# yangao07/LAMSA

Measured on AMD Instinct MI355X. Metric: aligned Gbase/s, 10 kbp ONT-error reads (12%: sub/ins/del 4% each), -T ont2d vs GRCh37-sized stand-in; inputs resident in HBM when the timed region starts (upload excluded: see pcie_inclusive_*), higher is better.
Workload: dtype int32

## Files before the change

### lamsa_amd/csrc/hp_align.h

```cpp
#pragma once
#include "hp_out.h"
#include "hp_sort.h"

namespace hp {

HP_FN void regs_push(ReadCtx &r, Regs &G, int cap, const Rec &rec)
{
    if (G.n >= cap) { r.cx.status |= ST_OVERFLOW; return; }
    const cig_t *c = rec.cig.c; const int n = rec.cig.n, k = G.n;
    const int reflen = cig_reflen(c, n);
    G.rb[k].chr = G.re[k].chr = rec.chr; G.rb[k].is_rev = G.re[k].is_rev = 1 - rec.nstrand;
    if (rec.nstrand == 1) {
        G.beg[k] = (c[0] & 0xf) == C_S ? (c[0] >> 4) + 1 : 1;
        G.end[k] = (c[n - 1] & 0xf) == C_S ? r.L - (c[n - 1] >> 4) : r.L;
        G.rb[k].pos = rec.offset; G.re[k].pos = rec.offset + reflen - 1;
    } else {
        G.beg[k] = (c[n - 1] & 0xf) == C_S ? (c[n - 1] >> 4) + 1 : 1;
        G.end[k] = (c[0] & 0xf) == C_S ? r.L - (c[0] >> 4) : r.L;
        G.re[k].pos = rec.offset; G.rb[k].pos = rec.offset + reflen - 1;
    }
    ++G.n;
}

HP_NOINL void regs_remain(ReadCtx &r, Regs &G, int min_thd, int max_thd)
{
    const lamsa_hp_para *P = r.cx.P;
    G.m = 0;
    if (G.n == 0) {
        if (min_thd < r.L && r.L <= max_thd) { G.r_beg[0] = 1; G.r_end[0] = r.L; G.r_bs[0] = G.r_bn[0] = G.r_es[0] = G.r_en[0] = 0; G.m = 1; }
        return;
    }
    for (int i = 1; i < G.n; ++i) {
        const int b = G.beg[i], e = G.end[i]; const RegB rb = G.rb[i], re = G.re[i];
        int k = i - 1;
        while (k >= 0 && G.beg[k] > b) { G.beg[k + 1] = G.beg[k]; G.end[k + 1] = G.end[k]; G.rb[k + 1] = G.rb[k]; G.re[k + 1] = G.re[k]; --k; }
        G.beg[k + 1] = b; G.end[k + 1] = e; G.rb[k + 1] = rb; G.re[k + 1] = re;
    }
    int gs = 0, g_beg = G.beg[0], g_end = G.end[0];
    int prev_gs = -1, prev_ge = -1, prev_end = 0, first = 1;
    for (int i = 1; i <= G.n; ++i) {
        if (i < G.n && G.beg[i] - g_end - 1 < P->bwt_seed_len) { if (G.end[i] > g_end) g_end = G.end[i]; continue; }
        if (first) {
            if (g_beg > min_thd && g_beg - 1 <= max_thd) { const int m = G.m++; G.r_beg[m] = 1; G.r_end[m] = g_beg - 1; G.r_bs[m] = 0; G.r_bn[m] = 0; G.r_es[m] = gs; G.r_en[m] = i - gs; }
            first = 0;
        } else if (g_beg - prev_end > min_thd && g_beg - 1 - prev_end <= max_thd) {
            const int m = G.m++; G.r_beg[m] = prev_end + 1; G.r_end[m] = g_beg - 1; G.r_bs[m] = prev_gs; G.r_bn[m] = prev_ge - prev_gs; G.r_es[m] = gs; G.r_en[m] = i - gs;
        }
        prev_gs = gs; prev_ge = i; prev_end = g_end;
        if (i < G.n) { gs = i; g_beg = G.beg[i]; g_end = G.end[i]; }
    }
    if (r.L - prev_end > min_thd && r.L - prev_end <= max_thd) {
        HP_STAT(10);
        const int m = G.m++; G.r_beg[m] = prev_end + 1; G.r_end[m] = r.L; G.r_bs[m] = prev_gs; G.r_bn[m] = prev_ge - prev_gs; G.r_es[m] = 0; G.r_en[m] = 0;
    }
}

HP_NOINL void fill_round(ReadCtx &r, const FLines &F, OutBuf &o, Regs *G, int reg_cap, int scale, int tags)
{
    Ctx &cx = r.cx;
    const size_t mark = arena_mark(cx.tmp);
    const LineBufs b = line_bufs(cx, r.L, scale, tags);
    LineRes *la = b.la;
    if (!la) { arena_release(cx.tmp, mark); return; }
    for (int j = 0; j < F.n; ++j) {
        if (!fill_line(r, F, j, *la, b.cur_buf, b.cur_cap, b.rec_buf, b.rec_cap)) break;
        out_line(cx, o, *la);
        if (G && la->tol_score >= 0) for (int k = 0; k <= la->cur_res_n; ++k) regs_push(r, *G, reg_cap, la->rec[k]);
    }
    arena_release(cx.tmp, mark);
}

HP_INL void read_bind(ReadCtx &r, const lamsa_hp_para &P, const RefView &ref, const BatchIn &in, int rd, char *slab, size_t slab_bytes, HP_L int32_t *lds, long long *prof, int lds_words = HP_BOTH_LDS_WORDS)
{
    r.cx.P = &P; r.cx.status = 0; r.cx.n_cells = 0; r.cx.lds_epoch = 0; r.cx.prof_dp = nullptr; r.n_pairs = 0; r.cx.lds = lds; r.cx.lds_words = lds_words; r.cx.prof = prof ? prof + (size_t)rd * 64 : nullptr;
    arena_init(r.cx.tmp, slab, slab_bytes);
    r.ref = ref;
    r.L = (int)(in.read_off[rd + 1] - in.read_off[rd]);
    r.read = in.read_seq + in.read_off[rd];
    r.seed_all = in.seed_all[rd]; r.last_len = in.last_len[rd];
    const int64_t s0 = in.seed_off[rd];
    r.seed_out = (int)(in.seed_off[rd + 1] - s0);
    r.seed_id = in.seed_id + s0; r.hit_off = in.hit_off + s0;
    r.hb = r.hit_off[0];
    r.H = (int)(r.hit_off[r.seed_out] - r.hb);
    r.h_pos = in.h_pos + r.hb; r.h_chr = in.h_chr + r.hb; r.h_cig_off = in.h_cig_off + r.hb; r.h_nm = in.h_nm + r.hb;
    r.h_len_dif = in.h_len_dif + r.hb; r.h_strand = in.h_strand + r.hb; r.h_cig_n = in.h_cig_n + r.hb; r.cig = in.cig;
    r.flip = false; r.cur_read = r.read; r.rc_ready = false; r.rc_read = nullptr; r.t_bases = 0; r.cs_words = 0;
    r.prof = r.cx.prof; r.leaf_bits = nullptr; r.leaf_on = false; r.nodes_ready = false;
}

HP_FN void nodes_fill(ReadCtx &r)
{
    const HP_G int64_t *g_hoff = (const HP_G int64_t *)r.hit_off;
    const HP_G int32_t *g_sid = (const HP_G int32_t *)r.seed_id;
    const HP_G int16_t *g_hnm = (const HP_G int16_t *)r.h_nm;
    const int64_t hb = r.hb;
    const int H = r.H, S = r.seed_out;
    const lamsa_hp_para *P = r.cx.P;
    HP_L int32_t *lo_ = r.cx.lds;
    const bool in_lds = S + 1 <= r.cx.lds_words;
    int min_num = 0;
    if (in_lds) wv::sync();
    for (int s0 = 0; s0 <= S; s0 += 64) {
        wv::Lane<int> few;
        WAVE_FOR(l) {
            const int s = s0 + l;
            int f = 0;
            if (s <= S) { const int o = (int)(g_hoff[s] - hb); if (in_lds) lo_[s] = o; if (s < S) f = (int)(g_hoff[s + 1] - hb) - o <= P->first_loci_thd; }
            few[l] = f;
        }
        min_num += __builtin_popcountll(wv::ballot(few));
    }
    wv::sync();
    const bool all_min = min_num == 0 || min_num * 3 < S;
    HP_G int32_t *g_from = (HP_G int32_t *)r.n_from, *g_in_de = (HP_G int32_t *)r.n_in_de, *g_son_n = (HP_G int32_t *)r.n_son_n, *g_first = (HP_G int32_t *)r.n_first,
                 *g_last = (HP_G int32_t *)r.n_last, *g_ms = (HP_G int32_t *)r.n_max_score, *g_mn = (HP_G int32_t *)r.n_max_NM, *g_mx = (HP_G int32_t *)r.n_max_node,
                 *g_nn = (HP_G int32_t *)r.n_node_n, *g_seed = (HP_G int32_t *)r.n_seed;
    HP_G NodeS *gd = (HP_G NodeS *)r.nd;
    for (int k0 = 0; k0 < H; k0 += 64) {
        WAVE_FOR(l) {
            const int k = k0 + l;
            if (k < H) {
                int lo = 0, hi = S;
                while (hi - lo > 1) { const int mid = (lo + hi) >> 1; if ((in_lds ? lo_[mid] : (int)(g_hoff[mid] - hb)) <= k) lo = mid; else hi = mid; }
                const int s = lo, b = in_lds ? lo_[s] : (int)(g_hoff[s] - hb), e = in_lds ? lo_[s + 1] : (int)(g_hoff[s + 1] - hb);
                const int nm = g_hnm[k];
                g_seed[k] = s;
                const int64_t pos = r.h_pos[k];
                const int w4 = ((int)g_sid[s] & 0xffff) | (((int)r.h_strand[k] & 0xff) << 16) | (((int)r.h_len_dif[k] & 0xff) << 24);
                const int flag = (all_min || e - b <= P->first_loci_thd) ? MIN_FLAG : MULTI_FLAG;
                hp_store16(gd + k, (int)(pos & 0xffffffffll), (int)(pos >> 32), r.h_chr[k], (s << 14) | (k - b));
                hp_store16((HP_G char *)(gd + k) + 16, w4, (flag & 0xff) | (F_INIT << 8) | (F_MATCH << 16), 1, nm);
                g_from[k] = -1; g_nn[k] = 1; g_in_de[k] = 0; g_son_n[k] = 0; g_first[k] = -1; g_last[k] = -1; g_ms[k] = 1; g_mn[k] = nm; g_mx[k] = k;
            }
        }
    }
    r.nodes_ready = true;
    wv::sync();
}

HP_INL void aux_bind(ReadCtx &r, int32_t *nm)
{
    const int c = r.H + 1;
    r.n_from = nm; r.n_in_de = nm + c; r.n_son_n = nm + 2 * c; r.n_first = nm + 3 * c;
    r.n_last = nm + 4 * c; r.n_next = nm + 5 * c; r.n_max_score = nm + 6 * c; r.n_max_NM = nm + 7 * c; r.n_max_node = nm + 8 * c;
    r.n_node_n = nm + 9 * c;
}

#ifdef HP_PROF
#define HP_STAMP(k) do { const long long now_ = wv::clock(); if (a.prof) a.prof[(size_t)rd * 64 + (k)] += now_ - t_last_; t_last_ = now_; } while (0)
#else
#define HP_STAMP(k) do { } while (0)
#endif

HP_NOINL void align_read(const AlignArgs &a, int rd, int wave_slot, HP_L int32_t *lds)
{
#ifdef HP_PROF
    long long t_last_ = wv::clock();
#endif
    ReadCtx r;
    read_bind(r, a.P, a.ref, a.in, rd, a.slab + (size_t)wave_slot * a.slab_per_wave, a.slab_per_wave, lds, a.prof);
    Ctx &cx = r.cx;
    const bool skip = a.in.read_skip && a.in.read_skip[rd];
    if (skip) { cx.status |= ST_UNSUPPORTED; r.H = 0; r.seed_out = 0; }
    const int H = r.H;
    const int tags = fill_tags(a.in.tags);
    const int out_cap = (int)read_out_cap(r.L, a.scale, tags);
    OutBuf o; o.n = 0; o.cap = out_cap;
    o.w = (int32_t *)arena_alloc(cx, sizeof(int32_t) * (size_t)out_cap);
    r.rc_read = (uint8_t *)arena_alloc(cx, (size_t)r.L + 16);
    int32_t *nm = (int32_t *)arena_alloc(cx, sizeof(int32_t) * 11 * (size_t)(H + 1));
    int32_t *sidx = (int32_t *)arena_alloc(cx, sizeof(int32_t) * 2 * (size_t)(H + 1));
    r.nd = (NodeS *)arena_alloc(cx, sizeof(NodeS) * (size_t)(H + 1));
    const int reg_cap = 256 * a.scale;
    Regs G; G.n = 0; G.m = 0;
    G.beg = (int32_t *)arena_alloc(cx, sizeof(int32_t) * 2 * (size_t)reg_cap); G.end = G.beg + reg_cap;
    G.rb = (RegB *)arena_alloc(cx, sizeof(RegB) * 2 * (size_t)reg_cap); G.re = G.rb + reg_cap;
    G.r_beg = (int32_t *)arena_alloc(cx, sizeof(int32_t) * 6 * (size_t)(reg_cap + 2));
    G.r_end = G.r_beg + (reg_cap + 2); G.r_bs = G.r_end + (reg_cap + 2); G.r_bn = G.r_bs + (reg_cap + 2); G.r_es = G.r_bn + (reg_cap + 2); G.r_en = G.r_es + (reg_cap + 2);
    int n0_pos = 1, n1_pos = 2;
    const size_t sort_mark = arena_mark(cx.tmp);
    uint64_t *sort_work = (uint64_t *)arena_alloc(cx, sizeof(uint64_t) * (size_t)(H + 1));
    if (!skip && o.w && r.rc_read && nm && sidx && sort_work && r.nd && G.beg && G.rb && G.r_beg) {
        const int c = H + 1;
        { HP_T0(t_sort_);
        sort_read_hits(r.h_pos, r.h_chr, r.h_strand, H, sidx, sidx + c, sort_work, (HP_L uint64_t *)lds, HP_BOTH_LDS_WORDS / 2, a.sort_pb, a.sort_cb);
        HP_TADD(cx, 46, t_sort_); }
        arena_release(cx.tmp, sort_mark);
        r.srt = sidx; r.rnk = sidx + c;
        aux_bind(r, nm); r.n_seed = nm + 10 * c;
        nodes_fill(r);
        out_put(cx, o, 0); out_put(cx, o, 0); out_put(cx, o, 0);
        HP_STAMP(0);
        {
            const size_t mark = arena_mark(cx.tmp);
            FLines F;
            const bool ok1 = chain_first(r, F);
            HP_STAMP(1);
            if (ok1 && F.n > 0) { o.w[n0_pos] = F.n; fill_round(r, F, o, &G, reg_cap, a.scale, tags); }
            HP_STAMP(2);
            arena_release(cx.tmp, mark);
        }
        if (!(cx.status & ST_DEAD)) {
            const size_t mark = arena_mark(cx.tmp);
            regs_remain(r, G, a.P.seed_len, r.L);
            FLines F;
            const bool ok2 = chain_remain(r, G, F);
            HP_STAMP(3);
            if (ok2 && F.n > 0) { o.w[n1_pos] = F.n; fill_round(r, F, o, nullptr, 0, a.scale, tags); }
            HP_STAMP(4);
            arena_release(cx.tmp, mark);
        }
    }
    const int st = cx.status;
    int n_words = (st & ST_DEAD) || !o.w ? 3 : o.n;
    unsigned long long off = 0;
    if (wv::leader()) off = atomicAdd(a.out.cursor, (unsigned long long)n_words);
    off = (unsigned long long)wv::uni64((long long)off);
    if ((int64_t)(off + (unsigned long long)n_words) <= a.out.stream_cap) {
        int32_t *dst = a.out.stream + off;
        if (n_words == 3 && (!o.w || (st & ST_DEAD))) { dst[0] = st; dst[1] = 0; dst[2] = 0; }
        else {
            o.w[0] = st;
            wv::sync();
            out_copy((HP_G int32_t *)dst, (const HP_G int32_t *)o.w, n_words);
        }
        a.out.read_out_off[rd] = (int64_t)off; a.out.read_out_len[rd] = n_words;
    } else { a.out.read_out_off[rd] = -1; a.out.read_out_len[rd] = 0; }
    a.out.read_status[rd] = st;
    HP_STAMP(5);
    if (a.out.read_tbases) a.out.read_tbases[rd] = (int32_t)(r.t_bases > 0x7fffffffLL ? 0x7fffffffLL : r.t_bases);
    if (a.out.read_work) {
        a.out.read_work[4 * rd] = (int32_t)(cx.n_cells > 0x7fffffffLL ? 0x7fffffffLL : cx.n_cells);
        a.out.read_work[4 * rd + 1] = (int32_t)(r.n_pairs > 0x7fffffffLL ? 0x7fffffffLL : r.n_pairs);
        a.out.read_work[4 * rd + 2] = (int32_t)(r.cs_words > 0x7fffffffLL ? 0x7fffffffLL : r.cs_words);
        a.out.read_work[4 * rd + 3] = 0;
    }
}

}
```

### lamsa_amd/csrc/hp_align_api.hip

```cpp
#include <hip/hip_runtime.h>
#include <algorithm>
#include <atomic>
#include <map>
#include <mutex>
#include <stdlib.h>
#include <string.h>
#include <time.h>
#include "hp_phase.h"
#include "hp_handle.h"
#include "hp_hostprep.h"

using namespace hp;

#ifndef HP_WAVES_PER_SIMD
#define HP_WAVES_PER_SIMD 4
#endif
__global__ __launch_bounds__(64, HP_WAVES_PER_SIMD) void k_align_batch(AlignArgs a)
{
    __shared__ int32_t lds[HP_BOTH_LDS_WORDS];
    const int slot = blockIdx.x;
    for (;;) {
        int u = 0;
        if (wv::leader()) u = atomicAdd(a.counter, 1);
        u = wv::uni(u);
        if (u >= a.n_units) break;
        align_read(a, a.order ? a.order[u] : u, slot, (HP_L int32_t *)lds);
    }
}

#ifndef HP_CHAIN_WAVES_PER_SIMD
#define HP_CHAIN_WAVES_PER_SIMD 4
#endif
#ifndef HP_FILL_WAVES_PER_SIMD
#define HP_FILL_WAVES_PER_SIMD 7
#endif
template <int WORDS, int WPS>
__global__ __launch_bounds__(64, WPS) void k_chain1(const PhaseArgs *ap)
{
    const PhaseArgs &a = *ap;
    constexpr bool ctx_lds = ph_ctx_in_lds(WORDS, WPS);
    __shared__ alignas(16) int32_t lds[WORDS + (ctx_lds ? PH_CTX_BYTES / 4 : 0)];
    ReadCtx &r = *(ctx_lds ? (ReadCtx *)(lds + WORDS) : (ReadCtx *)(a.slab + (size_t)blockIdx.x * a.slab_per_wave));
    for (;;) {
        int u = 0;
        if (wv::leader()) u = atomicAdd(&a.ctl->q_head[0], 1);
        u = wv::uni(u);
        if (u >= a.n_reads) break;
        phase_chain1(a, a.order ? a.order[u] : u, blockIdx.x, (HP_L int32_t *)lds, WORDS, r);
    }
    drain_stamp(a, 0);
}
template <int WORDS, int WPS>
__global__ __launch_bounds__(64, WPS) void k_chain2(const PhaseArgs *ap)
{
    const PhaseArgs &a = *ap;
    constexpr bool ctx_lds = ph_ctx_in_lds(WORDS, WPS);
    __shared__ alignas(16) int32_t lds[WORDS + (ctx_lds ? PH_CTX_BYTES / 4 : 0)];
    ReadCtx &r = *(ctx_lds ? (ReadCtx *)(lds + WORDS) : (ReadCtx *)(a.slab + (size_t)blockIdx.x * a.slab_per_wave));
    for (;;) {
        int u = 0;
        if (wv::leader()) u = atomicAdd(&a.ctl->q_head[2], 1);
        u = wv::uni(u);
        if (u >= a.n_reads) break;
        phase_chain2(a, a.order ? a.order[u] : u, blockIdx.x, (HP_L int32_t *)lds, WORDS, r);
    }
    drain_stamp(a, 2);
}
typedef void (*ChainKernel)(const PhaseArgs *);
struct ChainShape { ChainKernel k1, k2; int lds_words, waves_per_simd; };
static const ChainShape g_chain_shapes[3] = {
    {k_chain1<HP_CHAIN_LDS_WORDS, HP_CHAIN_WAVES_PER_SIMD>, k_chain2<HP_CHAIN_LDS_WORDS, HP_CHAIN_WAVES_PER_SIMD>, HP_CHAIN_LDS_WORDS, HP_CHAIN_WAVES_PER_SIMD},
    {k_chain1<3392, 3>, k_chain2<3392, 3>, 3392, 3},
    {k_chain1<5120, 2>, k_chain2<5120, 2>, 5120, 2},
};
__global__ __launch_bounds__(64, HP_FILL_WAVES_PER_SIMD) void k_fill(const PhaseArgs *ap, int round)
{
    const PhaseArgs &a = *ap;
    __shared__ alignas(16) int32_t lds[HP_LDS_WORDS + PH_CTX_BYTES / 4];
    ReadCtx &r = *(ReadCtx *)(lds + HP_LDS_WORDS);
    int n = 0;
    for (int b = 0; b < PH_NBUCKET; ++b) n += a.ctl->bucket_n[round][b];
    n = wv::uni(n);
    for (;;) {
        int g = 0;
        if (wv::leader()) g = atomicAdd(&a.ctl->q_head[1 + 2 * round], 1);
        g = wv::uni(g);
        if (g >= n) break;
        int b = 0;
        while (b < PH_NBUCKET - 1 && g >= a.ctl->bucket_n[round][b]) { g -= a.ctl->bucket_n[round][b]; ++b; }
        const int u = wv::uni(a.bucket_q[((size_t)round * PH_NBUCKET + b) * a.unit_cap + g]);
        phase_fill(a, round, u, blockIdx.x, (HP_L int32_t *)lds, r);
    }
    drain_stamp(a, 1 + 2 * round);
}
#ifndef HP_FILLDP_WAVES_PER_SIMD
#define HP_FILLDP_WAVES_PER_SIMD 2
#endif
#ifndef HP_LIST_WAVES_PER_SIMD
#define HP_LIST_WAVES_PER_SIMD 4
#endif
__global__ __launch_bounds__(64, HP_LIST_WAVES_PER_SIMD) void k_filllist(const PhaseArgs *ap, int round)
{
    const PhaseArgs &a = *ap;
    __shared__ alignas(16) int32_t lds[PH_CTX_BYTES / 4];
    ReadCtx &r = *(ReadCtx *)lds;
    int n = 0;
    for (int b = 0; b < PH_NBUCKET; ++b) n += a.ctl->bucket_n[round][b];
    n = wv::uni(n);
    for (;;) {
        int g = 0;
        if (wv::leader()) g = atomicAdd(&a.ctl->q_head[5], 1);
        g = wv::uni(g);
        if (g >= n) break;
        int b = 0;
        while (b < PH_NBUCKET - 1 && g >= a.ctl->bucket_n[round][b]) { g -= a.ctl->bucket_n[round][b]; ++b; }
        const int u = wv::uni(a.bucket_q[((size_t)round * PH_NBUCKET + b) * a.unit_cap + g]);
        phase_filllist(a, round, u, blockIdx.x, (HP_L int32_t *)lds, r);
    }
}
__global__ __launch_bounds__(64, 2) void k_filldp_small(const PhaseArgs *ap, int round)
{
    __shared__ int32_t lds[HP_LJ_LDS_WORDS(HP_LJ_QSMALL)];
    const PhaseArgs &a = *ap;
    int n = 0;
    for (int b = 0; b < LJ_NBUCKET; ++b) n += (lj_queue_n(a, round, b) + 63) >> 6;
    n = wv::uni(n);
    for (;;) {
        int g = 0;
        if (wv::leader()) g = atomicAdd(&a.ctl->q_head[6], 1);
        g = wv::uni(g);
        if (g >= n) break;
        int b = 0;
        for (; b < LJ_NBUCKET - 1; ++b) { const int gb = (lj_queue_n(a, round, b) + 63) >> 6; if (g < gb) break; g -= gb; }
        phase_filldp(a, round, b, g * 64, blockIdx.x, (HP_L int32_t *)lds, HP_LJ_QSMALL);
    }
}
__global__ __launch_bounds__(64, HP_WJ_WAVES_PER_SIMD) void k_filldp_wave(const PhaseArgs *ap, int round)
{
    __shared__ int32_t lds[HP_WJ_LDS_WORDS];
    const PhaseArgs &a = *ap;
    int n = 0, n_big = 0;
    for (int b = 0; b < WJ_NBUCKET; ++b) { const int k = wj_queue_n(a, round, b); if (b < WJ_NBIG) n_big += k; else n += k; }
    n = wv::uni(n); n_big = wv::uni(n_big);
    bool own_big = (int)blockIdx.x < a.n_wjb;
    for (;;) {
        int g = 0;
        const bool big = own_big;
        if (wv::leader()) g = atomicAdd(&a.ctl->q_head[big ? 8 : 7], 1);
        g = wv::uni(g);
        if (g >= (big ? n_big : n)) { if (!big) break; own_big = false; continue; }
        phase_wavejob(a, round, g, big, blockIdx.x, (HP_L int32_t *)lds);
    }
}
__global__ __launch_bounds__(64) void k_publish(const PhaseArgs *ap)
{
    const PhaseArgs &a = *ap;
    if (blockIdx.x == 0) publish_diag(a);
    for (;;) {
        int u = 0;
        if (wv::leader()) u = atomicAdd(&a.ctl->q_head[4], 1);
        u = wv::uni(u);
        if (u >= a.n_reads) break;
        phase_publish(a, u);
    }
}

__global__ void k_cig8_expand(const uint8_t *src, int32_t *dst, int64_t n)
{
    for (int64_t i = (int64_t)blockIdx.x * blockDim.x + threadIdx.x; i < n; i += (int64_t)gridDim.x * blockDim.x) { const int b = src[i]; dst[i] = ((b & 63) << 4) | (b >> 6); }
}
__global__ void k_off_widen(const int32_t *src, int64_t *dst, int64_t n)
{
    for (int64_t i = (int64_t)blockIdx.x * blockDim.x + threadIdx.x; i < n; i += (int64_t)gridDim.x * blockDim.x) dst[i] = src[i];
}
#define HP_SCAN_BLOCK 4096
__global__ __launch_bounds__(256) void k_scan_sums(const uint8_t *src, int64_t n, int64_t *sums)
{
    __shared__ int part[256];
    const int64_t b0 = (int64_t)blockIdx.x * HP_SCAN_BLOCK;
    int s = 0;
    for (int i = threadIdx.x; i < HP_SCAN_BLOCK; i += 256) { const int64_t k = b0 + i; s += k < n ? src[k] : 0; }
    part[threadIdx.x] = s;
    __syncthreads();
    for (int st = 128; st > 0; st >>= 1) { if ((int)threadIdx.x < st) part[threadIdx.x] += part[threadIdx.x + st]; __syncthreads(); }
    if (threadIdx.x == 0) sums[blockIdx.x] = part[0];
}
__global__ __launch_bounds__(256) void k_scan_bases(int64_t *sums, int64_t nb)
{
    __shared__ long long tot[256];
    const int64_t per = (nb + 255) / 256, a = (int64_t)threadIdx.x * per, b = a + per < nb ? a + per : nb;
    long long s = 0;
    for (int64_t i = a; i < b; ++i) s += sums[i];
    tot[threadIdx.x] = s;
    __syncthreads();
    if (threadIdx.x == 0) { long long run = 0; for (int t = 0; t < 256; ++t) { const long long v = tot[t]; tot[t] = run; run += v; } }
    __syncthreads();
    long long run = tot[threadIdx.x];
    for (int64_t i = a; i < b; ++i) { const long long v = sums[i]; sums[i] = run; run += v; }
}
__global__ __launch_bounds__(256) void k_scan_apply(const uint8_t *src, int64_t n, const int64_t *bases, int64_t *dst)
{
    __shared__ int part[256];
    const int64_t b0 = (int64_t)blockIdx.x * HP_SCAN_BLOCK + (int64_t)threadIdx.x * 16;
    int v[16], s = 0;
#pragma unroll
    for (int i = 0; i < 16; ++i) { const int64_t k = b0 + i; v[i] = k < n ? src[k] : 0; s += v[i]; }
    part[threadIdx.x] = s;
    __syncthreads();
    if (threadIdx.x == 0) { int run = 0; for (int t = 0; t < 256; ++t) { const int x = part[t]; part[t] = run; run += x; } }
    __syncthreads();
    long long run = bases[blockIdx.x] + part[threadIdx.x];
#pragma unroll
    for (int i = 0; i < 16; ++i) { const int64_t k = b0 + i; if (k < n) dst[k] = run; run += v[i]; }
}

static double now_s() { timespec t; clock_gettime(CLOCK_MONOTONIC, &t); return t.tv_sec + 1e-9 * t.tv_nsec; }
static const bool g_trace = getenv("LAMSA_HP_TRACE") != nullptr;
static const bool g_noshare = getenv("LAMSA_HP_FULL_GRIDS") != nullptr;
static const bool g_nowave = getenv("LAMSA_HP_NO_WAVE_JOBS") != nullptr;
static const bool g_nolane = getenv("LAMSA_HP_NO_LANE_DP") != nullptr;
static const bool g_mono = getenv("LAMSA_HP_ONE_KERNEL") != nullptr;

struct HostBuf {
    void *p = nullptr, *dev = nullptr; size_t cap = 0;
    int ensure(size_t bytes) {
        if (bytes <= cap) return 0;
        if (p) hipHostFree(p);
        p = dev = nullptr; cap = 0;
        size_t want = bytes + bytes / 4 + 256;
        if (hipHostMalloc(&p, want, hipHostMallocMapped) != hipSuccess) { p = nullptr; return -1; }
        if (hipHostGetDevicePointer(&dev, p, 0) != hipSuccess) { hipHostFree(p); p = nullptr; return -1; }
        cap = want;
        return 0;
    }
    void release() { if (p) hipHostFree(p); p = dev = nullptr; cap = 0; }
};

struct OutDev {
    DevBuf buf; HostBuf host; int64_t stream_cap = 0; int n_cap = 0;
    static size_t hdr(int n) { return al256(8 * (size_t)n) + 3 * al256(4 * (size_t)n) + 256 + al256(16 * (size_t)n); }
    int ensure(int n, int64_t cap) { stream_cap = cap; n_cap = n; return buf.ensure(4 * (size_t)cap + 256) || host.ensure(hdr(n) + 256); }
    int64_t *off() const { return (int64_t *)host.dev; }
    int32_t *len(int n) const { return (int32_t *)((char *)host.dev + al256(8 * (size_t)n)); }
    int32_t *st(int n) const { return (int32_t *)((char *)host.dev + al256(8 * (size_t)n) + al256(4 * (size_t)n)); }
    int32_t *tb(int n) const { return (int32_t *)((char *)host.dev + al256(8 * (size_t)n) + 2 * al256(4 * (size_t)n)); }
    unsigned long long *diag(int n) const { return (unsigned long long *)((char *)host.dev + al256(8 * (size_t)n) + 3 * al256(4 * (size_t)n)); }
    const unsigned long long *h_diag(int n) const { return (const unsigned long long *)((const char *)host.p + al256(8 * (size_t)n) + 3 * al256(4 * (size_t)n)); }
    int32_t *work(int n) const { return (int32_t *)((char *)host.dev + al256(8 * (size_t)n) + 3 * al256(4 * (size_t)n) + 256); }
    const int32_t *h_work(int n) const { return (const int32_t *)((const char *)host.p + al256(8 * (size_t)n) + 3 * al256(4 * (size_t)n) + 256); }
    const int64_t *h_off() const { return (const int64_t *)host.p; }
    const int32_t *h_len(int n) const { return (const int32_t *)((const char *)host.p + al256(8 * (size_t)n)); }
    const int32_t *h_st(int n) const { return (const int32_t *)((const char *)host.p + al256(8 * (size_t)n) + al256(4 * (size_t)n)); }
    const int32_t *h_tb(int n) const { return (const int32_t *)((const char *)host.p + al256(8 * (size_t)n) + 2 * al256(4 * (size_t)n)); }
    int32_t *stream(int) const { return (int32_t *)buf.p; }
    void release() { buf.release(); host.release(); }
};

struct Slot {
    DevBuf bin, misc, slab, pers, prof; OutDev out1;
    HostBuf args_host;
    hipEvent_t ep[7] = {nullptr, nullptr, nullptr, nullptr, nullptr, nullptr, nullptr};
    hipStream_t cs = nullptr;
    bool valid = false;
    bool phased = false;
    int32_t n_reads = 0; int64_t n_bases = 0, n_cig = 0, n_hits = 0;
    BatchIn in; const int32_t *d_order = nullptr;
    std::vector<int32_t> order, h_len, h_H; std::vector<uint8_t> h_skip;
    int32_t max_L = 0, max_H = 0;
    int32_t sort_pb = 40, sort_cb = 24;
    hipEvent_t e0 = nullptr, e1 = nullptr;
};

struct AlignState {
    Slot slot[2];
    int fifo[2] = {0, 0}, n_fifo = 0;
    int res_fifo[2] = {0, 0}, n_res = 0;
    DevBuf retry_list;
    OutDev out2;
    HostBuf stream;
    std::vector<int32_t> r_len, r_st, r_tb, r_work; std::vector<int64_t> r_off;
};

static std::map<lamsa_hp_handle *, AlignState *> g_states;
static std::mutex g_states_lock;
static AlignState *state_of(lamsa_hp_handle *h)
{
    std::lock_guard<std::mutex> guard(g_states_lock);
    auto it = g_states.find(h);
    if (it != g_states.end()) return it->second;
    return g_states[h] = new AlignState();
}
extern "C" void lamsa_hp_release_state_(lamsa_hp_handle *h)
{
    AlignState *S = nullptr;
    {
        std::lock_guard<std::mutex> guard(g_states_lock);
        auto it = g_states.find(h);
        if (it == g_states.end()) return;
        S = it->second;
        g_states.erase(it);
    }
    if (h->stream) hipStreamSynchronize(h->stream);
    if (h->stream_b) hipStreamSynchronize(h->stream_b);
    for (Slot &T : S->slot) { T.bin.release(); T.misc.release(); T.slab.release(); T.pers.release(); T.prof.release(); T.args_host.release(); T.out1.release(); for (hipEvent_t e : {T.e0, T.e1, T.ep[0], T.ep[1], T.ep[2], T.ep[3], T.ep[4], T.ep[5], T.ep[6]}) if (e) hipEventDestroy(e); }
    S->retry_list.release(); S->out2.release(); S->stream.release();
    delete S;
}

static int grow(lamsa_hp_handle *h, DevBuf &b, size_t bytes)
{
    if (bytes <= b.cap) return 0;
    if (hipStreamSynchronize(h->stream) != hipSuccess || hipStreamSynchronize(h->stream_b) != hipSuccess) return -1;
    return b.ensure(bytes);
}


static int upload_into(lamsa_hp_handle *h, Slot *S, const lamsa_hp_batch *B)
{
    S->valid = false;
    const double t_0 = now_s();
    const int n = B->n_reads;
    const int64_t n_slots = n ? B->seed_off[n] : 0, n_hits = n_slots ? B->hit_off[n_slots] : 0, n_bases = n ? B->read_off[n] : 0;
    S->h_len.assign((size_t)n, 0); S->h_H.assign((size_t)n, 0); S->h_skip.assign((size_t)n + 1, 0); S->max_L = 0; S->max_H = 0;
    if (n && (B->seed_off[0] != 0 || B->read_off[0] != 0 || (n_slots && B->hit_off[0] != 0))) { h->err = "offsets must start at 0"; return LAMSA_HP_EINVAL; }
    const bool packed_off = B->h_cig_off == nullptr, cig_bytes = B->cig8 != nullptr;
    if (B->n_cig < 0 || (!packed_off && B->n_cig > 0x7fffffffll)) { h->err = "more than 2^31-1 seed CIGAR elements with 32-bit h_cig_off: pass h_cig_off = NULL (CIGARs back to back in hit order) or split the batch"; return LAMSA_HP_EINVAL; }
    if (!cig_bytes && !B->cig && B->n_cig > 0) { h->err = "neither cig nor cig8 given"; return LAMSA_HP_EINVAL; }
    {
        std::atomic<int> bad(0);
        const int64_t sl = h->para.seed_len, ss = h->para.seed_step > 0 ? h->para.seed_step : 1;
        std::atomic<long long> max_pos(0), sum_cig(0);
        hp_parallel_blocks(n, [&](int r0, int r1) {
            long long mp = 0, sc = 0;
            for (int r = r0; r < r1 && !bad.load(std::memory_order_relaxed); ++r) {
                const int64_t L = B->read_off[r + 1] - B->read_off[r], ns = B->seed_off[r + 1] - B->seed_off[r];
                if (L < 0 || L > (1 << 24) || ns < 0) { bad = 1; return; }
                if (ns > HP_MAX_SLOTS) S->h_skip[r] = 1;
                {
                    const int64_t sa = L < sl ? 0 : 1 + (L - sl) / ss;
                    if (B->seed_all[r] != sa || B->last_len[r] != L - sl - (sa - 1) * ss) { bad = 7; return; }
                    if (sa > 32767) S->h_skip[r] = 1;
                }
                int64_t H = 0;
                for (int64_t s = B->seed_off[r]; s < B->seed_off[r + 1]; ++s) {
                    const int64_t m = B->hit_off[s + 1] - B->hit_off[s];
                    if (m < 0 || (m > HP_MAX_HITS_PER_SEED && !S->h_skip[r])) { bad = 2; return; }
                    if (B->seed_id[s] < 1 || B->seed_id[s] > B->seed_all[r] || (s > B->seed_off[r] && B->seed_id[s] <= B->seed_id[s - 1])) { bad = 3; return; }
                    H += m;
                }
                if (H > (1 << 22) && !S->h_skip[r]) { bad = 4; return; }
                for (int64_t i = B->read_off[r]; i < B->read_off[r + 1]; ++i) if (B->read_seq[i] > 4) { bad = 5; return; }
                for (int64_t k = B->hit_off[B->seed_off[r]]; k < B->hit_off[B->seed_off[r + 1]]; ++k) {
                    mp = B->h_pos[k] > mp ? B->h_pos[k] : mp;
                    if (B->h_len_dif[k] < -127 || B->h_len_dif[k] > 127) S->h_skip[r] = 1;
                    if (B->h_chr[k] < 1 || B->h_chr[k] > h->n_seqs || (B->h_strand[k] != 1 && B->h_strand[k] != -1) || B->h_pos[k] < 0 || B->h_pos[k] >= (1ll << 40) ||
                        (!packed_off && (B->h_cig_off[k] < 0 || (int64_t)B->h_cig_off[k] + B->h_cig_n[k] > B->n_cig))) { bad = 6; return; }
                    sc += B->h_cig_n[k];
                }
                S->h_len[r] = (int32_t)L; S->h_H[r] = (int32_t)H;
            }
            long long seen = max_pos.load();
            while (mp > seen && !max_pos.compare_exchange_weak(seen, mp)) { }
            sum_cig += sc;
        });
        static const char *why[] = {"", "read longer than 2^24 bases", "too many hits in one seed", "seed ids must be ascending in [1, seed_all]",
                                    "too many hits in one read", "read base code > 4",
                                    "bad hit record (contig id, strand, position or seed CIGAR range)",
                                    "seed_all / last_len do not match the read length and the handle's seed length and step"};
        if (bad) { h->err = why[bad.load()]; return LAMSA_HP_EINVAL; }
        if (packed_off && sum_cig.load() != B->n_cig) { h->err = "h_cig_off is NULL but the h_cig_n do not add up to n_cig"; return LAMSA_HP_EINVAL; }
        for (int r = 0; r < n; ++r) { if (S->h_skip[r]) { S->h_len[r] = 0; S->h_H[r] = 0; } S->max_L = std::max(S->max_L, S->h_len[r]); S->max_H = std::max(S->max_H, S->h_H[r]); }
        auto bits = [](unsigned long long x) { int b = 0; while (x) { ++b; x >>= 1; } return b; };
        S->sort_pb = bits((unsigned long long)max_pos.load()); S->sort_cb = bits((unsigned long long)(2 * (long long)h->n_seqs + 1));
    }
    const double t_1 = now_s();
    S->order.resize((size_t)n);
    for (int r = 0; r < n; ++r) S->order[r] = r;
    {
        std::vector<double> cost((size_t)n);
        for (int r = 0; r < n; ++r) cost[r] = (double)S->h_H[r] * S->h_H[r] / 64.0 + (double)S->h_len[r] * (2.0 * h->para.band_w + 1) / 16.0;
        std::stable_sort(S->order.begin(), S->order.end(), [&](int x, int y) { return cost[x] > cost[y]; });
    }
    size_t off = 0;
    auto place = [&](size_t bytes) { size_t o = off; off = al256(off + bytes + 16); return o; };
    const size_t o_roff = place(8 * ((size_t)n + 1)), o_rseq = place((size_t)n_bases), o_sall = place(4 * (size_t)n), o_last = place(4 * (size_t)n),
                 o_soff = place(8 * ((size_t)n + 1)), o_sid = place(4 * (size_t)n_slots), o_hoff = place(8 * ((size_t)n_slots + 1)),
                 o_pos = place(8 * (size_t)n_hits), o_chr = place(4 * (size_t)n_hits), o_coff = place(8 * (size_t)n_hits), o_nm = place(2 * (size_t)n_hits),
                 o_ld = place(2 * (size_t)n_hits), o_st = place((size_t)n_hits), o_cn = place((size_t)n_hits), o_cig = place(4 * (size_t)B->n_cig), o_ord = place(4 * (size_t)n),
                 o_stage = place(packed_off ? 8 * ((size_t)n_hits / HP_SCAN_BLOCK + 2) : 4 * (size_t)n_hits), o_cig8 = place(cig_bytes ? (size_t)B->n_cig : 0), o_skip = place((size_t)n);
    const double t_3 = now_s();
    if (S->bin.ensure(off)) { h->err = "hipMalloc(batch)"; return LAMSA_HP_ENOMEM; }
    char *d = (char *)S->bin.p;
    hipStream_t s = h->copy_stream;
    static const int64_t zero64 = 0;
#define UP(o, src, bytes) do { if ((bytes) > 0) HIPCHK(h, hipMemcpyAsync(d + (o), (src), (bytes), hipMemcpyHostToDevice, s), LAMSA_HP_EKERNEL); } while (0)
    if (n) { UP(o_roff, B->read_off, 8 * ((size_t)n + 1)); UP(o_soff, B->seed_off, 8 * ((size_t)n + 1)); }
    else { UP(o_roff, &zero64, 8); UP(o_soff, &zero64, 8); }
    UP(o_rseq, B->read_seq, (size_t)n_bases); UP(o_sall, B->seed_all, 4 * (size_t)n); UP(o_last, B->last_len, 4 * (size_t)n);
    UP(o_sid, B->seed_id, 4 * (size_t)n_slots);
    if (n_slots) UP(o_hoff, B->hit_off, 8 * ((size_t)n_slots + 1)); else UP(o_hoff, &zero64, 8);
    UP(o_pos, B->h_pos, 8 * (size_t)n_hits); UP(o_chr, B->h_chr, 4 * (size_t)n_hits);
    if (!packed_off) UP(o_stage, B->h_cig_off, 4 * (size_t)n_hits);
    UP(o_nm, B->h_nm, 2 * (size_t)n_hits); UP(o_ld, B->h_len_dif, 2 * (size_t)n_hits); UP(o_st, B->h_strand, (size_t)n_hits); UP(o_cn, B->h_cig_n, (size_t)n_hits);
    if (cig_bytes) UP(o_cig8, B->cig8, (size_t)B->n_cig); else UP(o_cig, B->cig, 4 * (size_t)B->n_cig);
    UP(o_ord, S->order.data(), 4 * (size_t)n); UP(o_skip, S->h_skip.data(), (size_t)n);
#undef UP
    if (cig_bytes && B->n_cig > 0) hipLaunchKernelGGL(k_cig8_expand, dim3(2048), dim3(256), 0, s, (const uint8_t *)(d + o_cig8), (int32_t *)(d + o_cig), (int64_t)B->n_cig);
    if (n_hits > 0) {
        if (!packed_off) hipLaunchKernelGGL(k_off_widen, dim3(2048), dim3(256), 0, s, (const int32_t *)(d + o_stage), (int64_t *)(d + o_coff), (int64_t)n_hits);
        else {
            const int64_t nb = (n_hits + HP_SCAN_BLOCK - 1) / HP_SCAN_BLOCK;
            hipLaunchKernelGGL(k_scan_sums, dim3((unsigned)nb), dim3(256), 0, s, (const uint8_t *)(d + o_cn), (int64_t)n_hits, (int64_t *)(d + o_stage));
            hipLaunchKernelGGL(k_scan_bases, dim3(1), dim3(256), 0, s, (int64_t *)(d + o_stage), nb);
            hipLaunchKernelGGL(k_scan_apply, dim3((unsigned)nb), dim3(256), 0, s, (const uint8_t *)(d + o_cn), (int64_t)n_hits, (const int64_t *)(d + o_stage), (int64_t *)(d + o_coff));
        }
    }
    HIPCHK(h, hipGetLastError(), LAMSA_HP_EKERNEL);
    HIPCHK(h, hipStreamSynchronize(s), LAMSA_HP_EKERNEL);
    if (g_trace) fprintf(stderr, "[lamsa_hp] upload: validate %.1f ms, order %.1f ms, copy %.1f ms (%.2f GB on the device)\n", 1e3 * (t_1 - t_0), 1e3 * (t_3 - t_1), 1e3 * (now_s() - t_3), off / 1e9);
    BatchIn &in = S->in;
    in.n_reads = n; in.read_skip = (const uint8_t *)(d + o_skip); in.read_off = (const int64_t *)(d + o_roff); in.read_seq = (const uint8_t *)(d + o_rseq);
    in.seed_all = (const int32_t *)(d + o_sall); in.last_len = (const int32_t *)(d + o_last); in.seed_off = (const int64_t *)(d + o_soff);
    in.seed_id = (const int32_t *)(d + o_sid); in.hit_off = (const int64_t *)(d + o_hoff); in.h_pos = (const int64_t *)(d + o_pos);
    in.h_chr = (const int32_t *)(d + o_chr); in.h_cig_off = (const int64_t *)(d + o_coff); in.h_nm = (const int16_t *)(d + o_nm);
    in.h_len_dif = (const int16_t *)(d + o_ld); in.h_strand = (const int8_t *)(d + o_st); in.h_cig_n = (const uint8_t *)(d + o_cn);
    in.cig = (const int32_t *)(d + o_cig);
    S->d_order = (const int32_t *)(d + o_ord);
    S->n_reads = n; S->n_bases = n_bases; S->n_cig = B->n_cig; S->n_hits = n_hits;
    S->valid = true;
    return LAMSA_HP_OK;
}

static int cap_waves(int n_waves, size_t slab_per_wave, int n_cu)
{
    static const size_t budget = []() { size_t f = 0, t = 0; if (hipMemGetInfo(&f, &t) != hipSuccess || t == 0) { t = (size_t)288 << 30; f = t; } return std::min(t / 4, f / 3); }();
    if (slab_per_wave * (size_t)n_waves <= budget) return n_waves;
    size_t fit = budget / (slab_per_wave ? slab_per_wave : 1);
    if (n_cu > 0 && fit >= (size_t)n_cu) fit -= fit % (size_t)n_cu;
    return fit < 1 ? 1 : (int)fit;
}

#ifdef HP_PROF
static void prof_report(Slot &T, const long long *d_prof, int n)
{
    if (!d_prof) return;
    {
        std::vector<long long> pr((size_t)n * 64);
        hipMemcpy(pr.data(), d_prof, sizeof(long long) * pr.size(), hipMemcpyDeviceToHost);
        if (const char *dump = getenv("LAMSA_HP_PROF_DUMP")) {
            if (FILE *fp = fopen(dump, "wb")) {
                for (int r = 0; r < n; ++r) { long long hl[2] = {T.h_H[r], T.h_len[r]}; fwrite(hl, 8, 2, fp); fwrite(&pr[(size_t)r * 64], 8, 64, fp); }
                fclose(fp);
            }
        }
        std::vector<int> idx((size_t)n); for (int i = 0; i < n; ++i) idx[i] = i;
        auto tot = [&](int r) { long long t = 0; for (int k = 0; k < 6; ++k) t += pr[(size_t)r * 64 + k]; return t; };
        std::sort(idx.begin(), idx.end(), [&](int x, int y) { return tot(x) > tot(y); });
        long long sum[64] = {0}; for (int r = 0; r < n; ++r) for (int k = 0; k < 64; ++k) sum[k] += pr[(size_t)r * 64 + k];
        fprintf(stderr, "[HP_PROF] cycles: setup chain1 fill1 chain2 fill2 publish | in chain1: init+minext mainscan track pop-loop bound+flines | o_l H\n");
        fprintf(stderr, "[HP_PROF] SUM  "); for (int k = 0; k < 11; ++k) fprintf(stderr, " %lld", sum[k] / 1000000); fprintf(stderr, " (Mcycles) targets %lld trips %lld init_Mcyc %lld\n", sum[11], sum[12], sum[13] / 1000000);
#ifdef HP_PROF_TRACK
        fprintf(stderr, "[HP_PROF] branch tracking (-DHP_PROF_TRACK: the line_build stamps below are off): marking pass, image build and write-back %lld Mcyc; %lld seeds visited; %lld tracks, %lld Mcyc in them, %lld steps up; "
                        "%lld arrivals at a node with several sons, %lld Mcyc in cut_branch\n", sum[16] / 1000000, sum[19], sum[18], sum[17] / 1000000, sum[20], sum[21], sum[22] / 1000000);
#endif
#ifdef HP_PROF_EDGE
        fprintf(stderr, "[HP_PROF] main pass (-DHP_PROF_EDGE: the line_build stamps below are off), Mcyc: dp_cluster_lds load+pack %lld, MIN extension %lld, target loop %lld, write-back %lld; cluster_lane %lld; build_sons %lld\n",
                sum[16] / 1000000, sum[17] / 1000000, sum[18] / 1000000, sum[19] / 1000000, sum[20] / 1000000, sum[21] / 1000000);
#else
        fprintf(stderr, "[HP_PROF] line_build: %lld lines (%lld without a gap), %lld anchors, %lld gaps | Mcyc: anchor walk %lld, gap list %lld, gaps in lanes %lld, gaps one by one %lld, assembly %lld\n",
                sum[21], sum[22], sum[12], sum[23], sum[16] / 1000000, sum[17] / 1000000, sum[18] / 1000000, sum[19] / 1000000, sum[20] / 1000000);
#endif
        fprintf(stderr, "[HP_PROF] gaps: %lld in lines with fewer than HP_GAP_MIN gaps (%lld lines with gaps); lane gaps: %lld hits scanned, %lld refused (range too long or too many active hits)\n", sum[54], sum[55], sum[11], sum[13]);
        { const char *nm[] = {"ksw_global", "ksw_extend", "backtrack", "ref_fetch", "head_fix", "frag_extend", "split_mapping", "tail_fix", "res_split", "res_aux", "mini_line_regs", "sort index"};
          for (int k = 0; k < 12; ++k) fprintf(stderr, "[HP_PROF] %-16s %8lld Mcyc %10lld calls\n", nm[k], sum[24 + 2 * k] / 1000000, sum[25 + 2 * k]);
#ifdef HP_PROF_FILL
          fprintf(stderr, "[HP_PROF] in frags_merge: boundary repair (merge_cigar_full) %lld Mcyc %lld calls; junctions through split_mapping %lld Mcyc %lld calls; fragments of several seeds %lld Mcyc %lld calls; 64-step gathers %lld Mcyc %lld\n", sum[16] / 1000000, sum[17], sum[18] / 1000000, sum[19], sum[20] / 1000000, sum[21], sum[22] / 1000000, sum[23]);
#endif
          fprintf(stderr, "[HP_PROF] direction-matrix bytes in HBM %lld (%lld jobs); hits passed through nodes_per_init %lld (%lld calls)\n", sum[52], sum[53], sum[54], sum[55]);
          fprintf(stderr, "[HP_PROF] chain_first start: seed loop %lld, node_set loop %lld, min_extend %lld Mcyc (%lld reads with a MIN pass)\n", sum[56] / 1000000, sum[57] / 1000000, sum[58] / 1000000, sum[59]);
          fprintf(stderr, "[HP_PROF] query <= 62: ksw_extend %lld Mcyc %lld calls, ksw_global %lld Mcyc %lld calls\n", sum[60] / 1000000, sum[61], sum[62] / 1000000, sum[63]);
          const char *bn[] = {"[bi_extend total]", "[bi_extend after left ext]", "17-32", "33-64", "65-128", "129-256", "257-512", ">512"};
          for (int k = 0; k < 2; ++k) fprintf(stderr, "[HP_PROF] ksw_extend qlen %-8s %8lld Mcyc %10lld calls\n", bn[k], sum[48 + 2 * k] / 1000000, sum[49 + 2 * k]); }
        {
            std::vector<long long> pd((size_t)n * 64);
            hipMemcpy(pd.data(), d_prof + ((size_t)n + 1) * 64, sizeof(long long) * pd.size(), hipMemcpyDeviceToHost);
            long long sd[64] = {0}; for (int r = 0; r < n; ++r) for (int k = 0; k < 64; ++k) sd[k] += pd[(size_t)r * 64 + k];
            const char *cn[] = {"one set, q <= 62", "packed, one set", "packed, two sets", "band 1 set slides", "band 2 sets slides", "band 4 sets slides", "int32 sets", "LDS / HBM rows",
                                "band 1 set fixed", "band 2 sets fixed", "band 4 sets fixed"};
            for (int c = 0; c < 11; ++c) fprintf(stderr, "[HP_PROF] wave jobs, ksw_extend %-18s %8lld Mcyc %10lld Mcells %9lld calls %10lld rows\n", cn[c], sd[4 * c] / 1000000, sd[4 * c + 1] / 1000000, sd[4 * c + 2], sd[4 * c + 3]);
            fprintf(stderr, "[HP_PROF] wave jobs, junctions of the class 'band 2 sets fixed': %lld jobs, wj_run %lld Mcyc of which staging %lld; ksw_bi_extend %lld Mcyc of which after the left extension %lld; "
                            "in ksw_extend_band<2>: setup and first fill %lld, rows %lld, backtrack %lld Mcyc\n",
                    sd[51], sd[50] / 1000000, sd[49] / 1000000, sd[47] / 1000000, sd[48] / 1000000, sd[44] / 1000000, sd[45] / 1000000, sd[46] / 1000000);
        }
        for (int q = 0; q < 8 && q < n; ++q) { int r = idx[q]; fprintf(stderr, "[HP_PROF] read %d L=%d:", r, T.h_len[r]); for (int k = 0; k < 11; ++k) fprintf(stderr, " %lld", pr[(size_t)r * 64 + k] / 1000000); fprintf(stderr, " | o_l %lld H %lld | targets %lld trips %lld init_Mcyc %lld\n", pr[(size_t)r * 64 + 14], pr[(size_t)r * 64 + 15], pr[(size_t)r * 64 + 11], pr[(size_t)r * 64 + 12], pr[(size_t)r * 64 + 13] / 1000000); }
    }
}
#endif

struct PhasedLayout { size_t bytes, o[15]; int unit_cap, lj_cap, wj_cap; int64_t fl_cap, line_cap, job_cap; };
static PhasedLayout phased_layout(int n, int64_t n_hits, int64_t n_bases, int64_t stream_cap)
{
    PhasedLayout Y;
    const size_t n_ent = (size_t)n_hits + (size_t)n + 1;
    Y.unit_cap = 8 * n + 1024;
    Y.fl_cap = 4 * n_hits + 2304 * (int64_t)n + 4096; Y.line_cap = stream_cap + 64 * (int64_t)Y.unit_cap;
    Y.job_cap = std::min<int64_t>(0x7fffff00ll, 4096 + 256 * (int64_t)n + 2 * n_bases);
    Y.lj_cap = (int)std::min<int64_t>(0x3fffffffll, 1024 + 16 * (int64_t)n + n_bases / 100);
    Y.wj_cap = (int)std::min<int64_t>(0x3fffffffll, 1024 + 32 * (int64_t)n + n_bases / 200);
    size_t off = 0;
    auto place = [&](size_t bytes) { size_t o = off; off = al256(off + bytes + 16); return o; };
    const size_t sz[15] = {sizeof(PhaseArgs), sizeof(PhaseCtl), sizeof(RdMeta) * ((size_t)n + 1), sizeof(NodeS) * n_ent, 4 * n_ent, 8 * n_ent, sizeof(UnitRec) * 2 * (size_t)Y.unit_cap,
                           4 * 2 * (size_t)PH_NBUCKET * Y.unit_cap, 4 * (size_t)Y.fl_cap, 4 * (size_t)Y.line_cap, 4 * (size_t)Y.job_cap, sizeof(LjRec) * (size_t)Y.lj_cap, 4 * (size_t)LJ_NBUCKET * Y.lj_cap,
                           sizeof(WjRec) * (size_t)Y.wj_cap, 4 * (size_t)WJ_NBUCKET * Y.wj_cap};
    for (int k = 0; k < 15; ++k) Y.o[k] = place(sz[k]);
    Y.bytes = off;
    return Y;
}

struct SlabPlan { size_t chain, fill, wj, wjb, wjb_off; int w_chain, w_fill, w_dp, w_wj, n_wjb, shape; size_t bytes; };
static int chain_shape(const lamsa_hp_para &P, int64_t n_reads, int64_t n_bases)
{
    static const int force = getenv("LAMSA_HP_CHAIN_SHAPE") ? atoi(getenv("LAMSA_HP_CHAIN_SHAPE")) : -1;
    if (force >= 0 && force < 3) return force;
    const int64_t mean_L = n_reads > 0 ? n_bases / n_reads : 0, ss = P.seed_step > 0 ? P.seed_step : 1;
    const int64_t est = mean_L / ss * 2 / 3;
    for (int k = 0; k < 2; ++k) if (est <= g_chain_shapes[k].lds_words / 5) return k;
    return 2;
}
static SlabPlan slab_plan(lamsa_hp_handle *h, int max_L, int max_H, bool shared = false, int shape = 0)
{
    SlabPlan Q;
    Q.shape = shape;
    const lamsa_hp_para &P = h->para;
    Q.chain = al256(((size_t)256 << 10) + 128 * (size_t)max_L + 424 * (size_t)max_H);
    Q.fill = al256(fill_slab_bytes(max_L, h->result_tags, sizeof(cig_t) * 3 * HP_LJ_CIG * 64 + (size_t)HP_LJ_QSMALL * HP_LJ_TSMALL * 64 + 64));
    { static const int kb = getenv("LAMSA_HP_WJ_SLAB_KB") ? atoi(getenv("LAMSA_HP_WJ_SLAB_KB")) : 0;
      Q.wj = ((size_t)(kb > 0 ? kb : 1024) << 10) + 33 * 256; }
    Q.wjb = al256((size_t)wj_need(&P, WJ_HEAD, max_L, max_L + 2 * P.hash_step + 64) + ((size_t)64 << 10)) + 33 * 256;
    if (Q.wjb < Q.wj) Q.wjb = Q.wj;
    if (g_nowave) Q.fill = std::max(Q.fill, al256(read_slab_bytes(P.band_w, max_L, max_H, 1, h->result_tags)));
    if (h->scratch_limit) { const size_t lim = al256(h->scratch_limit); Q.chain = std::min(Q.chain, lim); Q.fill = std::min(Q.fill, lim); Q.wj = std::min(Q.wj, lim); Q.wjb = std::min(Q.wjb, lim); }
    int pc = 0, pf = 0, pd = 0, pw = 0;
    if (hipOccupancyMaxActiveBlocksPerMultiprocessor(&pc, g_chain_shapes[shape].k1, 64, 0) != hipSuccess || pc < 1) pc = 4 * g_chain_shapes[shape].waves_per_simd;
    if (hipOccupancyMaxActiveBlocksPerMultiprocessor(&pf, k_fill, 64, 0) != hipSuccess || pf < 1) pf = 4;
    if (hipOccupancyMaxActiveBlocksPerMultiprocessor(&pd, k_filldp_small, 64, 0) != hipSuccess || pd < 1) pd = 4;
    if (hipOccupancyMaxActiveBlocksPerMultiprocessor(&pw, k_filldp_wave, 64, 0) != hipSuccess || pw < 1) pw = 4;
    if (shared && !g_noshare) { pc = std::min(pc, 8); pf = std::min(pf, 16); pw = std::min(pw, 16); }
    { static const int cf = getenv("LAMSA_HP_FILL_PER_CU") ? atoi(getenv("LAMSA_HP_FILL_PER_CU")) : 0, cc = getenv("LAMSA_HP_CHAIN_PER_CU") ? atoi(getenv("LAMSA_HP_CHAIN_PER_CU")) : 0,
                       cw = getenv("LAMSA_HP_WJ_PER_CU") ? atoi(getenv("LAMSA_HP_WJ_PER_CU")) : 0;
      if (cf > 0 && cf < pf) pf = cf;
      if (cc > 0 && cc < pc) pc = cc;
      if (cw > 0 && cw < pw) pw = cw; }
    Q.w_chain = cap_waves(h->n_cu * pc, Q.chain, h->n_cu); Q.w_fill = cap_waves(h->n_cu * pf, Q.fill, h->n_cu);
    Q.w_dp = std::min(h->n_cu * pd, Q.w_fill); Q.w_wj = cap_waves(h->n_cu * pw, Q.wj, h->n_cu);
    { const size_t budget_big = (size_t)12 << 30; size_t nb = budget_big / Q.wjb; if (nb < 1) nb = 1; Q.n_wjb = (int)std::min<size_t>(nb, (size_t)Q.w_wj); }
    Q.wjb_off = al256(Q.wj * (size_t)Q.w_wj);
    const size_t wj_bytes = Q.wjb_off + Q.wjb * (size_t)Q.n_wjb;
    Q.bytes = std::max(std::max(Q.chain * (size_t)Q.w_chain, Q.fill * (size_t)Q.w_fill), wj_bytes);
    return Q;
}

static int launch_phased(lamsa_hp_handle *h, AlignState *S, Slot &T, Slot &Ln, OutDev &O, hipEvent_t e0, hipEvent_t e1)
{
    const int n = T.n_reads;
    const int64_t n_hits = T.n_hits;
    const SlabPlan Q = slab_plan(h, T.max_L, T.max_H, S->n_fifo + S->n_res > 0, chain_shape(h->para, T.n_reads, T.n_bases));
    const int w_chain = Q.w_chain, w_fill = Q.w_fill, w_dp = Q.w_dp, w_wj = Q.w_wj;
    const PhasedLayout Y = phased_layout(n, n_hits, T.n_bases, O.stream_cap);
    const int unit_cap = Y.unit_cap, lj_cap = Y.lj_cap; const int64_t fl_cap = Y.fl_cap, line_cap = Y.line_cap, job_cap = Y.job_cap;
    const size_t off = Y.bytes, o_args = Y.o[0], o_ctl = Y.o[1], o_meta = Y.o[2], o_nd = Y.o[3], o_ns = Y.o[4], o_sx = Y.o[5], o_un = Y.o[6], o_bq = Y.o[7], o_fl = Y.o[8], o_ln = Y.o[9],
                 o_jb = Y.o[10], o_lj = Y.o[11], o_lq = Y.o[12], o_wj = Y.o[13], o_wq = Y.o[14];
    if (grow(h, Ln.slab, Q.bytes) || grow(h, Ln.pers, off) || Ln.misc.ensure(256)) { h->err = "hipMalloc(slab)"; return LAMSA_HP_ENOMEM; }
    char *d = (char *)Ln.pers.p;
    PhaseArgs a;
    a.P = h->para;
    a.ref.pac = h->d_pac; a.ref.l_pac = h->l_pac; a.ref.n_seqs = h->n_seqs; a.ref.seq_off = h->d_seq_off; a.ref.seq_len = h->d_seq_len;
    a.in = T.in; a.in.tags = h->result_tags;
    a.out.read_out_off = O.off(); a.out.read_out_len = O.len(n); a.out.read_status = O.st(n); a.out.read_tbases = O.tb(n); a.out.read_work = O.work(n); a.out.stream = O.stream(n);
    a.out.stream_cap = O.stream_cap; a.out.cursor = (unsigned long long *)((char *)Ln.misc.p + 64); a.out.diag = O.diag(n);
    a.slab = (char *)Ln.slab.p; a.slab_per_wave = Q.chain; a.slab_fill = Q.fill; a.slab_wj = Q.wj; a.slab_wjb = Q.wjb; a.wjb_off = Q.wjb_off; a.n_wjb = Q.n_wjb; a.sort_pb = T.sort_pb; a.sort_cb = T.sort_cb;
    a.order = T.d_order; a.n_reads = n; a.prof = nullptr;
#ifdef HP_PROF
    if (Ln.prof.ensure(sizeof(long long) * 64 * 2 * ((size_t)n + 1))) { h->err = "hipMalloc(prof)"; return LAMSA_HP_ENOMEM; }
    a.prof = (long long *)Ln.prof.p;
    HIPCHK(h, hipMemsetAsync(Ln.prof.p, 0, sizeof(long long) * 64 * 2 * ((size_t)n + 1), Ln.cs), LAMSA_HP_EKERNEL);
#endif
    a.g_nd = (NodeS *)(d + o_nd); a.g_nseed = (int32_t *)(d + o_ns); a.g_sidx = (int32_t *)(d + o_sx); a.meta = (RdMeta *)(d + o_meta);
    a.units = (UnitRec *)(d + o_un); a.unit_cap = unit_cap; a.bucket_q = (int32_t *)(d + o_bq);
    a.fl_base = (int32_t *)(d + o_fl); a.fl_cap = fl_cap; a.line_base = (int32_t *)(d + o_ln); a.line_cap = line_cap; a.ctl = (PhaseCtl *)(d + o_ctl);
    a.job_base = (int32_t *)(d + o_jb); a.job_cap = job_cap;
    a.ljobs = (LjRec *)(d + o_lj); a.lj_bucket = (int32_t *)(d + o_lq); a.lj_cap = g_nolane ? 0 : lj_cap;
    a.wjobs = (WjRec *)(d + o_wj); a.wj_bucket = (int32_t *)(d + o_wq); a.wj_cap = g_nowave ? 0 : Y.wj_cap;
    const bool list = !g_nolane || !g_nowave;
    hipStream_t s = Ln.cs;
    HIPCHK(h, hipMemsetAsync(Ln.misc.p, 0, 128, s), LAMSA_HP_EKERNEL);
    HIPCHK(h, hipMemsetAsync(d + o_ctl, 0, (o_meta - o_ctl) + sizeof(RdMeta) * ((size_t)n + 1), s), LAMSA_HP_EKERNEL);
    if (Ln.args_host.ensure(sizeof a)) { h->err = "hipHostMalloc(args)"; return LAMSA_HP_ENOMEM; }
    memcpy(Ln.args_host.p, &a, sizeof a);
    HIPCHK(h, hipMemcpyAsync(d + o_args, Ln.args_host.p, sizeof a, hipMemcpyHostToDevice, s), LAMSA_HP_EKERNEL);
    const PhaseArgs *da = (const PhaseArgs *)(d + o_args);
    HIPCHK(h, hipEventRecord(e0, s), LAMSA_HP_EKERNEL);
    hipLaunchKernelGGL(g_chain_shapes[Q.shape].k1, dim3(std::min(w_chain, n)), dim3(64), 0, s, da);
    HIPCHK(h, hipEventRecord(Ln.ep[0], s), LAMSA_HP_EKERNEL);
    if (list) {
        hipLaunchKernelGGL(k_filllist, dim3(w_fill), dim3(64), 0, s, da, 0);
        HIPCHK(h, hipEventRecord(Ln.ep[5], s), LAMSA_HP_EKERNEL);
        if (!g_nowave) hipLaunchKernelGGL(k_filldp_wave, dim3(w_wj), dim3(64), 0, s, da, 0);
        HIPCHK(h, hipEventRecord(Ln.ep[6], s), LAMSA_HP_EKERNEL);
        if (!g_nolane) hipLaunchKernelGGL(k_filldp_small, dim3(w_dp), dim3(64), 0, s, da, 0);
    } else { HIPCHK(h, hipEventRecord(Ln.ep[5], s), LAMSA_HP_EKERNEL); HIPCHK(h, hipEventRecord(Ln.ep[6], s), LAMSA_HP_EKERNEL); }
    HIPCHK(h, hipEventRecord(Ln.ep[4], s), LAMSA_HP_EKERNEL);
    hipLaunchKernelGGL(k_fill, dim3(w_fill), dim3(64), 0, s, da, 0);
    HIPCHK(h, hipEventRecord(Ln.ep[1], s), LAMSA_HP_EKERNEL);
    hipLaunchKernelGGL(g_chain_shapes[Q.shape].k2, dim3(std::min(w_chain, n)), dim3(64), 0, s, da);
    HIPCHK(h, hipEventRecord(Ln.ep[2], s), LAMSA_HP_EKERNEL);
    if (list) {
        HIPCHK(h, hipMemsetAsync(&((PhaseCtl *)(d + o_ctl))->q_head[5], 0, 16, s), LAMSA_HP_EKERNEL);
        hipLaunchKernelGGL(k_filllist, dim3(w_fill), dim3(64), 0, s, da, 1);
        if (!g_nowave) hipLaunchKernelGGL(k_filldp_wave, dim3(w_wj), dim3(64), 0, s, da, 1);
        if (!g_nolane) hipLaunchKernelGGL(k_filldp_small, dim3(w_dp), dim3(64), 0, s, da, 1);
    }
    hipLaunchKernelGGL(k_fill, dim3(w_fill), dim3(64), 0, s, da, 1);
    HIPCHK(h, hipEventRecord(Ln.ep[3], s), LAMSA_HP_EKERNEL);
    hipLaunchKernelGGL(k_publish, dim3(std::min(h->n_cu * 8, n)), dim3(64), 0, s, da);
    HIPCHK(h, hipGetLastError(), LAMSA_HP_EKERNEL);
    HIPCHK(h, hipEventRecord(e1, s), LAMSA_HP_EKERNEL);
    Ln.phased = true;
    return LAMSA_HP_OK;
}

static int launch_align(lamsa_hp_handle *h, AlignState *S, Slot &T, Slot &Ln, OutDev &O, const int32_t *d_order, int n_units, int scale, int max_L, int max_H,
                        hipEvent_t e0, hipEvent_t e1, bool wait)
{
    size_t slab_per_wave = al256(read_slab_bytes(h->para.band_w, max_L, max_H, scale, h->result_tags));
    if (scale == 1 && h->scratch_limit && slab_per_wave > h->scratch_limit) slab_per_wave = al256(h->scratch_limit);
    int per_cu = 0;
    if (hipOccupancyMaxActiveBlocksPerMultiprocessor(&per_cu, k_align_batch, 64, 0) != hipSuccess || per_cu < 1) per_cu = 4;
    int n_waves = h->n_cu * per_cu;
    if (n_waves > n_units) n_waves = n_units;
    n_waves = cap_waves(n_waves, slab_per_wave, h->n_cu);
    if (grow(h, Ln.slab, slab_per_wave * (size_t)n_waves) || Ln.misc.ensure(256)) { h->err = "hipMalloc(slab)"; return LAMSA_HP_ENOMEM; }
    const int n = T.n_reads;
    AlignArgs a;
    a.P = h->para;
    a.ref.pac = h->d_pac; a.ref.l_pac = h->l_pac; a.ref.n_seqs = h->n_seqs; a.ref.seq_off = h->d_seq_off; a.ref.seq_len = h->d_seq_len;
    a.in = T.in; a.in.tags = h->result_tags;
    a.out.read_out_off = O.off(); a.out.read_out_len = O.len(n); a.out.read_status = O.st(n); a.out.read_tbases = O.tb(n); a.out.read_work = O.work(n); a.out.stream = O.stream(n);
    a.out.stream_cap = O.stream_cap; a.out.cursor = (unsigned long long *)((char *)Ln.misc.p + 64); a.out.diag = nullptr;
    a.slab = (char *)Ln.slab.p; a.slab_per_wave = slab_per_wave; a.counter = (int32_t *)Ln.misc.p;
    a.order = d_order; a.n_units = n_units; a.scale = scale; a.prof = nullptr; a.sort_pb = T.sort_pb; a.sort_cb = T.sort_cb;
    hipStream_t s = Ln.cs;
    HIPCHK(h, hipMemsetAsync(Ln.misc.p, 0, 128, s), LAMSA_HP_EKERNEL);
    HIPCHK(h, hipEventRecord(e0, s), LAMSA_HP_EKERNEL);
    hipLaunchKernelGGL(k_align_batch, dim3(n_waves), dim3(64), 0, s, a);
    HIPCHK(h, hipGetLastError(), LAMSA_HP_EKERNEL);
    HIPCHK(h, hipEventRecord(e1, s), LAMSA_HP_EKERNEL);
    if (wait) HIPCHK(h, hipStreamSynchronize(s), LAMSA_HP_EKERNEL);
#ifdef HP_PROF
    prof_report(T, a.prof, n);
#endif
    return LAMSA_HP_OK;
}

static int slot_events(lamsa_hp_handle *h, Slot &Ln)
{
    Ln.cs = &Ln == &state_of(h)->slot[1] ? h->stream_b : h->stream;
    if (!Ln.e0) HIPCHK(h, hipEventCreate(&Ln.e0), LAMSA_HP_EKERNEL);
    if (!Ln.e1) HIPCHK(h, hipEventCreate(&Ln.e1), LAMSA_HP_EKERNEL);
    for (hipEvent_t &e : Ln.ep) if (!e) HIPCHK(h, hipEventCreate(&e), LAMSA_HP_EKERNEL);
    return LAMSA_HP_OK;
}

static int start_main(lamsa_hp_handle *h, AlignState *S, Slot &T, Slot &Ln)
{
    int rc = slot_events(h, Ln);
    if (rc) return rc;
    const int n = T.n_reads;
    if (n == 0) return LAMSA_HP_OK;
    if (Ln.out1.ensure(n, batch_out_cap(n, T.n_bases, h->result_tags))) { h->err = "hipMalloc(out)"; return LAMSA_HP_ENOMEM; }
    Ln.phased = false;
    if (!g_mono) return launch_phased(h, S, T, Ln, Ln.out1, Ln.e0, Ln.e1);
    return launch_align(h, S, T, Ln, Ln.out1, T.d_order, n, 1, T.max_L, T.max_H, Ln.e0, Ln.e1, false);
}

#define DL(dst, src, bytes) HIPCHK(h, hipMemcpyAsync((dst), (src), (bytes), hipMemcpyDeviceToHost, h->copy_stream), LAMSA_HP_EKERNEL)
#define DLSYNC() HIPCHK(h, hipStreamSynchronize(h->copy_stream), LAMSA_HP_EKERNEL)

static int finish_main(lamsa_hp_handle *h, AlignState *S, Slot &T, Slot &Ln, lamsa_hp_result *R)
{
    const int n = T.n_reads;
    for (float &v : h->kernel_ms) v = 0;
    S->r_st.assign((size_t)n + 1, 0); S->r_off.assign((size_t)n + 1, 0); S->r_len.assign((size_t)n + 1, 0); S->r_tb.assign((size_t)n + 1, 0); S->r_work.assign(4 * (size_t)n + 4, 0);
    if (S->stream.ensure(64)) { h->err = "hipHostMalloc(results)"; return LAMSA_HP_ENOMEM; }
    if (n == 0) {
        if (R) { R->stream = (const int32_t *)S->stream.p; R->stream_words = 0; R->read_off = S->r_off.data(); R->read_len = S->r_len.data(); R->read_status = S->r_st.data(); R->read_tbases = S->r_tb.data(); R->read_work = S->r_work.data(); }
        return LAMSA_HP_OK;
    }
    const double t_0 = now_s();
    HIPCHK(h, hipEventSynchronize(Ln.e1), LAMSA_HP_EKERNEL);
    const double t_1 = now_s();
    hipEventElapsedTime(&h->kernel_ms[0], Ln.e0, Ln.e1);
    if (Ln.phased) {
        hipEvent_t ev[6] = {Ln.e0, Ln.ep[0], Ln.ep[1], Ln.ep[2], Ln.ep[3], Ln.e1};
        for (int k = 0; k < 5; ++k) hipEventElapsedTime(&h->kernel_ms[2 + k], ev[k], ev[k + 1]);
        const unsigned long long *dg = Ln.out1.h_diag(n);
        for (int k = 0; k < 4; ++k) h->kernel_ms[7 + k] = dg[2 * k + 1] >= dg[2 * k] && dg[2 * k + 1] ? (float)((double)(dg[2 * k + 1] - dg[2 * k]) * 1e-5) : 0.f;
        h->kernel_ms[11] = (float)dg[8]; h->kernel_ms[12] = (float)dg[9];
        hipEventElapsedTime(&h->kernel_ms[13], Ln.ep[0], Ln.ep[4]);
        hipEventElapsedTime(&h->kernel_ms[14], Ln.ep[0], Ln.ep[5]);
        hipEventElapsedTime(&h->kernel_ms[15], Ln.ep[5], Ln.ep[6]);
        h->kernel_ms[16] = (float)dg[12]; h->kernel_ms[17] = (float)((double)dg[13] * 1e-6); h->kernel_ms[18] = (float)dg[14]; h->kernel_ms[19] = (float)((double)dg[15] * 4e-6); h->kernel_ms[20] = (float)((double)dg[16] * 1e-6);
#ifdef HP_PROF
        prof_report(T, (const long long *)Ln.prof.p, n);
#endif
    }
    memcpy(S->r_off.data(), Ln.out1.h_off(), 8 * (size_t)n); memcpy(S->r_len.data(), Ln.out1.h_len(n), 4 * (size_t)n);
    memcpy(S->r_st.data(), Ln.out1.h_st(n), 4 * (size_t)n); memcpy(S->r_tb.data(), Ln.out1.h_tb(n), 4 * (size_t)n); memcpy(S->r_work.data(), Ln.out1.h_work(n), 16 * (size_t)n);
    unsigned long long used1 = 0;
    for (int r = 0; r < n; ++r) if (S->r_off[r] >= 0 && (unsigned long long)(S->r_off[r] + S->r_len[r]) > used1) used1 = (unsigned long long)(S->r_off[r] + S->r_len[r]);
    if ((int64_t)used1 > Ln.out1.stream_cap) used1 = (unsigned long long)Ln.out1.stream_cap;
    std::vector<int32_t> again;
    for (int r = 0; r < n; ++r) if ((S->r_st[r] & LAMSA_HP_ST_OVERFLOW) || S->r_off[r] < 0) again.push_back(r);
#ifdef HP_CHAIN_STOP
    again.clear();
#endif
    unsigned long long used2 = 0;
    if (!again.empty()) {
        int mL = 0, mH = 0; int64_t cap2 = 1024;
        for (int r : again) { mL = std::max(mL, T.h_len[r]); mH = std::max(mH, T.h_H[r]); cap2 += read_out_cap(T.h_len[r], 8, h->result_tags); }
        if (grow(h, S->out2.buf, 4 * (size_t)cap2 + 256) || S->out2.host.ensure(OutDev::hdr(n) + 256) || grow(h, S->retry_list, 4 * again.size())) { h->err = "hipMalloc(retry)"; return LAMSA_HP_ENOMEM; }
        S->out2.stream_cap = cap2;
        HIPCHK(h, hipMemcpyAsync(S->retry_list.p, again.data(), 4 * again.size(), hipMemcpyHostToDevice, Ln.cs), LAMSA_HP_EKERNEL);
        int rc = launch_align(h, S, T, Ln, S->out2, (const int32_t *)S->retry_list.p, (int)again.size(), 8, mL, mH, h->ev0, h->ev1, true);
        if (rc) return rc;
        hipEventElapsedTime(&h->kernel_ms[1], h->ev0, h->ev1);
        const int64_t *off2 = S->out2.h_off(); const int32_t *len2 = S->out2.h_len(n), *st2 = S->out2.h_st(n), *tb2 = S->out2.h_tb(n), *wk2 = S->out2.h_work(n);
        for (int r : again) if (off2[r] >= 0 && (unsigned long long)(off2[r] + len2[r]) > used2) used2 = (unsigned long long)(off2[r] + len2[r]);
        if ((int64_t)used2 > cap2) used2 = (unsigned long long)cap2;
        for (int r : again) { S->r_st[r] = st2[r]; S->r_len[r] = len2[r]; S->r_tb[r] = tb2[r]; for (int q = 0; q < 4; ++q) S->r_work[4 * r + q] = wk2[4 * r + q]; S->r_off[r] = off2[r] < 0 ? -1 : (int64_t)used1 + off2[r]; }
    }
    for (int r = 0; r < n; ++r) if (S->r_off[r] < 0) { S->r_off[r] = 0; S->r_len[r] = 0; S->r_st[r] |= LAMSA_HP_ST_OVERFLOW; }
    if (!R) return LAMSA_HP_OK;
    if (S->stream.ensure(4 * (size_t)(used1 + used2) + 64)) { h->err = "hipHostMalloc(results)"; return LAMSA_HP_ENOMEM; }
    int32_t *hs = (int32_t *)S->stream.p;
    if (used1) DL(hs, Ln.out1.stream(n), 4 * (size_t)used1);
    if (used2) DL(hs + used1, S->out2.stream(n), 4 * (size_t)used2);
    DLSYNC();
    if (g_trace) fprintf(stderr, "[lamsa_hp] collect: waited %.1f ms for the kernel (%.1f ms), results %.1f ms (%.2f GB)\n", 1e3 * (t_1 - t_0), h->kernel_ms[0], 1e3 * (now_s() - t_1), 4e-9 * (double)(used1 + used2));
    R->stream = hs; R->stream_words = (int64_t)(used1 + used2); R->read_off = S->r_off.data(); R->read_len = S->r_len.data(); R->read_status = S->r_st.data(); R->read_tbases = S->r_tb.data(); R->read_work = S->r_work.data();
    return LAMSA_HP_OK;
}
#undef DL
#undef DLSYNC

static int check_batch_args(lamsa_hp_handle *h, const lamsa_hp_batch *B)
{
    if (!h || !B || B->n_reads < 0) return LAMSA_HP_EINVAL;
    if (!h->d_pac) { h->err = "handle was created without a reference"; return LAMSA_HP_EINVAL; }
    HIPCHK(h, hipSetDevice(h->device), LAMSA_HP_ENODEV);
    return LAMSA_HP_OK;
}

extern "C" int lamsa_hp_upload_batch(lamsa_hp_handle *h, const lamsa_hp_batch *B)
{
    int rc = check_batch_args(h, B);
    if (rc) return rc;
    AlignState *S = state_of(h);
    if (S->n_fifo || S->n_res) { h->err = "batches are in flight: collect them first"; return LAMSA_HP_EINVAL; }
    return upload_into(h, &S->slot[0], B);
}

extern "C" int lamsa_hp_run_uploaded(lamsa_hp_handle *h, lamsa_hp_result *R)
{
    if (!h) return LAMSA_HP_EINVAL;
    AlignState *S = state_of(h);
    if (S->n_fifo) { h->err = "submitted batches are in flight: collect them first"; return LAMSA_HP_EINVAL; }
    if (!S->slot[0].valid) { h->err = "no batch uploaded"; return LAMSA_HP_EINVAL; }
    HIPCHK(h, hipSetDevice(h->device), LAMSA_HP_ENODEV);
    if (S->n_res) { h->err = "runs of the resident batch are in flight: finish them first"; return LAMSA_HP_EINVAL; }
    int rc = start_main(h, S, S->slot[0], S->slot[0]);
    if (rc) return rc;
    return finish_main(h, S, S->slot[0], S->slot[0], R);
}

extern "C" int lamsa_hp_start_uploaded(lamsa_hp_handle *h)
{
    if (!h) return LAMSA_HP_EINVAL;
    AlignState *S = state_of(h);
    if (S->n_fifo) { h->err = "submitted batches are in flight: collect them first"; return LAMSA_HP_EINVAL; }
    if (!S->slot[0].valid) { h->err = "no batch uploaded"; return LAMSA_HP_EINVAL; }
    if (S->n_res >= 2) { h->err = "two runs are already in flight: finish one first"; return LAMSA_HP_EINVAL; }
    HIPCHK(h, hipSetDevice(h->device), LAMSA_HP_ENODEV);
    const int k = S->n_res == 1 ? 1 - S->res_fifo[0] : 0;
    S->slot[1].valid = false;
    const int rc = start_main(h, S, S->slot[0], S->slot[k]);
    if (rc) return rc;
    S->res_fifo[S->n_res++] = k;
    return LAMSA_HP_OK;
}

extern "C" int lamsa_hp_finish_uploaded(lamsa_hp_handle *h, lamsa_hp_result *R)
{
    if (!h) return LAMSA_HP_EINVAL;
    AlignState *S = state_of(h);
    if (S->n_res == 0) { h->err = "no run in flight"; return LAMSA_HP_EINVAL; }
    HIPCHK(h, hipSetDevice(h->device), LAMSA_HP_ENODEV);
    const int k = S->res_fifo[0];
    S->res_fifo[0] = S->res_fifo[1]; --S->n_res;
    return finish_main(h, S, S->slot[0], S->slot[k], R);
}

extern "C" int lamsa_hp_align_batch(lamsa_hp_handle *h, const lamsa_hp_batch *B, lamsa_hp_result *R)
{
    int rc = lamsa_hp_upload_batch(h, B);
    if (rc) return rc;
    return lamsa_hp_run_uploaded(h, R);
}

extern "C" int lamsa_hp_submit_batch(lamsa_hp_handle *h, const lamsa_hp_batch *B)
{
    int rc = check_batch_args(h, B);
    if (rc) return rc;
    AlignState *S = state_of(h);
    if (S->n_res) { h->err = "runs of the resident batch are in flight: finish them first"; return LAMSA_HP_EINVAL; }
    if (S->n_fifo >= 2) { h->err = "two batches are already in flight: collect one first"; return LAMSA_HP_EINVAL; }
    const int k = S->n_fifo == 1 ? 1 - S->fifo[0] : 0;
    rc = upload_into(h, &S->slot[k], B);
    if (rc) return rc;
    const double t_s = now_s();
    rc = start_main(h, S, S->slot[k], S->slot[k]);
    if (g_trace) fprintf(stderr, "[lamsa_hp] submit: launch queued in %.1f ms (scratch and output buffers are allocated on first use)\n", 1e3 * (now_s() - t_s));
    if (rc) { S->slot[k].valid = false; return rc; }
    S->fifo[S->n_fifo++] = k;
    return LAMSA_HP_OK;
}

extern "C" int lamsa_hp_collect_batch(lamsa_hp_handle *h, lamsa_hp_result *R)
{
    if (!h) return LAMSA_HP_EINVAL;
    AlignState *S = state_of(h);
    if (S->n_fifo == 0) { h->err = "no batch in flight"; return LAMSA_HP_EINVAL; }
    HIPCHK(h, hipSetDevice(h->device), LAMSA_HP_ENODEV);
    const int k = S->fifo[0];
    S->fifo[0] = S->fifo[1]; --S->n_fifo;
    const int rc = finish_main(h, S, S->slot[k], S->slot[k], R);
    S->slot[k].valid = false;
    return rc;
}

extern "C" void *lamsa_hp_host_alloc(size_t bytes)
{
    void *p = nullptr;
    if (hipHostMalloc(&p, bytes ? bytes : 1, hipHostMallocDefault) != hipSuccess) return nullptr;
    return p;
}
extern "C" void lamsa_hp_host_free(void *p) { if (p) hipHostFree(p); }

extern "C" int lamsa_hp_reserve(lamsa_hp_handle *h, int32_t n_reads, int64_t n_bases, int64_t n_hits, int64_t n_cig, int32_t max_read_len, int32_t max_hits_per_read)
{
    if (!h || n_reads < 0 || n_bases < 0 || n_hits < 0 || n_cig < 0) return LAMSA_HP_EINVAL;
    HIPCHK(h, hipSetDevice(h->device), LAMSA_HP_ENODEV);
    AlignState *S = state_of(h);
    if (S->n_fifo || S->n_res) { h->err = "batches are in flight"; return LAMSA_HP_EINVAL; }
    const SlabPlan Q = slab_plan(h, max_read_len, max_hits_per_read, false, chain_shape(h->para, n_reads, n_bases));
    const int64_t cap = batch_out_cap(n_reads, n_bases, h->result_tags);
    const PhasedLayout Y = phased_layout(n_reads, n_hits, n_bases, cap);
    const size_t in_bytes = (size_t)n_bases + 16 * (size_t)n_reads * 4 + 32 * ((size_t)n_hits + n_reads) + 8 * (size_t)n_hits + 5 * (size_t)n_cig + 64 * 256 + 4096;
    for (Slot &T : S->slot) {
        int rc = slot_events(h, T);
        if (rc) return rc;
        if (T.slab.ensure(Q.bytes) || T.pers.ensure(Y.bytes) || T.misc.ensure(256) || T.bin.ensure(in_bytes) || T.out1.ensure(n_reads, cap)) {
            for (Slot &U : S->slot) { U.slab.release(); U.pers.release(); U.bin.release(); U.out1.release(); }
            h->err = "hipMalloc(reserve)"; return LAMSA_HP_ENOMEM;
        }
    }
    return LAMSA_HP_OK;
}

extern "C" int lamsa_hp_set_scratch_limit(lamsa_hp_handle *h, size_t bytes)
{
    if (!h || (bytes && bytes < ((size_t)64 << 10))) return LAMSA_HP_EINVAL;
    h->scratch_limit = bytes;
    return LAMSA_HP_OK;
}

extern "C" int lamsa_hp_set_result_tags(lamsa_hp_handle *h, int flags)
{
    if (!h) return LAMSA_HP_EINVAL;
    if (!result_tags_valid(flags)) { h->err = "result tags: an unknown item, or LAMSA_HP_TAG_SUMMARY (no CIGAR is shipped) with an item that lists or splits"; return LAMSA_HP_EINVAL; }
    AlignState *S = state_of(h);
    if (S->n_fifo || S->n_res) { h->err = "batches are in flight: collect them first"; return LAMSA_HP_EINVAL; }
    h->result_tags = flags;
    return LAMSA_HP_OK;
}
```

### lamsa_amd/csrc/hp_core.h

```cpp
#pragma once
#include <hp/wave.h>
#include "../../include/lamsa_hp.h"

namespace hp {

typedef int32_t cig_t;
enum { C_M = 0, C_I = 1, C_D = 2, C_N = 3, C_S = 4, C_H = 5, C_EQ = 7, C_X = 8 };
enum { ST_OVERFLOW = LAMSA_HP_ST_OVERFLOW, ST_REFEXIT = LAMSA_HP_ST_REFEXIT, ST_UNSUPPORTED = LAMSA_HP_ST_UNSUPPORTED,
       ST_DEAD = ST_OVERFLOW | ST_REFEXIT | ST_UNSUPPORTED };

#define HP_NEG_INF (-0x40000000)

struct Arena {
    char *base; size_t cap, top;
};
HP_INL void arena_init(Arena &a, void *base, size_t cap) { a.base = (char *)base; a.cap = cap; a.top = 0; }
HP_INL size_t arena_mark(const Arena &a) { return a.top; }
HP_INL void arena_release(Arena &a, size_t m) { a.top = m; }

#ifndef HP_LDS_CELLS
#define HP_LDS_CELLS 512
#endif
#ifndef HP_LDS_Z_BYTES
#define HP_LDS_Z_BYTES 512
#endif
#define HP_LDS_WORDS (2 * HP_LDS_CELLS + HP_LDS_CELLS / 4 + HP_LDS_Z_BYTES / 4)
#ifndef HP_CHAIN_LDS_WORDS
#define HP_CHAIN_LDS_WORDS 2432
#endif
#define HP_BOTH_LDS_WORDS (HP_CHAIN_LDS_WORDS > HP_LDS_WORDS ? HP_CHAIN_LDS_WORDS : HP_LDS_WORDS)
#define HP_LANE_STRIP_WORDS HP_CHAIN_LDS_WORDS

struct Ctx {
    const lamsa_hp_para *P;
    HP_L int32_t *lds;
    int lds_words;
    Arena tmp;
    int status;
    long long n_cells;
    long long *prof;
    long long *prof_dp = nullptr;
    int lds_epoch;
};
#if defined(HP_PROF_EDGE) && (defined(HP_PROF_TRACK) || defined(HP_PROF_FILL))
#error "-DHP_PROF_EDGE, -DHP_PROF_TRACK and -DHP_PROF_FILL all use prof slots 16 .. 23: one of them per build"
#endif
#ifdef HP_PROF_FILL
#define HP_PROF_CHAIN_ON 0
#define HP_TADD_FILL(cx, slot, v) HP_TADD(cx, slot, v)
#else
#define HP_PROF_CHAIN_ON 1
#define HP_TADD_FILL(cx, slot, v) do { } while (0)
#endif
#ifdef HP_PROF
#define HP_T0(v) const long long v = wv::clock()
#define HP_TADD(cx, slot, v) do { if ((cx).prof) { (cx).prof[slot] += wv::clock() - (v); (cx).prof[(slot) + 1] += 1; } } while (0)
#else
#define HP_T0(v) do { } while (0)
#define HP_TADD(cx, slot, v) do { } while (0)
#endif

#ifndef HP_DPLOG
#define HP_DPLOG(kind, qlen, tlen, w, cells) do { } while (0)
#endif
#ifndef HP_STAT
#define HP_STAT(i) do { } while (0)
#endif
#ifndef HP_STAT_ADD
#define HP_STAT_ADD(i, n) ((void)0)
#endif
#ifndef HP_STAT_MAX
#define HP_STAT_MAX(i, v) ((void)0)
#endif
#ifdef HP_STAT_SLOTS
static_assert(HP_STAT_SLOTS >= 97, "the array of the path counters ends before the last slot the device sources use");
#define HP_STATX_ADD(i, n) HP_STAT_ADD(i, n)
#define HP_STATX_MAX(i, v) HP_STAT_MAX(i, v)
#else
#define HP_STATX_ADD(i, n) ((void)0)
#define HP_STATX_MAX(i, v) ((void)0)
#endif

HP_INL void *arena_alloc(Ctx &cx, size_t bytes) {
    size_t b = (bytes + 15) & ~(size_t)15;
    if (cx.tmp.top + b > cx.tmp.cap) { cx.status |= ST_OVERFLOW; return nullptr; }
    void *p = cx.tmp.base + cx.tmp.top;
    cx.tmp.top += b;
    return p;
}

struct CigV { cig_t *c; int n, cap; };
HP_INL void cig_bind(CigV &v, cig_t *mem, int cap) { v.c = mem; v.n = 0; v.cap = mem ? cap : 0; }
HP_INL bool cig_alloc(Ctx &cx, CigV &v, int cap) {
    cig_t *m = (cig_t *)arena_alloc(cx, (size_t)cap * sizeof(cig_t));
    cig_bind(v, m, cap);
    return m != nullptr;
}
HP_INL void cig_raw_push(Ctx &cx, CigV &v, cig_t w) {
    if (v.n >= v.cap) { cx.status |= ST_OVERFLOW; return; }
    v.c[v.n++] = w;
}
HP_INL void cig_push0(Ctx &cx, CigV &v, cig_t w) {
    if (v.n > 0 && (v.c[v.n - 1] & 0xf) == (w & 0xf)) { v.c[v.n - 1] += (w >> 4) << 4; return; }
    cig_raw_push(cx, v, w);
}
HP_INL void cig_push1(Ctx &cx, CigV &v, cig_t w) { if ((w >> 4) == 0) return; cig_push0(cx, v, w); }
HP_FN void cig_pushv(Ctx &cx, CigV &v, const cig_t *c, int n) {
    if (n == 0) return;
    const HP_G cig_t *src = (const HP_G cig_t *)c;
    HP_G cig_t *dst = (HP_G cig_t *)v.c;
    const int vn = v.n;
    int j = 0;
    if (vn > 0) {
        const cig_t last = dst[vn - 1], c0 = src[0];
        if ((last & 0xf) == (c0 & 0xf)) { dst[vn - 1] = last + ((c0 >> 4) << 4); j = 1; }
        else if (((last & 0xf) == C_I && (c0 & 0xf) == C_S) || ((last & 0xf) == C_S && (c0 & 0xf) == C_I)) {
            dst[vn - 1] = (((last >> 4) + (c0 >> 4)) << 4) | C_S; j = 1;
        }
    }
    const int m = n - j;
    if (vn + m > v.cap) { cx.status |= ST_OVERFLOW; return; }
    for (int b0 = 0; b0 < m; b0 += 64) { WAVE_FOR(l) { const int i = b0 + l; if (i < m) dst[vn + i] = src[j + i]; } }
    v.n = vn + m;
    wv::sync();
}
HP_FN void cig_pushw(Ctx &cx, CigV &v, cig_t w) {
    if (v.n > 0) {
        const cig_t last = v.c[v.n - 1];
        if ((last & 0xf) == (w & 0xf)) { v.c[v.n - 1] = last + ((w >> 4) << 4); return; }
        if (((last & 0xf) == C_I && (w & 0xf) == C_S) || ((last & 0xf) == C_S && (w & 0xf) == C_I)) { v.c[v.n - 1] = (((last >> 4) + (w >> 4)) << 4) | C_S; return; }
    }
    if (v.n + 1 > v.cap) { cx.status |= ST_OVERFLOW; return; }
    v.c[v.n++] = w;
}
HP_FN void cig_invert(cig_t *c, int n) {
    HP_G cig_t *g = (HP_G cig_t *)c;
    for (int b0 = 0; b0 < n / 2; b0 += 64) {
        WAVE_FOR(l) { const int a = b0 + l; if (a < n / 2) { const cig_t x = g[a], y = g[n - 1 - a]; g[a] = y; g[n - 1 - a] = x; } }
    }
    wv::sync();
}
HP_FN int cig_readlen(const cig_t *c, int n) {
    const HP_G cig_t *g = (const HP_G cig_t *)c;
    int tot = 0;
    for (int b0 = 0; b0 < n; b0 += 64) {
        wv::Lane<int> x;
        WAVE_FOR(l) { const int i = b0 + l; int v = 0; if (i < n) { const cig_t w = g[i]; const int op = w & 0xf; if (op == C_M || op == C_I || op == C_S) v = w >> 4; } x[l] = v; }
        tot += wv::reduce_sum(x);
    }
    return tot;
}
HP_FN int cig_reflen(const cig_t *c, int n) {
    const HP_G cig_t *g = (const HP_G cig_t *)c;
    int tot = 0;
    for (int b0 = 0; b0 < n; b0 += 64) {
        wv::Lane<int> x;
        WAVE_FOR(l) { const int i = b0 + l; int v = 0; if (i < n) { const cig_t w = g[i]; const int op = w & 0xf; if (op == C_M || op == C_D || op == C_H) v = w >> 4; } x[l] = v; }
        tot += wv::reduce_sum(x);
    }
    return tot;
}

struct Seq { const uint8_t *p; int stride; };
HP_INL int seq_at(const Seq &s, int i) { return s.p[(long)i * s.stride]; }
HP_INL Seq seq_fwd(const uint8_t *p) { Seq s; s.p = p; s.stride = 1; return s; }
HP_INL Seq seq_rev(const uint8_t *p, int len) { Seq s; s.p = p + (len > 0 ? len - 1 : 0); s.stride = -1; return s; }

HP_INL int sub_score(const lamsa_hp_para *P, int t, int q) { return (t > 3 || q > 3) ? -1 : (t == q ? P->match : -P->mis); }

HP_INL int iabs(int x) { return x < 0 ? -x : x; }
HP_INL int imin(int a, int b) { return a < b ? a : b; }
HP_INL int imax(int a, int b) { return a > b ? a : b; }

}
```

### lamsa_amd/csrc/hp_fill.h

```cpp
#pragma once
#include "hp_split.h"
#include "hp_lalign.h"

namespace hp {

#define HP_REC_MAX 64

struct Rec {
    int64_t offset, refend; int32_t chr, nstrand, readend, score, NM; CigV cig;
    int32_t *mm; int32_t n_mm;
    int32_t sum[8];
};
struct LineRes {
    int line_score, tol_score, tol_NM, cur_res_n;
    int32_t *ev; int ev_cap;
    int tags;
    Rec rec[HP_REC_MAX];
};


HP_INL bool contig_clip(const RefView &ref, int chr, int64_t start0, int32_t &len)
{
    const int32_t clen = ref.seq_len[chr - 1];
    if (start0 > clen || start0 < 0) return false;
// ... 247 lines not shown
#undef HP_MF_E2
        if (ok) {
            vn = n1;
            if (n1 > 0) c1c[n1 - 1] = e1;
            const int last = cig_pushv_known(cx, c1c, vn, c1cap, e1, bd.c, bd.n, bd_first);
            cig_pushv_known(cx, c1c, vn, c1cap, last, _c2 + ci, c2_n - ci, e2);
        }
        arena_release(cx.tmp, mark);
        if (!ok) return false;
    }
    c1.n = vn;
    *c1_refend = refend0 + c2_reflen;
    *c1_readend = readend0 + c2_readlen;
    HP_TADD_FILL(cx, 16, tmf_);
    return true;
}

HP_INL bool merge_cigar(ReadCtx &r, CigV &c1, int64_t *c1_refend, int *c1_readend, int chr,
                        const cig_t *_c2, int c2_n, int c2_reflen, int c2_readlen)
{
    if (c2_n == 0) return true;
    const int n1 = c1.n;
    if (n1 > 1) {
        const cig_t t = ((const HP_G cig_t *)c1.c)[n1 - 1], h = ((const HP_G cig_t *)_c2)[0];
        const int top = t & 0xf, hop = h & 0xf;
        if ((((top == C_I || top == C_D) && (t >> 4) <= 3) && hop != C_S && hop != C_H) ||
            (((hop == C_I || hop == C_D) && (h >> 4) <= 3) && top != C_S && top != C_H))
            return merge_cigar_full(r, c1, c1_refend, c1_readend, chr, _c2, c2_n, c2_reflen, c2_readlen);
    }
    cig_pushv(r.cx, c1, _c2, c2_n);
    *c1_refend += c2_reflen;
    *c1_readend += c2_readlen;
    return true;
}

#ifndef HP_FRAG_BLOCK_MIN
#define HP_FRAG_BLOCK_MIN 3
#endif
HP_INL int seed_at_after_block(const HP_G int32_t *g_seed, int i, int step, int nb) { return g_seed[i + step * (nb - 1)]; }

HP_INL bool frag_step(ReadCtx &r, const FLines &F, int frag, int i, int chr, CigV &fc, int64_t &ref_end, int &re, int &last)
{
    Ctx &cx = r.cx;
    const lamsa_hp_para *P = cx.P;
    const int s = F.fr_seed[F.fr_seed_off[frag] + i];
    GapGeo g;
    const bool inside = gap_geo(r, r.h_strand[last] == 1, last, s, g);
    const int32_t *gt = F.gt ? F.gt + GS_WORDS * (F.fr_seed_off[frag] + i) : nullptr;
    const size_t m2 = arena_mark(cx.tmp);
    const cig_t *gc; int gn; int32_t len2;
    if (gt && gt[GS_HAS] && F.jarena) { gc = F.jarena + gt[GS_OFF]; gn = gt[GS_N]; len2 = gt[GS_TLEN]; }
    else {
        if (!inside) { cx.status |= ST_REFEXIT; return false; }
        uint8_t *tb = nullptr;
        len2 = g.tlen;
        if (len2 > 0) {
            tb = (uint8_t *)arena_alloc(cx, (size_t)len2 + 16);
            if (!tb || !ref_fetch(r, g.chr, g.start0, &len2, tb)) return false;
        }
        const uint8_t *qp = r.cur_read + g.qoff;
        CigV c;
        if (!cig_alloc(cx, c, g.qlen + len2 + 8)) return false;
        ksw_global(cx, g.qlen, seq_fwd(qp), len2, seq_fwd(tb ? tb : qp), P->del_gapo, P->del_gape, P->ins_gapo, P->ins_gape, P->band_w, &c);
        gc = c.c; gn = c.n;
    }
    const bool ok = merge_cigar(r, fc, &ref_end, &re, chr, gc, gn, len2, g.qlen) &&
                    (r.cs_words += r.h_cig_n[s], merge_cigar(r, fc, &ref_end, &re, chr, r.cig + r.h_cig_off[s], r.h_cig_n[s], P->seed_len + r.h_len_dif[s], P->seed_len));
    last = s;
    arena_release(cx.tmp, m2);
    return ok;
}

HP_INL int frag_steps_block(ReadCtx &r, const FLines &F, int frag, int i, int step, int n_steps, CigV &fc, int64_t &ref_end, int &re, int &last, cig_t &top)
{
    Ctx &cx = r.cx;
    const lamsa_hp_para *P = cx.P;
    if (!F.gt || !F.jarena || fc.n < 1 || (top & 0xf) != C_M) return 0;
    const int fro = F.fr_seed_off[frag];
    const HP_G int32_t *g_seed = (const HP_G int32_t *)(F.fr_seed + fro);
    const HP_G int32_t *g_gt = (const HP_G int32_t *)(F.gt + GS_WORDS * (size_t)fro);
    const HP_G cig_t *g_ja = (const HP_G cig_t *)F.jarena, *g_cig = (const HP_G cig_t *)r.cig;
    const int nb = n_steps < 32 ? n_steps : 32, K = 2 * nb;
    const int seed_len = P->seed_len;
    const bool plus = r.h_strand[last] == 1;
    wv::Lane<int> n, wf, wl, rl, ql, cw; wv::Lane<long long> src;
    WAVE_FOR(l) {
        n[l] = 0; wf[l] = 0; wl[l] = 0; rl[l] = 0; ql[l] = 0; cw[l] = 0; src[l] = 0;
        if (l < K) {
            const int j = l >> 1, idx = i + step * j;
            const int s = g_seed[idx], prev = j == 0 ? last : g_seed[idx - step];
            if (!(l & 1)) {
                int g[GS_WORDS]; hp_load16(g_gt + GS_WORDS * (size_t)idx, g);
                if (g[GS_HAS]) {
                    GapGeo gg; gap_geo(r, plus, prev, s, gg);
                    n[l] = g[GS_N]; src[l] = (long long)(g_ja + g[GS_OFF]); rl[l] = g[GS_TLEN]; ql[l] = gg.qlen;
                } else n[l] = -1;
            } else {
                n[l] = r.h_cig_n[s]; src[l] = (long long)(g_cig + r.h_cig_off[s]); rl[l] = seed_len + r.h_len_dif[s]; ql[l] = seed_len; cw[l] = n[l];
            }
            if (n[l] > 0) { const HP_G cig_t *w = (const HP_G cig_t *)src[l]; wf[l] = w[0]; wl[l] = w[n[l] - 1]; }
        }
    }
    {
        wv::Lane<int> bad;
        WAVE_FOR(l) { bad[l] = l < K && (n[l] <= 0 || (wf[l] & 0xf) != C_M || (wl[l] & 0xf) != C_M); }
        if (wv::ballot(bad)) return 0;
    }
    wv::Lane<int> adv, S, big;
    WAVE_FOR(l) { adv[l] = l < K ? n[l] - 1 : 0; S[l] = l < K ? (wf[l] >> 4) : 0; big[l] = l < K && n[l] >= 2; }
    const int n_new = wv::reduce_sum(adv);
    if (fc.n + n_new > fc.cap) return 0;
    wv::Lane<int> base = adv;
    wv::scan_add_excl(base);
    { wv::Lane<int> h = S; wv::scan_add_excl(h); WAVE_FOR(l) { S[l] += h[l]; } }
    const unsigned long long mb = wv::ballot(big);
    wv::Lane<int> e_of;
    WAVE_FOR(l) { const unsigned long long above = l < 63 ? (mb >> (l + 1)) << (l + 1) : 0ull; e_of[l] = above ? __builtin_ctzll(above) : K - 1; }
    const wv::Lane<int> S_e = wv::gather(S, e_of);
    HP_G cig_t *out = (HP_G cig_t *)fc.c;
    const int B0 = fc.n - 1;
    const int e0 = mb ? __builtin_ctzll(mb) : K - 1;
    const cig_t top_new = top + (cig_t)(wv::bcast(S, e0) << 4);
    wv::Lane<int> adj;
    WAVE_FOR(l) {
        adj[l] = 0;
        if (l == 0) out[B0] = top_new;
        if (big[l]) {
            adj[l] = wl[l] + ((S_e[l] - S[l]) << 4);
            const HP_G cig_t *w = (const HP_G cig_t *)src[l];
            HP_G cig_t *o = out + B0 + base[l];
            for (int t = 1; t < n[l] - 1; ++t) o[t] = w[t];
            o[n[l] - 1] = adj[l];
        }
    }
    top = mb ? (cig_t)wv::bcast(adj, 63 - __builtin_clzll(mb)) : top_new;
    fc.n += n_new;
    ref_end += wv::reduce_sum(rl); re += wv::reduce_sum(ql); r.cs_words += wv::reduce_sum(cw);
    last = seed_at_after_block(g_seed, i, step, nb);
    wv::sync();
    return nb;
}

HP_NOINL bool frag_extend_multi(ReadCtx &r, const FLines &F, int frag, Rec &res)
{
    HP_STAT(27);
    Ctx &cx = r.cx;
    const lamsa_hp_para *P = cx.P;
    const int32_t *seed = F.fr_seed + F.fr_seed_off[frag];
    const int seed_n = F.fr_seed_off[frag + 1] - F.fr_seed_off[frag];
    const int strand = r.h_strand[seed[0]], chr = r.h_chr[seed[0]];
    const size_t mark = arena_mark(cx.tmp);
    CigV fc;
    int cap = 0;
    {   const HP_G int32_t *g_seed = (const HP_G int32_t *)seed;
        for (int b0 = 0; b0 < seed_n; b0 += 64) { wv::Lane<int> c; WAVE_FOR(l) { c[l] = b0 + l < seed_n ? (int)r.h_cig_n[g_seed[b0 + l]] : 0; } cap += wv::reduce_sum(c); }
        cap += seed_n * (2 * iabs(P->seed_step) + 64);
    }
    if (!cig_alloc(cx, fc, cap + 16)) return false;
    int i, rs, re, last;
    if (strand == 1) { i = seed_n - 1; last = seed[i]; rs = (sid(r, r.n_seed[last]) - 1) * P->seed_step + 1; }
    else { i = 0; last = seed[0]; rs = r.last_len + (sid(r, r.n_seed[last]) - 1) * P->seed_step + 1; }
    re = rs - 1 + P->seed_len;
    cig_pushv(cx, fc, r.cig + r.h_cig_off[last], r.h_cig_n[last]); r.cs_words += r.h_cig_n[last];
    const int64_t ref_start = r.h_pos[last];
    int64_t ref_end = r.h_pos[last] + P->seed_len - 1 + r.h_len_dif[last];
    const int step = strand == 1 ? -1 : 1;
    bool ok = true;
    i += step;
    while (i >= 0 && i < seed_n && ok) {
        const int left = step == 1 ? seed_n - i : i + 1;
        if (left >= HP_FRAG_BLOCK_MIN && fc.n > 0) {
            cig_t top = ((const HP_G cig_t *)fc.c)[fc.n - 1];
            const int took = frag_steps_block(r, F, frag, i, step, left, fc, ref_end, re, last, top);
            if (took) { HP_STAT(24); i += step * took; continue; }
        }
        const int one_by_one = left < 32 ? left : 32;
        HP_STAT(25);
        for (int t = 0; t < one_by_one && ok; ++t) { ok = frag_step(r, F, frag, i, chr, fc, ref_end, re, last); i += step; }
    }
    if (ok) ok = merge_cigar(r, res.cig, &res.refend, &res.readend, chr, fc.c, fc.n, (int)(ref_end - ref_start + 1), re - rs + 1);
    arena_release(cx.tmp, mark);
    return ok && !(cx.status & (ST_REFEXIT | ST_OVERFLOW));
}

HP_INL bool frag_extend(ReadCtx &r, const FLines &F, int frag, Rec &res)
{
    const int o0 = F.fr_seed_off[frag], o1 = F.fr_seed_off[frag + 1];
    if (o1 - o0 != 1) return frag_extend_multi(r, F, frag, res);
    const lamsa_hp_para *P = r.cx.P;
    const int s = F.fr_seed[o0];
    r.cs_words += r.h_cig_n[s];
    const bool ok = merge_cigar(r, res.cig, &res.refend, &res.readend, r.h_chr[s], r.cig + r.h_cig_off[s], r.h_cig_n[s],
                                P->seed_len + r.h_len_dif[s], P->seed_len);
    return ok && !(r.cx.status & (ST_REFEXIT | ST_OVERFLOW));
}

HP_NOINL bool split_sv(ReadCtx &r, const JGeo &g, Rec &res)
{
    HP_STAT(28);
    Ctx &cx = r.cx;
    const lamsa_hp_para *P = cx.P;
    const int hash_len = P->hash_len, s_qlen = g.s_qlen, dis = g.dis;
    const uint8_t *qp = r.cur_read + g.qoff;
    const int64_t at1_off = g.at1_off, at2_off = g.at2_off;
    const int at1_ld = g.at1_ld, at1_chr = g.at1_chr, at2_chr = g.at2_chr;
    const int gh0 = hash_len * P->match;
    const size_t mark = arena_mark(cx.tmp);
    int s_tlen = 0;
    int32_t tl;
    CigV sc;
    bool ok = true;
    if (dis > g.match_dis) {
        s_tlen = s_qlen + dis; tl = s_tlen;
        uint8_t *tb = (uint8_t *)arena_alloc(cx, (size_t)(s_tlen > 0 ? s_tlen : 0) + 16);
        ok = tb && cig_alloc(cx, sc, s_qlen + s_tlen + 64) && ref_fetch(r, at1_chr, at1_off + P->seed_len + at1_ld - 1, &tl, tb);
        if (ok) {
            s_tlen = tl;
            if (s_qlen < hash_len) { HP_STATX_ADD(64, 1); ksw_bi_extend(cx, s_qlen, seq_fwd(qp), s_tlen, seq_fwd(tb), gh0, gh0, sc); }
            else { HP_STATX_ADD(65, 1); split_indel_map(cx, sc, qp, s_qlen, tb, s_tlen, 0); }
        }
    } else {
        s_tlen = s_qlen + dis;
        if (s_tlen < 2 * P->hash_step) {
            int32_t _s_tlen = s_qlen + hash_len;
            int lqe, lte, rqe, rte;
            uint8_t *tb1 = (uint8_t *)arena_alloc(cx, (size_t)_s_tlen + 16), *tb2 = (uint8_t *)arena_alloc(cx, (size_t)_s_tlen + 16);
            CigV lc, rcg;
            ok = tb1 && tb2 && cig_alloc(cx, sc, 2 * (s_qlen + _s_tlen) + 64) && cig_alloc(cx, lc, s_qlen + _s_tlen + 8) && cig_alloc(cx, rcg, s_qlen + _s_tlen + 8);
            ok = ok && ref_fetch(r, at1_chr, at1_off + P->seed_len + at1_ld - 1, &_s_tlen, tb1);
            if (ok) {
                ksw_extend(cx, s_qlen, seq_fwd(qp), _s_tlen, seq_fwd(tb1), P->band_w, gh0, &lqe, &lte, &lc);
                ok = ref_fetch(r, at2_chr, at2_off - _s_tlen - 1, &_s_tlen, tb2);
            }
            if (ok) {
                HP_STATX_ADD(66, 1);
                const Seq rq = seq_rev(qp, s_qlen), rt = seq_rev(tb2, _s_tlen);
                ksw_extend(cx, s_qlen, rq, _s_tlen, rt, P->band_w, gh0, &rqe, &rte, &rcg);
                cig_invert(rcg.c, rcg.n);
                sw_mid_fix(cx, sc, lc.c, lc.n, rcg.c, rcg.n, s_qlen, rq, lqe, rqe, s_qlen + dis, rt, lte, rte);
            }
        } else {
            s_tlen += 2 * (hash_len - dis); tl = s_tlen;
            uint8_t *tb = (uint8_t *)arena_alloc(cx, (size_t)s_tlen + 16);
            ok = tb && cig_alloc(cx, sc, s_qlen + s_tlen + 64) && ref_fetch(r, at1_chr, at1_off + P->seed_len + at1_ld + dis - hash_len - 1, &tl, tb);
            if (ok) {
                s_tlen = tl;
                const int off_dis = (s_tlen != s_qlen - dis + 2 * hash_len) ? 0 : -dis;
                s_tlen = s_qlen + dis;
                if (s_tlen < hash_len) { HP_STATX_ADD(69, 1); ksw_bi_extend(cx, s_qlen, seq_fwd(qp), s_tlen, seq_fwd(tb + hash_len - dis), gh0, gh0, sc); }
                else { HP_STATX_ADD(off_dis ? 67 : 68, 1); split_indel_map(cx, sc, qp, s_qlen, tb + hash_len - dis, s_tlen, off_dis); }
            }
        }
    }
    if (ok) ok = merge_cigar(r, res.cig, &res.refend, &res.readend, at1_chr, sc.c, sc.n, s_tlen, s_qlen);
    arena_release(cx.tmp, mark);
    return ok && !(cx.status & (ST_REFEXIT | ST_OVERFLOW));
}

HP_NOINL bool split_mismatch(ReadCtx &r, const JGeo &g, const int32_t *jt, const int32_t *jarena, Rec &res)
{
    HP_STAT(29);
    Ctx &cx = r.cx;
    if (jt && jt[GS_HAS] && jarena) {
        return merge_cigar(r, res.cig, &res.refend, &res.readend, g.at1_chr, jarena + jt[GS_OFF], jt[GS_N], jt[GS_TLEN], g.s_qlen) && !(cx.status & (ST_REFEXIT | ST_OVERFLOW));
    }
    const size_t mark = arena_mark(cx.tmp);
    int32_t tl = g.tl;
    CigV sc;
    uint8_t *tb = (uint8_t *)arena_alloc(cx, (size_t)tl + 16);
    bool ok = tb && cig_alloc(cx, sc, g.s_qlen + tl + 64) && ref_fetch(r, g.at1_chr, g.start0, &tl, tb);
    if (ok) {
        ksw_bi_extend(cx, g.s_qlen, seq_fwd(r.cur_read + g.qoff), tl, seq_fwd(tb), 100, 100, sc);
        ok = merge_cigar(r, res.cig, &res.refend, &res.readend, g.at1_chr, sc.c, sc.n, tl, g.s_qlen);
    }
    arena_release(cx.tmp, mark);
    return ok && !(cx.status & (ST_REFEXIT | ST_OVERFLOW));
}

HP_INL bool split_mapping(ReadCtx &r, const FLines &F, int f1, int f2, Rec &res)
{
    Ctx &cx = r.cx;
    JGeo g; junction_geo(r, F, f1, f2, g);
    if (g.cls == JC_EXIT) { cx.status |= ST_REFEXIT; return false; }
    if (g.cls == JC_SV) return split_sv(r, g, res);
    if (g.cls == JC_MIS) return split_mismatch(r, g, F.jt ? F.jt + GS_WORDS * (f1 < f2 ? f1 : f2) : nullptr, F.jarena, res);
    if (g.tl <= 0) return !(cx.status & (ST_REFEXIT | ST_OVERFLOW));
    const size_t mark = arena_mark(cx.tmp);
    cig_t *w = (cig_t *)arena_alloc(cx, sizeof(cig_t));
    bool ok = w != nullptr;
    if (ok) {
        ((HP_G cig_t *)w)[0] = (g.tl << 4) | C_D;
        wv::sync();
        ok = merge_cigar(r, res.cig, &res.refend, &res.readend, g.at1_chr, w, 1, g.tl, 0);
    }
    arena_release(cx.tmp, mark);
    return ok && !(cx.status & (ST_REFEXIT | ST_OVERFLOW));
}


struct MergeSrc { const cig_t *p; int n, first, last, reflen, readlen; const HP_L int32_t *ls; bool staged; };
enum { FM_SW = 8, FM_JW = 10, FM_W = FM_SW + FM_JW };

struct MergeLoc { int n, readend; int64_t refend; };
HP_INL void mloc_out(const MergeLoc &m, Rec &res) { res.cig.n = m.n; res.refend = m.refend; res.readend = m.readend; }
HP_INL void mloc_in(MergeLoc &m, const Rec &res) { m.n = res.cig.n; m.refend = res.refend; m.readend = res.readend; }
HP_INL bool merge_fast_loc(ReadCtx &r, Rec &res, MergeLoc &m, int &tail, bool &ovf, int chr, const MergeSrc &S, HP_G cig_t *dst, int cap)
{
    if (S.n == 0) return true;
    Ctx &cx = r.cx;
    const int n1 = m.n;
    if (n1 > 1) {
        const int top = tail & 0xf, hop = S.first & 0xf;
        if ((((top == C_I || top == C_D) && (tail >> 4) <= 3) && hop != C_S && hop != C_H) ||
            (((hop == C_I || hop == C_D) && (S.first >> 4) <= 3) && top != C_S && top != C_H)) {
            mloc_out(m, res);
            wv::sync();
            bool ok;
            if (S.p) ok = merge_cigar_full(r, res.cig, &res.refend, &res.readend, chr, S.p, S.n, S.reflen, S.readlen);
            else {
                const size_t mark = arena_mark(cx.tmp);
                cig_t *w = (cig_t *)arena_alloc(cx, sizeof(cig_t));
                ok = w != nullptr;
                if (ok) { ((HP_G cig_t *)w)[0] = S.first; wv::sync(); ok = merge_cigar_full(r, res.cig, &res.refend, &res.readend, chr, w, 1, S.reflen, S.readlen); }
                arena_release(cx.tmp, mark);
            }
            wv::sync();
            mloc_in(m, res);
            tail = m.n > 0 ? (int)dst[m.n - 1] : 0;
            return ok && !(cx.status & (ST_REFEXIT | ST_OVERFLOW));
        }
    }
    int j = 0;
    if (n1 > 0) {
        if ((tail & 0xf) == (S.first & 0xf)) { tail = tail + ((S.first >> 4) << 4); dst[n1 - 1] = tail; j = 1; }
        else if (((tail & 0xf) == C_I && (S.first & 0xf) == C_S) || ((tail & 0xf) == C_S && (S.first & 0xf) == C_I)) { tail = (((tail >> 4) + (S.first >> 4)) << 4) | C_S; dst[n1 - 1] = tail; j = 1; }
    }
    const int mm = S.n - j;
    if (n1 + mm > cap) ovf = true;
    else if (mm > 0) {
        if (S.staged) { WAVE_FOR(l) { if (l < mm) dst[n1 + l] = S.ls[j + l]; } }
        else if (S.p) { const HP_G cig_t *src = (const HP_G cig_t *)S.p; for (int b0 = 0; b0 < mm; b0 += 64) { WAVE_FOR(l) { const int i = b0 + l; if (i < mm) dst[n1 + i] = src[j + i]; } } }
        else dst[n1] = S.first;
        m.n = n1 + mm; tail = S.last;
    }
    m.refend += S.reflen;
    m.readend += S.readlen;
    return !ovf;
}

HP_NOINL bool frags_merge(ReadCtx &r, const FLines &F, int f0, int nfr, int strand, Rec &res)
{
    Ctx &cx = r.cx;
    const lamsa_hp_para *P = cx.P;
    const size_t mark = arena_mark(cx.tmp);
    int32_t *pl = (int32_t *)arena_alloc(cx, sizeof(int32_t) * 16 * 64);
    if (!pl) return false;
    HP_G int32_t *g_pl = (HP_G int32_t *)pl;
    wv::sync();
    bool ok = true, ovf = false;
    long long cs_ = 0;
    MergeLoc ml; mloc_in(ml, res);
    HP_G cig_t *const res_c = (HP_G cig_t *)wv::uni64((long long)res.cig.c); const int res_cap = wv::uni(res.cig.cap);
    const cig_t *const seed_cigs = (const cig_t *)wv::uni64((long long)r.cig); const cig_t *const job_cigs = (const cig_t *)wv::uni64((long long)F.jarena);
    const int seed_len = wv::uni(P->seed_len);
    int tail = ml.n > 0 ? (int)res_c[ml.n - 1] : 0;
    HP_L int32_t *const stg = cx.lds;
    const bool stage = cx.lds_words >= 64 * FM_W;
    for (int t0 = 0; t0 < nfr && ok; t0 += 64) {
        HP_T0(tg64_);
        bool staged_ok = stage;
        const int epoch0 = cx.lds_epoch;
        wv::sync();
        WAVE_FOR(l) {
            const int t = t0 + l;
            int v[16];
            for (int k = 0; k < 16; ++k) v[k] = 0;
            if (t < nfr) {
                const int f = strand == 1 ? f0 + nfr - 1 - t : f0 + t;
                const int o0 = F.fr_seed_off[f], o1 = F.fr_seed_off[f + 1];
                v[0] = o1 - o0 == 1;
                if (v[0]) {
                    const int s = F.fr_seed[o0];
                    const int64_t co = r.h_cig_off[s]; const int cn = r.h_cig_n[s];
                    v[1] = (int)(co & 0xffffffffll); v[2] = (int)(co >> 32); v[3] = cn; v[6] = P->seed_len + r.h_len_dif[s]; v[7] = r.h_chr[s];
                    if (cn > 0) { v[4] = r.cig[co]; v[5] = r.cig[co + cn - 1]; }
                    if (stage && cn > 0 && cn <= FM_SW) {
                        int w[FM_SW];
#pragma unroll
                        for (int k = 0; k < FM_SW; ++k) w[k] = k < cn ? (int)r.cig[co + k] : 0;
#pragma unroll
                        for (int k = 0; k < FM_SW; ++k) stg[l * FM_W + k] = w[k];
                    }
                }
                if (t < nfr - 1) {
                    const int f2 = strand == 1 ? f - 1 : f + 1;
                    JGeo G; junction_geo(r, F, f, f2, G);
                    v[8] = 3; v[15] = G.at1_chr;
                    if (G.cls == JC_DEL) { v[8] = G.tl > 0 ? 1 : 0; v[10] = 1; v[11] = v[12] = (G.tl << 4) | C_D; v[13] = G.tl; v[14] = 0; }
                    else if (G.cls == JC_MIS) {
                        const int32_t *jt = F.jt ? F.jt + GS_WORDS * (f < f2 ? f : f2) : nullptr;
                        if (jt && jt[GS_HAS] && F.jarena) {
                            v[8] = 2; v[9] = jt[GS_OFF]; v[10] = jt[GS_N]; v[13] = jt[GS_TLEN]; v[14] = G.s_qlen;
                            if (jt[GS_N] > 0) { v[11] = F.jarena[jt[GS_OFF]]; v[12] = F.jarena[jt[GS_OFF] + jt[GS_N] - 1]; }
                            if (stage && jt[GS_N] > 0 && jt[GS_N] <= FM_JW) {
                                int w[FM_JW];
#pragma unroll
                                for (int k = 0; k < FM_JW; ++k) w[k] = k < jt[GS_N] ? (int)F.jarena[jt[GS_OFF] + k] : 0;
#pragma unroll
                                for (int k = 0; k < FM_JW; ++k) stg[l * FM_W + FM_SW + k] = w[k];
                            }
                        }
                    }
                }
            }
            for (int k = 0; k < 16; ++k) g_pl[k * 64 + l] = v[k];
        }
        wv::sync();
        wv::Lane<int> V[16];
        WAVE_FOR(l) { for (int k = 0; k < 16; ++k) V[k][l] = g_pl[k * 64 + l]; }
        const int cnt = nfr - t0 < 64 ? nfr - t0 : 64;
        HP_TADD_FILL(cx, 22, tg64_);
        for (int q = 0; q < cnt && ok; ++q) {
            const int t = t0 + q, f = strand == 1 ? f0 + nfr - 1 - t : f0 + t;
            if (wv::bcast(V[0], q)) {
#if defined(HP_PROF) && defined(HP_PROF_FILL)
                const long long tpa_ = wv::clock();
#endif
                MergeSrc S;
                S.p = seed_cigs + (((int64_t)wv::bcast(V[2], q) << 32) | (unsigned)wv::bcast(V[1], q)); S.n = wv::bcast(V[3], q); S.first = wv::bcast(V[4], q); S.last = wv::bcast(V[5], q);
                S.reflen = wv::bcast(V[6], q); S.readlen = seed_len;
                if (cx.lds_epoch != epoch0) staged_ok = false;
                S.ls = stg + q * FM_W; S.staged = staged_ok && S.n <= FM_SW;
                cs_ += S.n;
#if defined(HP_PROF) && defined(HP_PROF_FILL)
                const long long tpb_ = wv::clock();
#endif
                ok = merge_fast_loc(r, res, ml, tail, ovf, wv::bcast(V[7], q), S, res_c, res_cap);
#if defined(HP_PROF) && defined(HP_PROF_FILL)
                if (cx.prof) { cx.prof[13] += tpb_ - tpa_; cx.prof[11] += wv::clock() - tpb_; }
#endif
            } else {
                mloc_out(ml, res);
                wv::sync();
                HP_T0(tfm_);
                staged_ok = false;
                ok = frag_extend_multi(r, F, f, res);
                HP_TADD_FILL(cx, 20, tfm_);
                wv::sync();
                mloc_in(ml, res);
                tail = ml.n > 0 ? (int)res_c[ml.n - 1] : 0;
            }
            if (!ok || t == nfr - 1) continue;
            const int kind = wv::bcast(V[8], q);
            if (kind == 3) {
                mloc_out(ml, res);
                wv::sync();
                HP_T0(tsm_);
                staged_ok = false;
                ok = split_mapping(r, F, f, strand == 1 ? f - 1 : f + 1, res);
                HP_TADD_FILL(cx, 18, tsm_);
                wv::sync();
                mloc_in(ml, res);
                tail = ml.n > 0 ? (int)res_c[ml.n - 1] : 0;
            } else if (kind != 0) {
#if defined(HP_PROF) && defined(HP_PROF_FILL)
                const long long tpc_ = wv::clock();
#endif
                MergeSrc S;
                S.p = kind == 2 ? job_cigs + wv::bcast(V[9], q) : nullptr; S.n = wv::bcast(V[10], q); S.first = wv::bcast(V[11], q); S.last = wv::bcast(V[12], q);
                S.reflen = wv::bcast(V[13], q); S.readlen = wv::bcast(V[14], q);
                if (cx.lds_epoch != epoch0) staged_ok = false;
                S.ls = stg + q * FM_W + FM_SW; S.staged = staged_ok && kind == 2 && S.n <= FM_JW;
                ok = merge_fast_loc(r, res, ml, tail, ovf, wv::bcast(V[15], q), S, res_c, res_cap);
#if defined(HP_PROF) && defined(HP_PROF_FILL)
                if (cx.prof) cx.prof[12] += wv::clock() - tpc_;
#endif
            }
        }
    }
    mloc_out(ml, res);
    r.cs_words += cs_;
    if (ovf) cx.status |= ST_OVERFLOW;
    wv::sync();
    arena_release(cx.tmp, mark);
    return ok && !(cx.status & (ST_REFEXIT | ST_OVERFLOW));
}

HP_NOINL bool head_fix(ReadCtx &r, const FLines &F, int line, Rec &res)
{
    Ctx &cx = r.cx;
    const lamsa_hp_para *P = cx.P;
    EndGeo g;
    const int kind = end_geo(r, F, line, r.h_strand[F.fr_seed[F.fr_seed_off[F.frag_off[line]]]], true, g);
    if (kind == EG_EXIT) { cx.status |= ST_REFEXIT; return false; }
    res.offset = r.h_pos[g.s];
    if (kind == EG_NONE) { res.refend = res.offset - 1; res.cig.n = 0; return true; }
    {   const int32_t *ht = F.ht ? F.ht + ES_LINE * line : nullptr;
        if (ht && ht[ES_HAS] && F.jarena) {
            HP_STAT(20);
            res.offset -= ht[ES_REFLEN];
            res.refend = res.offset - 1;
            cig_pushv(cx, res.cig, F.jarena + ht[ES_OFF], ht[ES_N]);
            res.refend += ht[ES_REFLEN];
            res.readend += ht[ES_READLEN];
            return !(cx.status & (ST_REFEXIT | ST_OVERFLOW));
        }
    }
    const int read_len = g.read_len;
    int32_t ref_len = g.ref_len;
    const size_t mark = arena_mark(cx.tmp);
    uint8_t *tb = (uint8_t *)arena_alloc(cx, (size_t)(ref_len > 0 ? ref_len : 0) + 16);
    CigV c;
    bool ok = tb && cig_alloc(cx, c, read_len + ref_len + 16) && ref_fetch(r, g.chr, g.start0, &ref_len, tb);
    if (ok) {
        int qre, tre;
        const int rr = ksw_extend_r(cx, read_len, seq_fwd(r.cur_read + g.read_start), ref_len, seq_fwd(tb), P->band_w, P->seed_len * P->match, &qre, &tre, &c);
        if (rr != 0) cig_push1(cx, c, ((read_len - qre) << 4) | C_S);
        cig_invert(c.c, c.n);
        res.offset -= cig_reflen(c.c, c.n);
        res.refend = res.offset - 1;
        cig_pushv(cx, res.cig, c.c, c.n);
        res.refend += cig_reflen(c.c, c.n);
        res.readend += cig_readlen(c.c, c.n);
    }
    arena_release(cx.tmp, mark);
    return ok && !(cx.status & (ST_REFEXIT | ST_OVERFLOW));
}

HP_NOINL bool tail_fix(ReadCtx &r, const FLines &F, int line, Rec &res)
{
    Ctx &cx = r.cx;
    const lamsa_hp_para *P = cx.P;
    EndGeo g;
    const int kind = end_geo(r, F, line, r.h_strand[F.fr_seed[F.fr_seed_off[F.frag_off[line]]]], false, g);
    if (kind == EG_EXIT) { cx.status |= ST_REFEXIT; return false; }
    if (kind == EG_NONE) return true;
    {   const int32_t *ht = F.ht ? F.ht + ES_LINE * line + ES_WORDS : nullptr;
        if (ht && ht[ES_HAS] && F.jarena) {
            HP_STAT(21);
            return merge_cigar(r, res.cig, &res.refend, &res.readend, g.chr, F.jarena + ht[ES_OFF], ht[ES_N], ht[ES_REFLEN], ht[ES_READLEN]) && !(cx.status & (ST_REFEXIT | ST_OVERFLOW));
        }
    }
    const int read_len = g.read_len;
    int32_t ref_len = g.ref_len;
    const size_t mark = arena_mark(cx.tmp);
    uint8_t *tb = (uint8_t *)arena_alloc(cx, (size_t)ref_len + 16);
    CigV c;
    bool ok = tb && cig_alloc(cx, c, read_len + ref_len + 16) && ref_fetch(r, g.chr, g.start0, &ref_len, tb);
    if (ok) {
        int qle, tle;
        const int rr = ksw_extend_c(cx, read_len, seq_fwd(r.cur_read + g.read_start), ref_len, seq_fwd(tb), P->band_w, P->seed_len * P->match, &qle, &tle, &c);
        if (rr != 0) cig_push1(cx, c, ((read_len - qle) << 4) | C_S);
        ok = merge_cigar(r, res.cig, &res.refend, &res.readend, g.chr, c.c, c.n, cig_reflen(c.c, c.n), cig_readlen(c.c, c.n));
    }
    arena_release(cx.tmp, mark);
    return ok && !(cx.status & (ST_REFEXIT | ST_OVERFLOW));
}

HP_NOINL bool res_split(ReadCtx &r, LineRes &la, cig_t *buf, int buf_cap)
{
    Ctx &cx = r.cx;
    const lamsa_hp_para *P = cx.P;
    const int read_len = r.L, split_len = P->split_len;
    const int n = la.rec[0].cig.n;
    const HP_G cig_t *src = (const HP_G cig_t *)la.rec[0].cig.c;
    if (la.rec[0].cig.c == buf) { cx.status |= ST_REFEXIT; return false; }
    HP_G cig_t *oc = (HP_G cig_t *)buf;
    {
        bool plain = n <= buf_cap;
        for (int j0 = 0; j0 < n && plain; j0 += 64) {
            wv::Lane<int> bad;
            WAVE_FOR(l) {
                const int j = j0 + l;
                int b = 0;
                if (j < n) {
                    const int w = src[j], op = w & 0xf, len = w >> 4;
                    const int nxt = j + 1 < n ? (int)src[j + 1] : -1;
                    b = len == 0 || (op != C_M && op != C_I && op != C_D && op != C_S) || ((op == C_I || op == C_D) && len >= split_len) ||
                        (nxt >= 0 && (nxt & 0xf) == op) || (op == C_S && j > 0 && j < n - 1 && nxt >= 0 && (nxt & 0xf) == C_H);
                }
                bad[l] = b;
            }
            if (wv::ballot(bad) != 0) plain = false;
        }
        if (plain) {
            for (int j0 = 0; j0 < n; j0 += 64) { WAVE_FOR(l) { const int j = j0 + l; if (j < n) oc[j] = src[j]; } }
            cig_bind(la.rec[0].cig, buf, buf_cap); la.rec[0].cig.n = n;
            wv::sync();
            return !(cx.status & ST_OVERFLOW);
        }
    }
    int res_n = 0, used = 0;
    int wn = 0, pend = 0; bool have = false;
    int rd_tot = 0, ref_rec = 0;
#define HP_RS_PUSH(w_) do { const int v_ = (w_); if ((v_ >> 4) != 0) { \
        if (have && (pend & 0xf) == (v_ & 0xf)) pend += (v_ >> 4) << 4; \
        else { if (have) { if (used + wn < buf_cap) oc[used + wn++] = pend; else cx.status |= ST_OVERFLOW; } pend = v_; have = true; } } } while (0)
#define HP_RS_NEW_REC(extra_ref) do { \
        if (have) { if (used + wn < buf_cap) oc[used + wn++] = pend; else cx.status |= ST_OVERFLOW; have = false; } \
        cig_bind(la.rec[res_n].cig, buf + used, wn); la.rec[res_n].cig.n = wn; \
        used += wn; wn = 0; \
        if (res_n + 1 >= HP_REC_MAX) { cx.status |= ST_OVERFLOW; return false; } \
        ++res_n; ++la.cur_res_n; \
        la.rec[res_n].chr = la.rec[res_n - 1].chr; la.rec[res_n].nstrand = la.rec[res_n - 1].nstrand;         \
        la.rec[res_n].offset = la.rec[res_n - 1].offset + ref_rec + (extra_ref); ref_rec = 0; } while (0)
    bool skip = false;
    for (int j0 = 0; j0 < n; j0 += 64) {
        wv::Lane<int> W;
        WAVE_FOR(l) { const int j = j0 + l; W[l] = j < n ? src[j] : 0; }
        const int peek = j0 + 64 < n ? (int)src[j0 + 64] : 0;
        const int cnt = n - j0 < 64 ? n - j0 : 64;
        for (int jj = 0; jj < cnt; ++jj) {
            if (skip) { skip = false; continue; }
            const int j = j0 + jj;
            const int cw = wv::bcast(W, jj), nw = jj < 63 ? wv::bcast(W, jj + 1) : peek;
            const int op = cw & 0xf, len = cw >> 4;
            if (op == C_M) { HP_RS_PUSH(cw); rd_tot += len; if (len != 0) ref_rec += len; }
            else if (op == C_I && len >= split_len) {
                HP_RS_PUSH(((read_len - rd_tot) << 4) | C_S);
                HP_RS_NEW_REC(0);
                HP_RS_PUSH(((len + rd_tot) << 4) | C_S);
                rd_tot += len;
            } else if (op == C_D && len >= split_len) {
                HP_RS_PUSH(((read_len - rd_tot) << 4) | C_S);
                HP_RS_NEW_REC(len);
                HP_RS_PUSH((rd_tot << 4) | C_S);
            } else if (op == C_I) { HP_RS_PUSH(cw); rd_tot += len; }
            else if (op == C_D) { HP_RS_PUSH(cw); ref_rec += len; }
            else if (op == C_S) {
                if (j > 0 && j < n - 1 && (nw & 0xf) == C_H) {
                    const int Sn = len, Hn = nw >> 4;
                    HP_RS_PUSH(((read_len - rd_tot) << 4) | C_S);
                    HP_RS_NEW_REC(Hn);
                    HP_RS_PUSH(((rd_tot + Sn) << 4) | C_S);
                    rd_tot += Sn;
                    skip = true;
                } else { HP_RS_PUSH(cw); rd_tot += len; }
            } else if (op != C_H) { cx.status |= ST_REFEXIT; return false; }
        }
    }
    if (have) { if (used + wn < buf_cap) oc[used + wn++] = pend; else cx.status |= ST_OVERFLOW; }
    cig_bind(la.rec[res_n].cig, buf + used, buf_cap - used); la.rec[res_n].cig.n = wn;
#undef HP_RS_PUSH
#undef HP_RS_NEW_REC
    wv::sync();
    return !(cx.status & ST_OVERFLOW);
}

HP_NOINL bool res_aux(ReadCtx &r, LineRes &la)
{
    Ctx &cx = r.cx;
    const lamsa_hp_para *P = cx.P;
    HP_G int32_t *ev = (HP_G int32_t *)la.ev;
    int ev_n = 0;
    for (int m = 0; m <= la.cur_res_n; ++m) {
        Rec &rec = la.rec[m];
        const int ev0 = ev_n;
        const size_t mark = arena_mark(cx.tmp);
        int32_t ref_len = cig_reflen(rec.cig.c, rec.cig.n);
        uint8_t *ref = (uint8_t *)arena_alloc(cx, (size_t)(ref_len > 0 ? ref_len : 0) + 16);
        if (!ref || !ref_fetch(r, rec.chr, rec.offset - 1, &ref_len, ref)) { arena_release(cx.tmp, mark); return false; }
        if (la.tags & LAMSA_HP_TAG_LEFT_ALIGN) lalign_cigar(rec.cig.c, rec.cig.n, r.cur_read, r.L, ref, ref_len);
        int ref_i = 0, read_i = 0, n_mm = 0, n_m = 0, n_io = 0, n_ie = 0, n_do = 0, n_de = 0;
        bool bad = false;
        const HP_G cig_t *gc = (const HP_G cig_t *)rec.cig.c;
        const HP_G uint8_t *gread = (const HP_G uint8_t *)r.cur_read, *gref = (const HP_G uint8_t *)ref;
        const int cn = rec.cig.n;
        for (int c0 = 0; c0 < cn && !bad; c0 += 64) {
            wv::Lane<int> rinc, finc, opl, lenl, isbad;
            WAVE_FOR(l) {
                const int i = c0 + l;
                int op = -1, len = 0;
                if (i < cn) { const cig_t w = gc[i]; op = w & 0xf; len = w >> 4; }
                opl[l] = op; lenl[l] = len;
                rinc[l] = (op == C_M || op == C_I || op == C_S) ? len : 0;
                finc[l] = (op == C_M || op == C_D) ? len : 0;
                isbad[l] = i < cn && op != C_M && op != C_I && op != C_D && op != C_S;
            }
            const int r_tot = wv::reduce_sum(rinc), f_tot = wv::reduce_sum(finc);
            wv::Lane<int> rs = rinc, fs = finc;
            wv::scan_add_excl(rs); wv::scan_add_excl(fs);
            wv::Lane<int> mlen, mm, il, dl, io, dq;
            WAVE_FOR(l) {
                const int op = opl[l], len = lenl[l];
                int ml = 0;
                if (op == C_M) {
                    if (len < 0 || read_i + rs[l] + len > r.L || ref_i + fs[l] + len > ref_len) isbad[l] = 1;
                    else ml = len;
                }
                mlen[l] = ml; mm[l] = 0;
                il[l] = op == C_I ? len : 0; dl[l] = op == C_D ? len : 0; io[l] = op == C_I; dq[l] = op == C_D;
            }
            if (wv::ballot(isbad) != 0) { bad = true; break; }
            {
                wv::Lane<int> rend, delta, ism;
                WAVE_FOR(l) { rend[l] = rs[l] + rinc[l]; delta[l] = fs[l] - rs[l]; ism[l] = mlen[l] > 0; }
                enum { RA_U = 4 };
                for (int q0 = 0; q0 < r_tot; q0 += 64 * RA_U) {
                    wv::Lane<int> e[RA_U];
#pragma unroll
                    for (int u = 0; u < RA_U; ++u) { WAVE_FOR(l) { e[u][l] = 0; } }
#pragma unroll
                    for (int step = 32; step >= 1; step >>= 1) {
#pragma unroll
                        for (int u = 0; u < RA_U; ++u) {
                            wv::Lane<int> probe;
                            WAVE_FOR(l) { probe[l] = e[u][l] + step - 1; }
                            const wv::Lane<int> v = wv::gather(rend, probe);
                            WAVE_FOR(l) { if (v[l] <= q0 + 64 * u + l) e[u][l] += step; }
                        }
                    }
                    wv::Lane<int> a[RA_U], b[RA_U];
#pragma unroll
                    for (int u = 0; u < RA_U; ++u) {
                        const wv::Lane<int> dv = wv::gather(delta, e[u]), mv = wv::gather(ism, e[u]);
                        WAVE_FOR(l) { const int q = q0 + 64 * u + l; a[u][l] = 0; b[u][l] = 0; if (q < r_tot && mv[l]) { a[u][l] = gread[read_i + q]; b[u][l] = gref[ref_i + q + dv[l]] + 256; } }
                    }
#pragma unroll
                    for (int u = 0; u < RA_U; ++u) { WAVE_FOR(l) { mm[l] += b[u][l] != 0 && a[u][l] != b[u][l] - 256; } }
                    if (ev) {
#pragma unroll
                        for (int u = 0; u < RA_U; ++u) {
                            const wv::Lane<int> dv = wv::gather(delta, e[u]);
                            wv::Lane<int> f, slot;
                            WAVE_FOR(l) { f[l] = b[u][l] != 0 && a[u][l] != b[u][l] - 256; slot[l] = f[l]; }
                            const int cnt = __builtin_popcountll(wv::ballot(f));
                            if (cnt == 0) continue;
                            wv::scan_add_excl(slot);
                            WAVE_FOR(l) {
                                const int k = ev_n + slot[l];
                                if (f[l] && k < la.ev_cap) ev[k] = ((ref_i + q0 + 64 * u + l + dv[l]) << 2) | (b[u][l] - 256);
                            }
                            ev_n += cnt;
                        }
                    }
                }
            }
            const int mms = wv::reduce_sum(mm);
            n_mm += mms; n_m += wv::reduce_sum(mlen) - mms;
            n_ie += wv::reduce_sum(il); n_de += wv::reduce_sum(dl);
            n_io += __builtin_popcountll(wv::ballot(io)); n_do += __builtin_popcountll(wv::ballot(dq));
            read_i += r_tot; ref_i += f_tot;
        }
        arena_release(cx.tmp, mark);
        if (bad || read_i != r.L || ref_i != ref_len) { cx.status |= ST_REFEXIT; return false; }
        rec.NM = n_mm + n_ie + n_de;
        rec.score = n_m * P->match - n_mm * P->mis - n_io * P->ins_gapo - n_ie * P->ins_gape - n_do * P->del_gapo - n_de * P->del_gape;
        {
            const int w0 = cn > 0 ? (int)gc[0] : 0, w1 = cn > 0 ? (int)gc[cn - 1] : 0;
            const int s0 = (w0 & 0xf) == C_S ? w0 >> 4 : 0, s1 = (w1 & 0xf) == C_S ? w1 >> 4 : 0;
            rec.sum[0] = (rec.nstrand == 1 ? s0 : s1) + 1; rec.sum[1] = r.L - (rec.nstrand == 1 ? s1 : s0);
            rec.sum[2] = ref_len; rec.sum[3] = n_m + n_mm; rec.sum[4] = n_ie; rec.sum[5] = n_de; rec.sum[6] = n_io; rec.sum[7] = n_do;
        }
        if (ev) {
            if (ev_n > la.ev_cap) { cx.status |= ST_OVERFLOW; return false; }
            rec.mm = la.ev + ev0; rec.n_mm = ev_n - ev0;
        }
        if (rec.score < 0) {
            ev_n = ev0;
            for (int i = m + 1; i <= la.cur_res_n; ++i) la.rec[i - 1] = la.rec[i];
            --m; --la.cur_res_n;
        } else { la.tol_score += rec.score; la.tol_NM += rec.NM; }
    }
    if (ev) wv::sync();
    if (la.cur_res_n < 0) la.tol_score = -1;
    else la.tol_score -= la.cur_res_n * P->split_pen;
    return true;
}


#ifdef HP_PROF
#define HP_TIMED(slot, call) ([&]() { HP_T0(t_); const bool ok_ = (call); HP_TADD(r.cx, slot, t_); return ok_; }())
#else
#define HP_TIMED(slot, call) (call)
#endif
HP_NOINL bool fill_line(ReadCtx &r, const FLines &F, int line, LineRes &la, cig_t *cur_buf, int cur_cap, cig_t *rec_buf, int rec_cap)
{
    Ctx &cx = r.cx;
    const lamsa_hp_para *P = cx.P;
    const int f0 = F.frag_off[line], nfr = F.frag_off[line + 1] - f0;
    const int first_seed = F.fr_seed[F.fr_seed_off[f0]];
    const int strand = r.h_strand[first_seed];
    la.line_score = F.line_score[line]; la.cur_res_n = 0; la.tol_score = la.tol_NM = 0;
    Rec &r0 = la.rec[0];
    cig_bind(r0.cig, cur_buf, cur_cap);
// ... 25 lines not shown
```

### lamsa_amd/csrc/hp_phase.h

```cpp
#pragma once
#include "hp_align.h"
#include "hp_lanedp.h"
#include "hp_wavejob.h"

namespace hp {

struct RdMeta {
    int64_t fl_off[2];
    int32_t fl_n[2], fl_tot[2], fl_nfrag[2];
    int32_t unit_base[2];
    int32_t status;
    int32_t tbases;
    int32_t cells, pairs;
    int32_t cs_words, pad_;
};

struct UnitRec {
    int32_t read, line;
    int64_t out_off;
    int32_t out_len, n_reg;
    int32_t pad[2];
};

enum { PH_NBUCKET = 8 };

struct alignas(128) PhaseCtl {
    alignas(128) int32_t q_head[12];
    alignas(128) int32_t n_units[2];
    int32_t bucket_n[2][PH_NBUCKET];
    alignas(128) unsigned long long fl_cursor;
    alignas(128) unsigned long long line_cursor;
    alignas(128) unsigned long long job_cursor;
    alignas(128) int32_t lj_n[2]; int32_t lj_bucket_n[2][24];
    alignas(128) int32_t wj_n[2]; int32_t wj_bucket_n[2][WJ_NBUCKET];
    alignas(128) unsigned long long wj_bytes;
    alignas(128) unsigned long long wj_cells;
    alignas(128) unsigned long long t_first_inv[4], t_last[4];
};

struct LjRec;
struct PhaseArgs {
    lamsa_hp_para P;
    RefView ref;
    BatchIn in;
    BatchOut out;
    char *slab; size_t slab_per_wave;
    int32_t sort_pb, sort_cb;
    const int32_t *order;
    int32_t n_reads;
    long long *prof;
    NodeS *g_nd; int32_t *g_nseed; int32_t *g_sidx;
    RdMeta *meta;
    UnitRec *units; int32_t unit_cap;
    int32_t *bucket_q;
    int32_t *fl_base; int64_t fl_cap;
    int32_t *line_base; int64_t line_cap;
    int32_t *job_base; int64_t job_cap;
    struct LjRec *ljobs; int32_t *lj_bucket; int32_t lj_cap;
    WjRec *wjobs; int32_t *wj_bucket; int32_t wj_cap;
    size_t slab_fill, slab_wj;
    size_t slab_wjb, wjb_off; int32_t n_wjb;
    PhaseCtl *ctl;
};

HP_INL void drain_stamp(const PhaseArgs &a, int k)
{
    if (wv::leader()) { const unsigned long long now = wv::wall(); atomicMax(&a.ctl->t_first_inv[k], ~now); atomicMax(&a.ctl->t_last[k], now); }
}

HP_INL void meta_flag(const PhaseArgs &a, int rd, const ReadCtx &r)
{
    if (wv::leader()) {
        const long long tb = r.t_bases, nc = r.cx.n_cells, np = r.n_pairs, cw = r.cs_words;
        if (r.cx.status) atomicOr(&a.meta[rd].status, r.cx.status);
        if (tb > 0) atomicAdd(&a.meta[rd].tbases, (int)(tb > 0x3fffffffLL ? 0x3fffffffLL : tb));
        if (nc > 0) atomicAdd(&a.meta[rd].cells, (int)(nc > 0x3fffffffLL ? 0x3fffffffLL : nc));
        if (np > 0) atomicAdd(&a.meta[rd].pairs, (int)(np > 0x3fffffffLL ? 0x3fffffffLL : np));
        if (cw > 0) atomicAdd(&a.meta[rd].cs_words, (int)(cw > 0x3fffffffLL ? 0x3fffffffLL : cw));
    }
}

HP_FN void units_push(const PhaseArgs &a, ReadCtx &r, int rd, int round, const FLines &F, const FlStore &fs)
{
    RdMeta &M = a.meta[rd];
    int base = 0;
    if (wv::leader()) base = atomicAdd(&a.ctl->n_units[round], F.n);
    base = wv::uni(base);
    if (base + F.n > a.unit_cap) { r.cx.status |= ST_OVERFLOW; return; }
    M.fl_off[round] = fs.got_off; M.fl_n[round] = F.n; M.fl_tot[round] = fs.got_tot; M.fl_nfrag[round] = F.nfrag; M.unit_base[round] = base;
    const lamsa_hp_para *P = r.cx.P;
    const int tiles = (2 * P->band_w + 1 + 63) / 64;
    for (int j = 0; j < F.n; ++j) {
        const int f0 = F.frag_off[j], f1 = F.frag_off[j + 1];
        const int n_seed = F.fr_seed_off[f1] - F.fr_seed_off[f0];
        const int sa = r.seed_id[r.n_seed[F.fr_seed[F.fr_seed_off[f0]]]], sb = r.seed_id[r.n_seed[F.fr_seed[F.fr_seed_off[f1] - 1]]];
        const int s_lo = sa < sb ? sa : sb, s_hi = sa < sb ? sb : sa;
        long long ext = (long long)(s_lo - 1 + r.seed_all - s_hi) * P->seed_step;
        if (ext < 0) ext = 0;
        const long long cost = ext * tiles * 8 + (long long)n_seed * 64;
        int b = 0;
        for (long long c = cost >> 10; c > 0 && b < PH_NBUCKET - 1; c >>= 1) ++b;
        const int bucket = PH_NBUCKET - 1 - b;
        UnitRec &U = a.units[(size_t)round * a.unit_cap + base + j];
        U.read = rd; U.line = j; U.out_off = 0; U.out_len = 0; U.n_reg = 0;
        int at = 0;
        if (wv::leader()) at = atomicAdd(&a.ctl->bucket_n[round][bucket], 1);
        at = wv::uni(at);
        a.bucket_q[((size_t)round * PH_NBUCKET + bucket) * a.unit_cap + at] = base + j;
    }
}

HP_INL void pers_bind(ReadCtx &r, const PhaseArgs &a, int rd)
{
    const int64_t pb = r.hb + rd;
    r.nd = a.g_nd + pb; r.n_seed = a.g_nseed + pb;
    r.srt = a.g_sidx + 2 * pb; r.rnk = a.g_sidx + 2 * pb + (r.H + 1);
}

#ifdef HP_PROF
#define PH_T0() const long long ph_t0_ = wv::clock()
#define PH_TADD(k) do { if (r.prof) r.prof[k] += wv::clock() - ph_t0_; } while (0)
#define PH_TMID(k, v) do { if (r.prof) { const long long now_ = wv::clock(); r.prof[k] += now_ - v; v = now_; } } while (0)
#else
#define PH_T0() do { } while (0)
#define PH_TADD(k) do { } while (0)
#define PH_TMID(k, v) do { } while (0)
#endif

enum { PH_CTX_BYTES = 512 };
static_assert(sizeof(ReadCtx) <= PH_CTX_BYTES, "the read context must fit its per-wave block");
constexpr bool ph_ctx_in_lds(int words, int waves_per_simd)
{
    return 4 * waves_per_simd * (((size_t)words * 4 + PH_CTX_BYTES + 511) / 512 * 512) <= 160 * 1024;
}
static_assert(PH_CTX_BYTES % 512 == 0, "the LDS block of a wave is sized in units of 512 bytes");
static_assert(28 * (4 * HP_LDS_WORDS + PH_CTX_BYTES) <= 160 * 1024, "DP rows + read context of 7 waves per SIMD must fit the CU's LDS");
struct ChainOut { FLines F; FlStore fs; };

HP_NOINL void phase_chain1(const PhaseArgs &a, int rd, int wave_slot, HP_L int32_t *lds, int lds_words, ReadCtx &r)
{
#ifdef HP_PROF
    long long ph_t_ = wv::clock();
#endif
    if (a.in.read_skip && a.in.read_skip[rd]) { if (wv::leader()) atomicOr(&a.meta[rd].status, ST_UNSUPPORTED); return; }
    read_bind(r, a.P, a.ref, a.in, rd, a.slab + (size_t)wave_slot * a.slab_per_wave + PH_CTX_BYTES, a.slab_per_wave - PH_CTX_BYTES, lds, a.prof, lds_words);
    pers_bind(r, a, rd);
    Ctx &cx = r.cx;
    const int H = r.H, c = H + 1;
    ChainOut *co = (ChainOut *)arena_alloc(cx, sizeof(ChainOut));
    int32_t *nm = (int32_t *)arena_alloc(cx, sizeof(int32_t) * 10 * (size_t)c);
    const size_t sort_mark = arena_mark(cx.tmp);
    uint64_t *sort_work = (uint64_t *)arena_alloc(cx, sizeof(uint64_t) * (size_t)c);
    if (co && nm && sort_work) {
        int32_t *sidx = a.g_sidx + 2 * (r.hb + rd);
        { HP_T0(t_sort_);
        sort_read_hits(r.h_pos, r.h_chr, r.h_strand, H, sidx, sidx + c, sort_work, (HP_L uint64_t *)lds, lds_words / 2, a.sort_pb, a.sort_cb);
        HP_TADD(cx, 46, t_sort_); }
        arena_release(cx.tmp, sort_mark);
        aux_bind(r, nm);
        nodes_fill(r);
        PH_TMID(0, ph_t_);
        FLines &F = co->F;
        FlStore &fs = co->fs; fs.base = a.fl_base; fs.cap = a.fl_cap; fs.cursor = &a.ctl->fl_cursor; fs.got_off = 0; fs.got_tot = 0;
#if defined(HP_CHAIN_STOP) && HP_CHAIN_STOP == 0
        const bool ok1 = true; F.n = 0; F.nfrag = 0;
#else
        const bool ok1 = chain_first(r, F, &fs);
#endif
        PH_TMID(1, ph_t_);
        if (ok1 && F.n > 0) units_push(a, r, rd, 0, F, fs);
        else if (!ok1 && !(cx.status & (ST_REFEXIT | ST_OVERFLOW))) cx.status |= ST_OVERFLOW;
    }
    meta_flag(a, rd, r);
}

#ifdef HP_PH_CTX_SHARED
HP_INL ReadCtx &ph_frame_ctx()
{
    alignas(16) static thread_local unsigned char blk[PH_CTX_BYTES];
    static thread_local bool born = false;
    if (!born) { for (int i = 0; i < PH_CTX_BYTES; ++i) blk[i] = 0xa5; born = true; }
    return *reinterpret_cast<ReadCtx *>(blk);
}
#define PH_FRAME_CTX(r) ReadCtx &r = ph_frame_ctx()
#else
#define PH_FRAME_CTX(r) ReadCtx r##_frame_; ReadCtx &r = r##_frame_
#endif
HP_FN void phase_chain1(const PhaseArgs &a, int rd, int wave_slot, HP_L int32_t *lds, int lds_words = HP_CHAIN_LDS_WORDS)
{
    PH_FRAME_CTX(r);
    phase_chain1(a, rd, wave_slot, lds, lds_words, r);
}

struct FillLoc { FLines F; OutBuf o; Regs G; };

HP_NOINL void phase_fill(const PhaseArgs &a, int round, int u, int wave_slot, HP_L int32_t *lds, ReadCtx &r)
{
    UnitRec &U = a.units[(size_t)round * a.unit_cap + u];
    const int rd = U.read, line = U.line;
    RdMeta &M = a.meta[rd];
    if (*(volatile int32_t *)&M.status & ST_DEAD) return;
    PH_T0();
    read_bind(r, a.P, a.ref, a.in, rd, a.slab + (size_t)wave_slot * a.slab_fill, a.slab_fill, lds, a.prof, HP_LDS_WORDS);
    pers_bind(r, a, rd);
    Ctx &cx = r.cx;
    FillLoc *fl = (FillLoc *)arena_alloc(cx, sizeof(FillLoc));
    if (!fl) { meta_flag(a, rd, r); return; }
    FLines &F = fl->F;
    F.n = M.fl_n[round]; F.nfrag = M.fl_nfrag[round];
    flines_bind(F, a.fl_base + M.fl_off[round], F.n, M.fl_tot[round]);
    F.jarena = a.job_base;
    const int tags = fill_tags(a.in.tags);
    OutBuf &o = fl->o; o.n = 0; o.cap = line_out_cap(r.L, tags);
    o.w = (int32_t *)arena_alloc(cx, sizeof(int32_t) * (size_t)o.cap);
    r.rc_read = (uint8_t *)arena_alloc(cx, (size_t)r.L + 16);
    const LineBufs b = line_bufs(cx, r.L, 1, tags);
    LineRes *la = b.la;
    int n_reg = 0;
    if (o.w && r.rc_read && la) {
        const bool ok = fill_line(r, F, line, *la, b.cur_buf, b.cur_cap, b.rec_buf, b.rec_cap);
        if (!ok && !(cx.status & (ST_REFEXIT | ST_OVERFLOW))) cx.status |= ST_OVERFLOW;
        if (ok) {
            out_line(cx, o, *la);
            if (round == 0 && la->tol_score >= 0) {
                Regs &G = fl->G; G.n = 0; G.m = 0;
                const size_t mark = arena_mark(cx.tmp);
                G.beg = (int32_t *)arena_alloc(cx, sizeof(int32_t) * 2 * HP_REC_MAX); G.end = G.beg ? G.beg + HP_REC_MAX : nullptr;
                G.rb = (RegB *)arena_alloc(cx, sizeof(RegB) * 2 * HP_REC_MAX); G.re = G.rb ? G.rb + HP_REC_MAX : nullptr;
                if (G.beg && G.rb) {
                    for (int k = 0; k <= la->cur_res_n; ++k) regs_push(r, G, HP_REC_MAX, la->rec[k]);
                    for (int k = 0; k < G.n; ++k) out_reg(cx, o, G, k);
                    n_reg = G.n;
                }
                arena_release(cx.tmp, mark);
            }
        }
    }
    if (!(cx.status & (ST_REFEXIT | ST_OVERFLOW))) {
        unsigned long long off = 0;
        if (wv::leader()) off = atomicAdd(&a.ctl->line_cursor, (unsigned long long)o.n);
        off = (unsigned long long)wv::uni64((long long)off);
        if ((int64_t)(off + (unsigned long long)o.n) <= a.line_cap) {
            wv::sync();
            out_copy((HP_G int32_t *)(a.line_base + off), (const HP_G int32_t *)o.w, o.n);
            U.out_off = (int64_t)off; U.out_len = o.n; U.n_reg = n_reg;
        } else cx.status |= ST_OVERFLOW;
    }
    PH_TADD(round == 0 ? 2 : 4);
    meta_flag(a, rd, r);
}

HP_FN void phase_fill(const PhaseArgs &a, int round, int u, int wave_slot, HP_L int32_t *lds)
{
    PH_FRAME_CTX(r);
    phase_fill(a, round, u, wave_slot, lds, r);
}

struct LjRec { int64_t qaddr, tk, slot; int32_t rd; uint16_t tlen; uint8_t qlen; int8_t type_comp; };
enum { LJ_NCLS = HP_LJ_QSMALL / 16, LJ_NBUCKET = 2 * LJ_NCLS };
HP_INL int lj_bucket_of(int type, int qlen)
{
    const int cls = (qlen > 0 ? qlen - 1 : 0) >> 4;
    return (type == 1 ? 0 : LJ_NCLS) + (LJ_NCLS - 1 - cls);
}

HP_NOINL void phase_filllist(const PhaseArgs &a, int round, int u, int wave_slot, HP_L int32_t *lds, ReadCtx &r)
{
    UnitRec &U = a.units[(size_t)round * a.unit_cap + u];
    const int rd = U.read, line = U.line;
    RdMeta &M = a.meta[rd];
    if (*(volatile int32_t *)&M.status & ST_DEAD) return;
    read_bind(r, a.P, a.ref, a.in, rd, a.slab + (size_t)wave_slot * a.slab_fill, a.slab_fill, lds, a.prof, 0);
    pers_bind(r, a, rd);
    const lamsa_hp_para *P = r.cx.P;
    const bool lane_ok = lj_params_ok(P) && a.lj_cap > 0, wave_ok = a.wj_cap > 0;
    if (!lane_ok && !wave_ok) return;
    FLines F;
    F.n = M.fl_n[round]; F.nfrag = M.fl_nfrag[round];
    flines_bind(F, a.fl_base + M.fl_off[round], F.n, M.fl_tot[round]);
    const int f0 = F.frag_off[line], nfr = F.frag_off[line + 1] - f0;
    const int p0 = F.fr_seed_off[f0], np = F.fr_seed_off[f0 + nfr] - p0;
    const int strand = r.h_strand[F.fr_seed[p0]];
    const int n_junc = (nfr - 1) + np, n_cand = n_junc + 2;
    r.flip = strand != 1;
    const int64_t rbase = a.in.read_off[rd];
    long long tb = 0;
    int32_t *frag_of = (int32_t *)arena_alloc(r.cx, sizeof(int32_t) * (size_t)(np + 1));
    if (!frag_of) { r.flip = false; return; }
    {
        HP_G int32_t *g_fo = (HP_G int32_t *)frag_of;
        const HP_G int32_t *g_so = (const HP_G int32_t *)F.fr_seed_off;
        for (int b0 = 0; b0 < nfr; b0 += 64) { WAVE_FOR(l) { const int f = f0 + b0 + l; if (b0 + l < nfr) { for (int q = g_so[f]; q < g_so[f + 1]; ++q) g_fo[q - p0] = f; } } }
        wv::sync();
    }
    long long *cand = (long long *)arena_alloc(r.cx, sizeof(long long) * 4 * (size_t)(n_cand + 64));
    if (!cand) { r.flip = false; return; }
    int n_lb[LJ_NBUCKET], n_wb[WJ_NBUCKET];
#pragma unroll
    for (int b = 0; b < LJ_NBUCKET; ++b) n_lb[b] = 0;
#pragma unroll
    for (int b = 0; b < WJ_NBUCKET; ++b) n_wb[b] = 0;
    for (int c0 = 0; c0 < n_cand; c0 += 64) {
        wv::Lane<int> ty, qo, ql, tl, qrev; wv::Lane<long long> tk, sl;
        WAVE_FOR(l) {
            const int c = c0 + l;
            int type = 0, qoff = 0, qlen = 0, tlen = 0, rev = 0; long long k0 = 0, slot = 0;
            if (c < nfr - 1) {
                const int jf = f0 + c;
                JGeo G; junction_geo(r, F, strand == 1 ? jf + 1 : jf, strand == 1 ? jf : jf + 1, G);
                if (G.cls == JC_MIS) { type = 1; qoff = G.qoff; qlen = G.s_qlen; tlen = G.tl; slot = (F.jt + GS_WORDS * jf) - a.fl_base; k0 = r.ref.seq_off[G.at1_chr - 1] + G.start0; }
            } else if (c < n_junc) {
                const int p = p0 + (c - (nfr - 1));
                const int lo = ((const HP_G int32_t *)frag_of)[p - p0];
                const int fb = F.fr_seed_off[lo], seed_n = F.fr_seed_off[lo + 1] - fb;
                const int ip = p - fb + (strand == 1 ? 1 : -1);
                GapGeo G;
                if (seed_n > 1 && ip >= 0 && ip < seed_n && gap_geo(r, strand == 1, F.fr_seed[fb + ip], F.fr_seed[p], G)) {
                    type = 2; qoff = G.qoff; qlen = G.qlen; tlen = G.tlen; slot = (F.gt + GS_WORDS * p) - a.fl_base; k0 = r.ref.seq_off[G.chr - 1] + G.start0;
                }
            } else if (c < n_cand && wave_ok) {
                const bool head = c == n_junc;
                EndGeo G;
                if (end_geo(r, F, line, strand, head, G) == EG_JOB && G.read_len > 0 && G.ref_len > 0 && G.read_start >= 0 && G.read_start + G.read_len <= r.L) {
                    type = head ? 3 : 4; qlen = G.read_len; tlen = G.ref_len; slot = (F.ht + ES_LINE * line + (head ? 0 : ES_WORDS)) - a.fl_base;
                    qoff = head ? G.read_start + G.read_len - 1 : G.read_start; rev = head;
                    k0 = r.ref.seq_off[G.chr - 1] + G.start0 + (head ? G.ref_len - 1 : 0);
                }
            }
            const bool small = type != 0 && type <= 2 && qlen <= HP_LJ_QSMALL && tlen <= HP_LJ_TSMALL;
            if (type != 0 && !(small ? lane_ok : wave_ok)) type = 0;
            if (type != 0 && !small) type |= 16;
            ty[l] = type; qo[l] = qoff; ql[l] = qlen; tl[l] = tlen; sl[l] = slot; tk[l] = k0; qrev[l] = rev;
        }
        WAVE_FOR(l) {
            const int c = c0 + l;
            if (c < n_cand) { HP_G int32_t *cw = (HP_G int32_t *)cand + 8 * (size_t)c; cw[0] = ty[l]; cw[1] = qo[l]; cw[2] = ql[l]; cw[3] = tl[l] | (qrev[l] << 30); *(HP_G long long *)(cw + 4) = tk[l]; *(HP_G long long *)(cw + 6) = sl[l]; }
        }
#pragma unroll
        for (int b = 0; b < LJ_NBUCKET; ++b) { wv::Lane<int> inb; WAVE_FOR(l) inb[l] = ty[l] != 0 && !(ty[l] & 16) && lj_bucket_of(ty[l], ql[l]) == b; n_lb[b] += __builtin_popcountll(wv::ballot(inb)); }
        { wv::Lane<int> wb; WAVE_FOR(l) wb[l] = (ty[l] & 16) ? wj_bucket_of(P, ty[l] & 15, ql[l], tl[l], wj_need(P, ty[l] & 15, ql[l], tl[l]) > (long long)a.slab_wj) : -1;
#pragma unroll
          for (int b = 0; b < WJ_NBUCKET; ++b) { wv::Lane<int> inb; WAVE_FOR(l) inb[l] = wb[l] == b; n_wb[b] += __builtin_popcountll(wv::ballot(inb)); } }
    }
    int n_l = 0, n_w = 0;
#pragma unroll
    for (int b = 0; b < LJ_NBUCKET; ++b) n_l += n_lb[b];
#pragma unroll
    for (int b = 0; b < WJ_NBUCKET; ++b) n_w += n_wb[b];
    if (n_l + n_w > 0) {
        wv::Lane<int> got;
        WAVE_FOR(l) {
            int v = 0, add = 0; int32_t *ctr = nullptr;
#pragma unroll
            for (int b = 0; b < LJ_NBUCKET; ++b) if (l == b) { add = n_lb[b]; ctr = &a.ctl->lj_bucket_n[round][b]; }
#pragma unroll
            for (int b = 0; b < WJ_NBUCKET; ++b) if (l == LJ_NBUCKET + b) { add = n_wb[b]; ctr = &a.ctl->wj_bucket_n[round][b]; }
            if (l == LJ_NBUCKET + WJ_NBUCKET) { add = n_l; ctr = &a.ctl->lj_n[round]; }
            if (l == LJ_NBUCKET + WJ_NBUCKET + 1) { add = n_w; ctr = &a.ctl->wj_n[round]; }
            if (ctr && add > 0) v = atomicAdd(ctr, add);
            got[l] = v;
        }
        int base_l = wv::bcast(got, LJ_NBUCKET + WJ_NBUCKET), base_w = wv::bcast(got, LJ_NBUCKET + WJ_NBUCKET + 1);
        bool ok_l = n_l > 0 && base_l + n_l <= a.lj_cap, ok_w = n_w > 0 && base_w + n_w <= a.wj_cap;
        int pos_lb[LJ_NBUCKET], pos_wb[WJ_NBUCKET];
#pragma unroll
        for (int b = 0; b < LJ_NBUCKET; ++b) { pos_lb[b] = wv::bcast(got, b); if (n_lb[b] > 0 && pos_lb[b] + n_lb[b] > a.lj_cap) ok_l = false; }
#pragma unroll
        for (int b = 0; b < WJ_NBUCKET; ++b) { pos_wb[b] = wv::bcast(got, LJ_NBUCKET + b); if (n_wb[b] > 0 && pos_wb[b] + n_wb[b] > a.wj_cap) ok_w = false; }
#pragma unroll
        for (int b = 0; b < LJ_NBUCKET; ++b) if (!ok_l && n_lb[b] > 0) { for (int k0 = 0; k0 < n_lb[b]; k0 += 64) { WAVE_FOR(l) { const int k = pos_lb[b] + k0 + l; if (k0 + l < n_lb[b] && k < a.lj_cap) a.lj_bucket[(size_t)b * a.lj_cap + k] = -1; } } }
#pragma unroll
        for (int b = 0; b < WJ_NBUCKET; ++b) if (!ok_w && n_wb[b] > 0) { for (int k0 = 0; k0 < n_wb[b]; k0 += 64) { WAVE_FOR(l) { const int k = pos_wb[b] + k0 + l; if (k0 + l < n_wb[b] && k < a.wj_cap) a.wj_bucket[(size_t)b * a.wj_cap + k] = -1; } } }
        wv::sync();
        for (int c0 = 0; c0 < n_cand && (ok_l || ok_w); c0 += 64) {
            wv::Lane<int> ty, qo, ql, tl, qrev; wv::Lane<long long> tk, sl;
            WAVE_FOR(l) {
                const int c = c0 + l;
                ty[l] = 0; qo[l] = 0; ql[l] = 0; tl[l] = 0; qrev[l] = 0; tk[l] = 0; sl[l] = 0;
                if (c < n_cand) { const HP_G int32_t *cw = (const HP_G int32_t *)cand + 8 * (size_t)c; ty[l] = cw[0]; qo[l] = cw[1]; ql[l] = cw[2]; tl[l] = cw[3] & 0x3fffffff; qrev[l] = (cw[3] >> 30) & 1; tk[l] = *(const HP_G long long *)(cw + 4); sl[l] = *(const HP_G long long *)(cw + 6); }
            }
            wv::Lane<int> has, big, tbl;
            WAVE_FOR(l) { has[l] = ok_l && ty[l] != 0 && !(ty[l] & 16); big[l] = ok_w && (ty[l] & 16) != 0; tbl[l] = (has[l] || big[l]) ? tl[l] : 0; }
            const unsigned long long m = wv::ballot(has), mw = wv::ballot(big);
            if (m) {
                wv::Lane<int> at;
                WAVE_FOR(l) {
                    at[l] = base_l + __builtin_popcountll(m & ((1ull << l) - 1));
                    if (has[l]) {
                        LjRec &J = a.ljobs[at[l]];
                        J.qaddr = strand == 1 ? rbase + qo[l] : rbase + (r.L - 1 - qo[l]);
                        J.tk = tk[l]; J.slot = sl[l]; J.rd = rd; J.qlen = (uint8_t)ql[l]; J.tlen = (uint16_t)tl[l]; J.type_comp = (int8_t)(ty[l] | (strand == 1 ? 0 : 16));
                    }
                }
                base_l += __builtin_popcountll(m);
#pragma unroll
                for (int b = 0; b < LJ_NBUCKET; ++b) {
                    wv::Lane<int> inb;
                    WAVE_FOR(l) inb[l] = has[l] && lj_bucket_of(ty[l], ql[l]) == b;
                    const unsigned long long mb = wv::ballot(inb);
                    if (!mb) continue;
                    WAVE_FOR(l) { if (inb[l]) a.lj_bucket[(size_t)b * a.lj_cap + pos_lb[b] + __builtin_popcountll(mb & ((1ull << l) - 1))] = at[l]; }
                    pos_lb[b] += __builtin_popcountll(mb);
                }
            }
            if (mw) {
                wv::Lane<int> at, bk;
                WAVE_FOR(l) {
                    at[l] = base_w + __builtin_popcountll(mw & ((1ull << l) - 1)); bk[l] = -1;
                    if (big[l]) {
                        const int type = ty[l] & 15;
                        WjRec &J = a.wjobs[at[l]];
                        const int back = qrev[l] ? 1 : 0, comp = strand == 1 ? 0 : 1;
                        J.qaddr = strand == 1 ? rbase + qo[l] : rbase + (r.L - 1 - qo[l]);
                        J.tk = tk[l]; J.slot = sl[l]; J.rd = rd; J.qlen = ql[l]; J.tlen = tl[l];
                        J.type_comp = type | (comp << 4) | ((back ^ comp) << 5) | (back << 6);
                        bk[l] = wj_bucket_of(P, type, ql[l], tl[l], wj_need(P, type, ql[l], tl[l]) > (long long)a.slab_wj);
                    }
                }
                base_w += __builtin_popcountll(mw);
#pragma unroll
                for (int b = 0; b < WJ_NBUCKET; ++b) {
                    wv::Lane<int> inb;
                    WAVE_FOR(l) inb[l] = bk[l] == b;
                    const unsigned long long mb = wv::ballot(inb);
                    if (!mb) continue;
                    WAVE_FOR(l) { if (inb[l]) a.wj_bucket[(size_t)b * a.wj_cap + pos_wb[b] + __builtin_popcountll(mb & ((1ull << l) - 1))] = at[l]; }
                    pos_wb[b] += __builtin_popcountll(mb);
                }
            }
            tb += wv::reduce_sum(tbl);
        }
    }
    r.flip = false;
    r.t_bases = tb;
    meta_flag(a, rd, r);
}

HP_FN void phase_filllist(const PhaseArgs &a, int round, int u, int wave_slot, HP_L int32_t *lds)
{
    PH_FRAME_CTX(r);
    phase_filllist(a, round, u, wave_slot, lds, r);
}

HP_INL int lj_queue_n(const PhaseArgs &a, int round, int b) { const int n = a.ctl->lj_bucket_n[round][b]; return n < a.lj_cap ? n : a.lj_cap; }
HP_INL int wj_queue_n(const PhaseArgs &a, int round, int b) { const int n = a.ctl->wj_bucket_n[round][b]; return n < a.wj_cap ? n : a.wj_cap; }

HP_INL void phase_filldp(const PhaseArgs &a, int round, int bucket, int off, int wave_slot, HP_L int32_t *lds, int qcap)
{
    const lamsa_hp_para *P = &a.P;
    const int n_in = lj_queue_n(a, round, bucket);
    const int cnt = n_in - off < 64 ? n_in - off : 64;
    char *slab = a.slab + (size_t)wave_slot * a.slab_fill;
    cig_t *cbuf = (cig_t *)slab;
    uint8_t *zbuf = (uint8_t *)(slab + sizeof(cig_t) * 3 * HP_LJ_CIG * 64);
    if (sizeof(cig_t) * 3 * HP_LJ_CIG * 64 + (size_t)qcap * HP_LJ_TSMALL * 64 + 64 > a.slab_fill) return;
    const int32_t *bq = a.lj_bucket + (size_t)bucket * a.lj_cap + off;
    wv::Lane<int> nw, rdl, cel; wv::Lane<long long> slotl;
    wv::sync();
    WAVE_FOR(l) {
        nw[l] = 0; rdl[l] = -1; cel[l] = 0; slotl[l] = 0;
        if (l < cnt && bq[l] >= 0) {
            const LjRec R = a.ljobs[bq[l]];
            LaneJob J;
            const int comp = (R.type_comp >> 4) & 1, type = R.type_comp & 15;
            J.q = (const HP_G uint8_t *)(a.in.read_seq + R.qaddr); J.qs = comp ? -1 : 1; J.qcomp = comp; J.qlen = R.qlen; J.pac = (const HP_G uint8_t *)a.ref.pac; J.tk = R.tk; J.ts = 1; J.tlen = R.tlen;
            J.z = (HP_G uint8_t *)zbuf; J.zl = l; J.zs = qcap; J.cells = 0; J.row = lds + l; J.qrow = (HP_L uint8_t *)(lds + (qcap + 2) * 64) + l; J.rev = 0;
            lj_stage_query(J);
            LCig out, Lc, Rc;
            out.c = cbuf + (size_t)l * 3 * HP_LJ_CIG; out.n = 0; Lc.c = out.c + HP_LJ_CIG; Lc.n = 0; Rc.c = Lc.c + HP_LJ_CIG; Rc.n = 0;
            if (type == 1) lj_bi_extend(P, J, 100, 100, Lc, Rc, out);
            else lj_global(P, J, P->del_gapo, P->del_gape, P->ins_gapo, P->ins_gape, P->band_w, &out);
            nw[l] = out.n; rdl[l] = R.rd; cel[l] = (int)J.cells; slotl[l] = R.slot | ((long long)R.tlen << 48);
        }
    }
    wv::Lane<int> pre = nw;
    wv::scan_add_excl(pre);
    const int total = wv::reduce_sum(nw);
    unsigned long long base = 0;
    if (wv::leader()) base = atomicAdd(&a.ctl->job_cursor, (unsigned long long)total);
    base = (unsigned long long)wv::uni64((long long)base);
    if ((int64_t)(base + (unsigned long long)total) > a.job_cap) return;
    WAVE_FOR(l) {
        if (l < cnt && bq[l] >= 0) {
            const cig_t *src = cbuf + (size_t)l * 3 * HP_LJ_CIG;
            int32_t *dst = a.job_base + base + pre[l];
            for (int k = 0; k < nw[l]; ++k) dst[k] = src[k];
            int32_t *slot = a.fl_base + (slotl[l] & 0xffffffffffffll);
            slot[GS_OFF] = (int32_t)(base + pre[l]); slot[GS_N] = nw[l]; slot[GS_TLEN] = (int32_t)(slotl[l] >> 48); slot[GS_HAS] = 1;
            if (cel[l] > 0) atomicAdd(&a.meta[rdl[l]].cells, cel[l]);
        }
    }
    wv::sync();
}

#ifdef HP_WJ_NOINL
HP_NOINL
#else
HP_INL
#endif
void phase_wavejob(const PhaseArgs &a, int round, int g, bool big, int wave_slot, HP_L int32_t *lds)
{
    const int b1 = big ? WJ_NBIG : WJ_NBUCKET;
    int b = big ? 0 : WJ_NBIG;
    for (; b < b1 - 1; ++b) { const int nb = wj_queue_n(a, round, b); if (g < nb) break; g -= nb; }
    const int ji = wv::uni(a.wj_bucket[(size_t)b * a.wj_cap + g]);
    if (ji < 0) return;
    const WjRec R = a.wjobs[ji];
    const int rd = wv::uni(R.rd), type = wv::uni(R.type_comp) & 15, comp = (wv::uni(R.type_comp) >> 4) & 1;
// ... 128 lines not shown
```

Measured before the change: 4.313.

## Precompute seed-junction boundary repairs in a new lane-parallel kernel ahead of fill

Adds a k_fillrepair kernel, launched before the fill pass in each round. It lists the junctions where a short I/D next to a seed boundary would otherwise force a serial merge_cigar_full repair inside frags_merge, solves each one with a per-lane banded DP, and writes the repaired CIGAR pieces into the job arena with a slot pointer. frags_merge then applies a matching precomputed repair verbatim through repair_apply and falls back to the old path when the record is missing or no longer matches. This moves serial repair work off the critical fill path into a parallel kernel. The cost is an extra launch, extra arena space and more DP cells spent on candidates that may never be used.

```diff
diff --git a/lamsa_amd/csrc/hp_align.h b/lamsa_amd/csrc/hp_align.h
--- a/lamsa_amd/csrc/hp_align.h
+++ b/lamsa_amd/csrc/hp_align.h
@@ -72,7 +72,11 @@
 
 HP_INL void read_bind(ReadCtx &r, const lamsa_hp_para &P, const RefView &ref, const BatchIn &in, int rd, char *slab, size_t slab_bytes, HP_L int32_t *lds, long long *prof, int lds_words = HP_BOTH_LDS_WORDS)
 {
-    r.cx.P = &P; r.cx.status = 0; r.cx.n_cells = 0; r.cx.lds_epoch = 0; r.cx.prof_dp = nullptr; r.n_pairs = 0; r.cx.lds = lds; r.cx.lds_words = lds_words; r.cx.prof = prof ? prof + (size_t)rd * 64 : nullptr;
+    r.cx.P = &P; r.cx.status = 0; r.cx.n_cells = 0; r.cx.lds_epoch = 0; r.cx.prof_dp = nullptr;
+#ifdef HP_PROF
+    r.cx.prof_rp = nullptr;
+#endif
+    r.n_pairs = 0; r.cx.lds = lds; r.cx.lds_words = lds_words; r.cx.prof = prof ? prof + (size_t)rd * 64 : nullptr;
     arena_init(r.cx.tmp, slab, slab_bytes);
     r.ref = ref;
     r.L = (int)(in.read_off[rd + 1] - in.read_off[rd]);
diff --git a/lamsa_amd/csrc/hp_align_api.hip b/lamsa_amd/csrc/hp_align_api.hip
--- a/lamsa_amd/csrc/hp_align_api.hip
+++ b/lamsa_amd/csrc/hp_align_api.hip
@@ -7,6 +7,7 @@
 #include <string.h>
 #include <time.h>
 #include "hp_phase.h"
+#include "hp_repair.h"
 #include "hp_handle.h"
 #include "hp_hostprep.h"
 
@@ -135,6 +136,25 @@
         phase_filldp(a, round, b, g * 64, blockIdx.x, (HP_L int32_t *)lds, HP_LJ_QSMALL);
     }
 }
+__global__ __launch_bounds__(64, 4) void k_fillrepair(const PhaseArgs *ap, int round)
+{
+    const PhaseArgs &a = *ap;
+    __shared__ alignas(16) int32_t lds[HP_RP_LDS_WORDS + PH_CTX_BYTES / 4];
+    ReadCtx &r = *(ReadCtx *)(lds + HP_RP_LDS_WORDS);
+    int n = 0;
+    for (int b = 0; b < PH_NBUCKET; ++b) n += a.ctl->bucket_n[round][b];
+    n = wv::uni(n);
+    for (;;) {
+        int g = 0;
+        if (wv::leader()) g = atomicAdd(&a.ctl->q_head[9], 1);
+        g = wv::uni(g);
+        if (g >= n) break;
+        int b = 0;
+        while (b < PH_NBUCKET - 1 && g >= a.ctl->bucket_n[round][b]) { g -= a.ctl->bucket_n[round][b]; ++b; }
+        const int u = wv::uni(a.bucket_q[((size_t)round * PH_NBUCKET + b) * a.unit_cap + g]);
+        phase_fillrepair(a, round, u, blockIdx.x, (HP_L int32_t *)lds, r);
+    }
+}
 __global__ __launch_bounds__(64, HP_WJ_WAVES_PER_SIMD) void k_filldp_wave(const PhaseArgs *ap, int round)
 {
     __shared__ int32_t lds[HP_WJ_LDS_WORDS];
@@ -219,6 +239,7 @@
 static const bool g_noshare = getenv("LAMSA_HP_FULL_GRIDS") != nullptr;
 static const bool g_nowave = getenv("LAMSA_HP_NO_WAVE_JOBS") != nullptr;
 static const bool g_nolane = getenv("LAMSA_HP_NO_LANE_DP") != nullptr;
+static const bool g_norepair = getenv("LAMSA_HP_NO_REPAIR_AHEAD") != nullptr;
 static const bool g_mono = getenv("LAMSA_HP_ONE_KERNEL") != nullptr;
 
 struct HostBuf {
@@ -491,6 +512,9 @@
             fprintf(stderr, "[HP_PROF] wave jobs, junctions of the class 'band 2 sets fixed': %lld jobs, wj_run %lld Mcyc of which staging %lld; ksw_bi_extend %lld Mcyc of which after the left extension %lld; "
                             "in ksw_extend_band<2>: setup and first fill %lld, rows %lld, backtrack %lld Mcyc\n",
                     sd[51], sd[50] / 1000000, sd[49] / 1000000, sd[47] / 1000000, sd[48] / 1000000, sd[44] / 1000000, sd[45] / 1000000, sd[46] / 1000000);
+            fprintf(stderr, "[HP_PROF] boundary repairs: met %lld, from a record %lld; fallbacks: no record %lld, other element on top %lld, other ends %lld, more elements looked at than left verbatim %lld, no room %lld | "
+                            "lister: records %lld; not listed: walk reaches the first element of piece p-1 %lld, S or H %lld, window outside read or contig %lld, caps / empty CIGAR / arena full %lld\n",
+                    sd[52], sd[53], sd[54], sd[55], sd[56], sd[57], sd[58], sd[59], sd[60], sd[61], sd[62], sd[63]);
         }
         for (int q = 0; q < 8 && q < n; ++q) { int r = idx[q]; fprintf(stderr, "[HP_PROF] read %d L=%d:", r, T.h_len[r]); for (int k = 0; k < 11; ++k) fprintf(stderr, " %lld", pr[(size_t)r * 64 + k] / 1000000); fprintf(stderr, " | o_l %lld H %lld | targets %lld trips %lld init_Mcyc %lld\n", pr[(size_t)r * 64 + 14], pr[(size_t)r * 64 + 15], pr[(size_t)r * 64 + 11], pr[(size_t)r * 64 + 12], pr[(size_t)r * 64 + 13] / 1000000); }
     }
@@ -517,7 +541,7 @@
     return Y;
 }
 
-struct SlabPlan { size_t chain, fill, wj, wjb, wjb_off; int w_chain, w_fill, w_dp, w_wj, n_wjb, shape; size_t bytes; };
+struct SlabPlan { size_t chain, fill, wj, wjb, wjb_off; int w_chain, w_fill, w_dp, w_wj, w_rp, n_wjb, shape; size_t bytes; };
 static int chain_shape(const lamsa_hp_para &P, int64_t n_reads, int64_t n_bases)
 {
     static const int force = getenv("LAMSA_HP_CHAIN_SHAPE") ? atoi(getenv("LAMSA_HP_CHAIN_SHAPE")) : -1;
@@ -540,11 +564,12 @@
     if (Q.wjb < Q.wj) Q.wjb = Q.wj;
     if (g_nowave) Q.fill = std::max(Q.fill, al256(read_slab_bytes(P.band_w, max_L, max_H, 1, h->result_tags)));
     if (h->scratch_limit) { const size_t lim = al256(h->scratch_limit); Q.chain = std::min(Q.chain, lim); Q.fill = std::min(Q.fill, lim); Q.wj = std::min(Q.wj, lim); Q.wjb = std::min(Q.wjb, lim); }
-    int pc = 0, pf = 0, pd = 0, pw = 0;
+    int pc = 0, pf = 0, pd = 0, pw = 0, pr = 0;
     if (hipOccupancyMaxActiveBlocksPerMultiprocessor(&pc, g_chain_shapes[shape].k1, 64, 0) != hipSuccess || pc < 1) pc = 4 * g_chain_shapes[shape].waves_per_simd;
     if (hipOccupancyMaxActiveBlocksPerMultiprocessor(&pf, k_fill, 64, 0) != hipSuccess || pf < 1) pf = 4;
     if (hipOccupancyMaxActiveBlocksPerMultiprocessor(&pd, k_filldp_small, 64, 0) != hipSuccess || pd < 1) pd = 4;
     if (hipOccupancyMaxActiveBlocksPerMultiprocessor(&pw, k_filldp_wave, 64, 0) != hipSuccess || pw < 1) pw = 4;
+    if (hipOccupancyMaxActiveBlocksPerMultiprocessor(&pr, k_fillrepair, 64, 0) != hipSuccess || pr < 1) pr = 4;
     if (shared && !g_noshare) { pc = std::min(pc, 8); pf = std::min(pf, 16); pw = std::min(pw, 16); }
     { static const int cf = getenv("LAMSA_HP_FILL_PER_CU") ? atoi(getenv("LAMSA_HP_FILL_PER_CU")) : 0, cc = getenv("LAMSA_HP_CHAIN_PER_CU") ? atoi(getenv("LAMSA_HP_CHAIN_PER_CU")) : 0,
                        cw = getenv("LAMSA_HP_WJ_PER_CU") ? atoi(getenv("LAMSA_HP_WJ_PER_CU")) : 0;
@@ -552,7 +577,7 @@
       if (cc > 0 && cc < pc) pc = cc;
       if (cw > 0 && cw < pw) pw = cw; }
     Q.w_chain = cap_waves(h->n_cu * pc, Q.chain, h->n_cu); Q.w_fill = cap_waves(h->n_cu * pf, Q.fill, h->n_cu);
-    Q.w_dp = std::min(h->n_cu * pd, Q.w_fill); Q.w_wj = cap_waves(h->n_cu * pw, Q.wj, h->n_cu);
+    Q.w_dp = std::min(h->n_cu * pd, Q.w_fill); Q.w_rp = std::min(h->n_cu * pr, Q.w_fill); Q.w_wj = cap_waves(h->n_cu * pw, Q.wj, h->n_cu);
     { const size_t budget_big = (size_t)12 << 30; size_t nb = budget_big / Q.wjb; if (nb < 1) nb = 1; Q.n_wjb = (int)std::min<size_t>(nb, (size_t)Q.w_wj); }
     Q.wjb_off = al256(Q.wj * (size_t)Q.w_wj);
     const size_t wj_bytes = Q.wjb_off + Q.wjb * (size_t)Q.n_wjb;
@@ -608,6 +633,7 @@
         if (!g_nowave) hipLaunchKernelGGL(k_filldp_wave, dim3(w_wj), dim3(64), 0, s, da, 0);
         HIPCHK(h, hipEventRecord(Ln.ep[6], s), LAMSA_HP_EKERNEL);
         if (!g_nolane) hipLaunchKernelGGL(k_filldp_small, dim3(w_dp), dim3(64), 0, s, da, 0);
+        if (!g_norepair) hipLaunchKernelGGL(k_fillrepair, dim3(Q.w_rp), dim3(64), 0, s, da, 0);
     } else { HIPCHK(h, hipEventRecord(Ln.ep[5], s), LAMSA_HP_EKERNEL); HIPCHK(h, hipEventRecord(Ln.ep[6], s), LAMSA_HP_EKERNEL); }
     HIPCHK(h, hipEventRecord(Ln.ep[4], s), LAMSA_HP_EKERNEL);
     hipLaunchKernelGGL(k_fill, dim3(w_fill), dim3(64), 0, s, da, 0);
@@ -615,10 +641,11 @@
     hipLaunchKernelGGL(g_chain_shapes[Q.shape].k2, dim3(std::min(w_chain, n)), dim3(64), 0, s, da);
     HIPCHK(h, hipEventRecord(Ln.ep[2], s), LAMSA_HP_EKERNEL);
     if (list) {
-        HIPCHK(h, hipMemsetAsync(&((PhaseCtl *)(d + o_ctl))->q_head[5], 0, 16, s), LAMSA_HP_EKERNEL);
+        HIPCHK(h, hipMemsetAsync(&((PhaseCtl *)(d + o_ctl))->q_head[5], 0, 20, s), LAMSA_HP_EKERNEL);
         hipLaunchKernelGGL(k_filllist, dim3(w_fill), dim3(64), 0, s, da, 1);
         if (!g_nowave) hipLaunchKernelGGL(k_filldp_wave, dim3(w_wj), dim3(64), 0, s, da, 1);
         if (!g_nolane) hipLaunchKernelGGL(k_filldp_small, dim3(w_dp), dim3(64), 0, s, da, 1);
+        if (!g_norepair) hipLaunchKernelGGL(k_fillrepair, dim3(Q.w_rp), dim3(64), 0, s, da, 1);
     }
     hipLaunchKernelGGL(k_fill, dim3(w_fill), dim3(64), 0, s, da, 1);
     HIPCHK(h, hipEventRecord(Ln.ep[3], s), LAMSA_HP_EKERNEL);
diff --git a/lamsa_amd/csrc/hp_core.h b/lamsa_amd/csrc/hp_core.h
--- a/lamsa_amd/csrc/hp_core.h
+++ b/lamsa_amd/csrc/hp_core.h
@@ -40,6 +40,9 @@
     long long n_cells;
     long long *prof;
     long long *prof_dp = nullptr;
+#ifdef HP_PROF
+    long long *prof_rp;
+#endif
     int lds_epoch;
 };
 #if defined(HP_PROF_EDGE) && (defined(HP_PROF_TRACK) || defined(HP_PROF_FILL))
@@ -60,6 +63,11 @@
 #define HP_TADD(cx, slot, v) do { } while (0)
 #endif
 
+#ifdef HP_PROF
+#define HP_RP_COUNT(cx, k, n) do { if ((cx).prof_rp && wv::leader()) atomicAdd((unsigned long long *)&(cx).prof_rp[((k) <= 108 ? (k) : 108) - 45], (unsigned long long)(n)); } while (0)
+#else
+#define HP_RP_COUNT(cx, k, n) HP_STATX_ADD(k, n)
+#endif
 #ifndef HP_DPLOG
 #define HP_DPLOG(kind, qlen, tlen, w, cells) do { } while (0)
 #endif
@@ -73,7 +81,7 @@
 #define HP_STAT_MAX(i, v) ((void)0)
 #endif
 #ifdef HP_STAT_SLOTS
-static_assert(HP_STAT_SLOTS >= 97, "the array of the path counters ends before the last slot the device sources use");
+static_assert(HP_STAT_SLOTS >= 111, "the array of the path counters ends before the last slot the device sources use");
 #define HP_STATX_ADD(i, n) HP_STAT_ADD(i, n)
 #define HP_STATX_MAX(i, v) HP_STAT_MAX(i, v)
 #else
diff --git a/lamsa_amd/csrc/hp_fill.h b/lamsa_amd/csrc/hp_fill.h
--- a/lamsa_amd/csrc/hp_fill.h
+++ b/lamsa_amd/csrc/hp_fill.h
@@ -573,9 +573,57 @@
 enum { FM_SW = 8, FM_JW = 10, FM_W = FM_SW + FM_JW };
 
 struct MergeLoc { int n, readend; int64_t refend; };
+
+enum { RP_TAIL, RP_READEND, RP_REFEND_LO, RP_REFEND_HI, RP_NEED, RP_POP, RP_E1, RP_CI, RP_E2, RP_BDN, RP_TB, RP_CELLS, RP_HDR, RP_BD_MAX = 64 - RP_HDR };
+struct MergeSrc;
+HP_INL int rp_push_merge(int last, int w, int &j)
+{
+    j = 0;
+    if ((last & 0xf) == (w & 0xf)) { j = 1; return last + ((w >> 4) << 4); }
+    if (((last & 0xf) == C_I && (w & 0xf) == C_S) || ((last & 0xf) == C_S && (w & 0xf) == C_I)) { j = 1; return (((last >> 4) + (w >> 4)) << 4) | C_S; }
+    return last;
+}
 HP_INL void mloc_out(const MergeLoc &m, Rec &res) { res.cig.n = m.n; res.refend = m.refend; res.readend = m.readend; }
 HP_INL void mloc_in(MergeLoc &m, const Rec &res) { m.n = res.cig.n; m.refend = res.refend; m.readend = res.readend; }
-HP_INL bool merge_fast_loc(ReadCtx &r, Rec &res, MergeLoc &m, int &tail, bool &ovf, int chr, const MergeSrc &S, HP_G cig_t *dst, int cap)
+HP_NOINL hp_v4i repair_apply(ReadCtx &r_, int n1, int readend, int64_t refend, int tail, int verb, const cig_t *sp, int sn, int slast, cig_t *dst_, int cap, const int32_t *rec_)
+{
+    ReadCtx &r = *(ReadCtx *)wv::uni64((long long)&r_);
+    HP_G cig_t *const dst = (HP_G cig_t *)wv::uni64((long long)dst_);
+    const HP_G int32_t *const rec = (const HP_G int32_t *)wv::uni64((long long)rec_);
+    const HP_G cig_t *const src0 = (const HP_G cig_t *)wv::uni64((long long)sp);
+    n1 = wv::uni(n1); readend = wv::uni(readend); refend = wv::uni64(refend); tail = wv::uni(tail); verb = wv::uni(verb); sn = wv::uni(sn); slast = wv::uni(slast); cap = wv::uni(cap);
+    hp_v4i out; out.x = 0; out.y = 0; out.z = 0; out.w = 0;
+    wv::Lane<int> W;
+    WAVE_FOR(l) { W[l] = rec[l]; }
+    if (wv::bcast(W, RP_TAIL) != tail) { HP_RP_COUNT(r.cx, 100, 1); return out; }
+    if (wv::bcast(W, RP_READEND) != readend || (((int64_t)wv::bcast(W, RP_REFEND_HI) << 32) | (unsigned)wv::bcast(W, RP_REFEND_LO)) != refend) { HP_RP_COUNT(r.cx, 101, 1); return out; }
+    if (wv::bcast(W, RP_NEED) > verb) { HP_RP_COUNT(r.cx, 102, 1); return out; }
+    const int bdn = wv::bcast(W, RP_BDN), ci = wv::bcast(W, RP_CI), e2 = wv::bcast(W, RP_E2), rest = sn - ci;
+    int vn = n1 - wv::bcast(W, RP_POP);
+    if (vn < 1 || vn + bdn + rest > cap) { HP_RP_COUNT(r.cx, 103, 1); return out; }
+    int j;
+    int last = rp_push_merge(wv::bcast(W, RP_E1), wv::bcast(W, RP_HDR), j);
+    dst[vn - 1] = last;
+    WAVE_FOR(l) { const int k = l - RP_HDR - j; if (k >= 0 && k < bdn - j) dst[vn + k] = W[l]; }
+    if (bdn - j > 0) last = wv::bcast(W, RP_HDR + bdn - 1);
+    vn += bdn - j;
+    if (rest > 0) {
+        last = rp_push_merge(last, e2, j);
+        if (j) dst[vn - 1] = last;
+        const int mm = rest - j;
+        if (mm > 0) {
+            if (src0) { const HP_G cig_t *src = src0 + ci; for (int b0 = 0; b0 < mm; b0 += 64) { WAVE_FOR(l) { const int i = b0 + l; if (i < mm) dst[vn + i] = j + i == 0 ? e2 : (int)src[j + i]; } } }
+            else dst[vn] = e2;
+            last = rest == 1 ? e2 : slast;
+            vn += mm;
+        }
+    }
+    r.t_bases += wv::bcast(W, RP_TB); r.cx.n_cells += wv::bcast(W, RP_CELLS);
+    HP_RP_COUNT(r.cx, 98, 1);
+    out.x = 1; out.y = vn; out.z = last; out.w = rest > 0 ? rest - 1 : 0;
+    return out;
+}
+HP_INL bool merge_fast_loc(ReadCtx &r, Rec &res, MergeLoc &m, int &tail, int chr, const MergeSrc &S, HP_G cig_t *dst, int cap, int &verb, const HP_G int32_t *rp_slot, const cig_t *recs)
 {
     if (S.n == 0) return true;
     Ctx &cx = r.cx;
@@ -584,6 +632,16 @@
         const int top = tail & 0xf, hop = S.first & 0xf;
         if ((((top == C_I || top == C_D) && (tail >> 4) <= 3) && hop != C_S && hop != C_H) ||
             (((hop == C_I || hop == C_D) && (S.first >> 4) <= 3) && top != C_S && top != C_H)) {
+            HP_RP_COUNT(cx, 97, 1);
+            {
+                const int ro = wv::uni(*rp_slot);
+                if (ro > 0) {
+                    const hp_v4i q = repair_apply(r, n1, m.readend, m.refend, tail, verb, S.p, S.n, S.last, (cig_t *)dst, cap, (const int32_t *)recs + (ro - 1));
+                    if (q.x) { m.n = q.y; tail = q.z; verb = q.w; m.refend += S.reflen; m.readend += S.readlen; return !(cx.status & (ST_REFEXIT | ST_OVERFLOW)); }
+                }
+                else HP_RP_COUNT(cx, 99, 1);
+            }
+            verb = 0;
             mloc_out(m, res);
             wv::sync();
             bool ok;
@@ -607,7 +665,8 @@
         else if (((tail & 0xf) == C_I && (S.first & 0xf) == C_S) || ((tail & 0xf) == C_S && (S.first & 0xf) == C_I)) { tail = (((tail >> 4) + (S.first >> 4)) << 4) | C_S; dst[n1 - 1] = tail; j = 1; }
     }
     const int mm = S.n - j;
-    if (n1 + mm > cap) ovf = true;
+    verb = mm > 0 ? mm : 0;
+    if (n1 + mm > cap) verb = -1;
     else if (mm > 0) {
         if (S.staged) { WAVE_FOR(l) { if (l < mm) dst[n1 + l] = S.ls[j + l]; } }
         else if (S.p) { const HP_G cig_t *src = (const HP_G cig_t *)S.p; for (int b0 = 0; b0 < mm; b0 += 64) { WAVE_FOR(l) { const int i = b0 + l; if (i < mm) dst[n1 + i] = src[j + i]; } } }
@@ -616,7 +675,7 @@
     }
     m.refend += S.reflen;
     m.readend += S.readlen;
-    return !ovf;
+    return verb >= 0;
 }
 
 HP_NOINL bool frags_merge(ReadCtx &r, const FLines &F, int f0, int nfr, int strand, Rec &res)
@@ -624,17 +683,18 @@
     Ctx &cx = r.cx;
     const lamsa_hp_para *P = cx.P;
     const size_t mark = arena_mark(cx.tmp);
-    int32_t *pl = (int32_t *)arena_alloc(cx, sizeof(int32_t) * 16 * 64);
+    int32_t *pl = (int32_t *)arena_alloc(cx, sizeof(int32_t) * 18 * 64);
     if (!pl) return false;
     HP_G int32_t *g_pl = (HP_G int32_t *)pl;
     wv::sync();
-    bool ok = true, ovf = false;
+    bool ok = true;
     long long cs_ = 0;
     MergeLoc ml; mloc_in(ml, res);
     HP_G cig_t *const res_c = (HP_G cig_t *)wv::uni64((long long)res.cig.c); const int res_cap = wv::uni(res.cig.cap);
     const cig_t *const seed_cigs = (const cig_t *)wv::uni64((long long)r.cig); const cig_t *const job_cigs = (const cig_t *)wv::uni64((long long)F.jarena);
     const int seed_len = wv::uni(P->seed_len);
     int tail = ml.n > 0 ? (int)res_c[ml.n - 1] : 0;
+    int verb = 0;
     HP_L int32_t *const stg = cx.lds;
     const bool stage = cx.lds_words >= 64 * FM_W;
     for (int t0 = 0; t0 < nfr && ok; t0 += 64) {
@@ -646,12 +706,14 @@
             const int t = t0 + l;
             int v[16];
             for (int k = 0; k < 16; ++k) v[k] = 0;
+            int rp_a = 0, rp_b = 0;
             if (t < nfr) {
                 const int f = strand == 1 ? f0 + nfr - 1 - t : f0 + t;
                 const int o0 = F.fr_seed_off[f], o1 = F.fr_seed_off[f + 1];
                 v[0] = o1 - o0 == 1;
                 if (v[0]) {
                     const int s = F.fr_seed[o0];
+                    if (F.gt && F.jarena) { const int32_t *gs = F.gt + GS_WORDS * (size_t)o0; rp_a = gs[GS_OFF]; rp_b = gs[GS_N]; }
                     const int64_t co = r.h_cig_off[s]; const int cn = r.h_cig_n[s];
                     v[1] = (int)(co & 0xffffffffll); v[2] = (int)(co >> 32); v[3] = cn; v[6] = P->seed_len + r.h_len_dif[s]; v[7] = r.h_chr[s];
                     if (cn > 0) { v[4] = r.cig[co]; v[5] = r.cig[co + cn - 1]; }
@@ -685,6 +747,7 @@
                 }
             }
             for (int k = 0; k < 16; ++k) g_pl[k * 64 + l] = v[k];
+            g_pl[16 * 64 + l] = rp_a; g_pl[17 * 64 + l] = rp_b;
         }
         wv::sync();
         wv::Lane<int> V[16];
@@ -706,7 +769,7 @@
 #if defined(HP_PROF) && defined(HP_PROF_FILL)
                 const long long tpb_ = wv::clock();
 #endif
-                ok = merge_fast_loc(r, res, ml, tail, ovf, wv::bcast(V[7], q), S, res_c, res_cap);
+                ok = merge_fast_loc(r, res, ml, tail, wv::bcast(V[7], q), S, res_c, res_cap, verb, g_pl + 16 * 64 + q, job_cigs);
 #if defined(HP_PROF) && defined(HP_PROF_FILL)
                 if (cx.prof) { cx.prof[13] += tpb_ - tpa_; cx.prof[11] += wv::clock() - tpb_; }
 #endif
@@ -715,6 +778,7 @@
                 wv::sync();
                 HP_T0(tfm_);
                 staged_ok = false;
+                verb = 0;
                 ok = frag_extend_multi(r, F, f, res);
                 HP_TADD_FILL(cx, 20, tfm_);
                 wv::sync();
@@ -728,6 +792,7 @@
                 wv::sync();
                 HP_T0(tsm_);
                 staged_ok = false;
+                verb = 0;
                 ok = split_mapping(r, F, f, strand == 1 ? f - 1 : f + 1, res);
                 HP_TADD_FILL(cx, 18, tsm_);
                 wv::sync();
@@ -742,7 +807,7 @@
                 S.reflen = wv::bcast(V[13], q); S.readlen = wv::bcast(V[14], q);
                 if (cx.lds_epoch != epoch0) staged_ok = false;
                 S.ls = stg + q * FM_W + FM_SW; S.staged = staged_ok && kind == 2 && S.n <= FM_JW;
-                ok = merge_fast_loc(r, res, ml, tail, ovf, wv::bcast(V[15], q), S, res_c, res_cap);
+                ok = merge_fast_loc(r, res, ml, tail, wv::bcast(V[15], q), S, res_c, res_cap, verb, g_pl + 17 * 64 + q, job_cigs);
 #if defined(HP_PROF) && defined(HP_PROF_FILL)
                 if (cx.prof) cx.prof[12] += wv::clock() - tpc_;
 #endif
@@ -751,7 +816,7 @@
     }
     mloc_out(ml, res);
     r.cs_words += cs_;
-    if (ovf) cx.status |= ST_OVERFLOW;
+    if (verb < 0) cx.status |= ST_OVERFLOW;
     wv::sync();
     arena_release(cx.tmp, mark);
     return ok && !(cx.status & (ST_REFEXIT | ST_OVERFLOW));
diff --git a/lamsa_amd/csrc/hp_phase.h b/lamsa_amd/csrc/hp_phase.h
--- a/lamsa_amd/csrc/hp_phase.h
+++ b/lamsa_amd/csrc/hp_phase.h
@@ -204,6 +204,9 @@
     read_bind(r, a.P, a.ref, a.in, rd, a.slab + (size_t)wave_slot * a.slab_fill, a.slab_fill, lds, a.prof, HP_LDS_WORDS);
     pers_bind(r, a, rd);
     Ctx &cx = r.cx;
+#ifdef HP_PROF
+    cx.prof_rp = a.prof ? a.prof + ((size_t)a.n_reads + 1 + rd) * 64 : nullptr;
+#endif
     FillLoc *fl = (FillLoc *)arena_alloc(cx, sizeof(FillLoc));
     if (!fl) { meta_flag(a, rd, r); return; }
     FLines &F = fl->F;
diff --git a/lamsa_amd/csrc/hp_repair.h b/lamsa_amd/csrc/hp_repair.h
--- /dev/null
+++ b/lamsa_amd/csrc/hp_repair.h
@@ -0,0 +1,279 @@
+#pragma once
+#include "hp_phase.h"
+
+namespace hp {
+
+#define HP_RP_QCAP 26
+#define HP_RP_TCAP 32
+#define HP_RP_CIG (RP_HDR + HP_RP_QCAP + HP_RP_TCAP + 8)
+#define HP_RP_LDS_WORDS HP_LJ_LDS_WORDS(HP_RP_QCAP)
+static_assert(HP_RP_QCAP <= HP_LJ_QCAP && HP_RP_TCAP <= HP_LJ_TCAP, "lj_params_ok vouches for 16-bit cells up to the lane DP's caps");
+
+struct RpCand { long long c1, c2, refend0; int32_t n1, n2, first2, readend0, chr, slot; };
+struct RpOut { int tail, need, pop, e1, ci, e2, tb; int len2, len1, band, rounds; };
+#ifndef HP_RPLOG
+#define HP_RPLOG(why, len2, len1, band, rounds, need, n1) do { } while (0)
+#endif
+enum { RP_CAND_WORDS = 12 };
+HP_INL int32_t rp_cand_word(const RpCand &C, int k)
+{
+    switch (k) {
+    case 0: return (int32_t)(C.c1 & 0xffffffffll); case 1: return (int32_t)(C.c1 >> 32); case 2: return (int32_t)(C.c2 & 0xffffffffll); case 3: return (int32_t)(C.c2 >> 32);
+    case 4: return (int32_t)(C.refend0 & 0xffffffffll); case 5: return (int32_t)(C.refend0 >> 32); case 6: return C.n1; case 7: return C.n2; case 8: return C.first2;
+    case 9: return C.readend0; case 10: return C.chr; default: return C.slot;
+    }
+}
+HP_INL void rp_cand_load(const HP_G int32_t *w, RpCand &C)
+{
+    C.c1 = ((long long)w[1] << 32) | (unsigned)w[0]; C.c2 = ((long long)w[3] << 32) | (unsigned)w[2]; C.refend0 = ((long long)w[5] << 32) | (unsigned)w[4];
+    C.n1 = w[6]; C.n2 = w[7]; C.first2 = w[8]; C.readend0 = w[9]; C.chr = w[10]; C.slot = w[11];
+}
+
+HP_INL bool rp_junction_test(int t, int h)
+{
+    const int top = t & 0xf, hop = h & 0xf;
+    return (((top == C_I || top == C_D) && (t >> 4) <= 3) && hop != C_S && hop != C_H) ||
+           (((hop == C_I || hop == C_D) && (h >> 4) <= 3) && top != C_S && top != C_H);
+}
+
+HP_INL int rp_lane_job(const lamsa_hp_para *P, const RefView &ref, const HP_G uint8_t *read, int L, bool plus, const RpCand &C, LaneJob &J, LCig &bd, RpOut &o)
+{
+    const HP_G cig_t *g1 = (const HP_G cig_t *)C.c1, *g2 = (const HP_G cig_t *)C.c2;
+    const int n2 = C.n2, md = 5;
+    if (C.n1 < 2) return 105;
+    int k1 = C.n1, ci = 0;
+    int e1 = (int)g1[k1 - 1], e2 = n2 > 0 ? (g2 ? (int)g2[0] : C.first2) : 0;
+    int len1, len11, len2, len21 = 0, len22 = 0, len_dif1 = 0, len_dif2 = 0, b = 0, left = 1, right = 1, need = 0;
+    int64_t ref_start = 0; int read_start = 0;
+    o.tail = e1; o.tb = 0; o.len2 = o.len1 = o.band = o.rounds = o.need = 0;
+    J.cells = 0;
+    for (;;) {
+        if (left) {
+            for (;;) {
+                const int op = e1 & 0xf, l = e1 >> 4;
+                if (C.n1 - k1 + 1 > need) need = C.n1 - k1 + 1;
+                if (op == C_M && l > md) { e1 -= md << 4; len21 += md; break; }
+                else if (op == C_M) len21 += l;
+                else if (op == C_I) { len21 += l; len_dif1 -= l; b += l; }
+                else if (op == C_D) { len_dif1 += l; b += l; }
+                else return 106;
+                if (--k1 < 2) return 105;
+                e1 = (int)g1[k1 - 1];
+            }
+            len11 = len21 + len_dif1;
+            read_start = C.readend0 - len21 + 1;
+            ref_start = C.refend0 - len11 + 1;
+        }
+        if (right) {
+            while (ci < n2) {
+                const int op = e2 & 0xf, l = e2 >> 4;
+                if (op == C_M && l > md) { e2 -= md << 4; len22 += md; break; }
+                else if (op == C_M) len22 += l;
+                else if (op == C_I) { len22 += l; len_dif2 -= l; b += l; }
+                else if (op == C_D) { len_dif2 += l; b += l; }
+                else return 106;
+                ++ci;
+                e2 = ci < n2 ? (int)g2[ci] : 0;
+            }
+        }
+        len2 = len21 + len22; len1 = len2 + len_dif1 + len_dif2;
+        { const int min_b = iabs(len_dif1 + len_dif2) + md; b = b > min_b ? b : min_b; }
+        o.len2 = len2; o.len1 = len1; o.band = b; o.rounds += 1; o.need = need;
+        if (len2 < 1 || len1 < 1 || len2 > HP_RP_QCAP || len1 > HP_RP_TCAP) return 108;
+        if (read_start < 1 || read_start - 1 + len2 > L) return 107;
+        const int64_t start0 = ref_start - 1;
+        if (start0 < 0 || start0 + len1 > ref.seq_len[C.chr - 1]) return 107;
+        o.tb += len1;
+        {
+            const int x0 = read_start - 1;
+            J.q = read + (plus ? x0 : L - 1 - x0); J.qs = plus ? 1 : -1; J.qcomp = plus ? 0 : 1; J.qlen = len2;
+            J.tk = ref.seq_off[C.chr - 1] + start0; J.ts = 1; J.tlen = len1; J.rev = 0;
+        }
+        lj_stage_query(J);
+        bd.n = 0;
+        lj_global(P, J, P->del_gapo, P->del_gape, P->ins_gapo, P->ins_gape, b, &bd);
+        if (bd.n == 0) return 109;
+        bool stop = false;
+        if ((bd.c[0] & 0xf) == C_M) left = 0;
+        if ((bd.c[bd.n - 1] & 0xf) == C_M) right = 0;
+        else if (ci == n2) stop = true;
+        if (stop || left + right == 0) break;
+    }
+    if (bd.n > RP_BD_MAX) return 108;
+    o.need = need; o.pop = C.n1 - k1; o.e1 = e1; o.ci = ci; o.e2 = e2;
+    return 0;
+}
+
+struct RpStep {
+    int single, s_n, s_first, s_last, s_reflen, s_chr, s_slot; long long s_ptr;
+    int rend; int64_t fend;
+    int jk, j_n, j_first, j_last, j_reflen, j_readlen, j_chr; long long j_ptr;
+};
+HP_INL void rp_seed_piece(const ReadCtx &r, const FLines &F, const int32_t *fl_base, int strand, int f, bool ends, RpStep &D)
+{
+    const lamsa_hp_para *P = r.cx.P;
+    const int o0 = F.fr_seed_off[f], o1 = F.fr_seed_off[f + 1];
+    D.single = o1 - o0 == 1; D.s_n = 0; D.s_first = D.s_last = 0; D.s_reflen = 0; D.s_chr = 0; D.s_ptr = 0; D.s_slot = 0; D.rend = 0; D.fend = 0;
+    D.jk = 3; D.j_n = 0; D.j_first = D.j_last = 0; D.j_reflen = D.j_readlen = 0; D.j_chr = 0; D.j_ptr = 0;
+    if (D.single) {
+        const int s = F.fr_seed[o0];
+        const int64_t co = r.h_cig_off[s];
+        D.s_n = r.h_cig_n[s]; D.s_ptr = (long long)(r.cig + co); D.s_reflen = P->seed_len + r.h_len_dif[s]; D.s_chr = r.h_chr[s];
+        if (D.s_n > 0) { D.s_first = r.cig[co]; D.s_last = r.cig[co + D.s_n - 1]; }
+        D.s_slot = (int)((F.gt + GS_WORDS * (size_t)o0) - fl_base);
+        if (ends) {
+            D.rend = (strand == 1 ? 0 : r.last_len) + (sid(r, r.n_seed[s]) - 1) * P->seed_step + P->seed_len;
+            D.fend = r.h_pos[s] + P->seed_len - 1 + r.h_len_dif[s];
+        }
+    }
+}
+HP_INL void rp_step(const ReadCtx &r, const FLines &F, const int32_t *fl_base, int strand, int f, bool has_next, RpStep &D)
+{
+    rp_seed_piece(r, F, fl_base, strand, f, true, D);
+    if (!has_next) { D.jk = 0; return; }
+    if (!D.single) return;
+    JGeo G; junction_geo(r, F, f, strand == 1 ? f - 1 : f + 1, G);
+    D.j_chr = G.at1_chr;
+    if (G.cls == JC_DEL) { D.jk = G.tl > 0 ? 1 : 0; D.j_n = G.tl > 0 ? 1 : 0; D.j_first = D.j_last = (G.tl << 4) | C_D; D.j_reflen = G.tl; }
+    else if (G.cls == JC_MIS) {
+        const int f2 = strand == 1 ? f - 1 : f + 1;
+        const int32_t *jt = F.jt + GS_WORDS * (f < f2 ? f : f2);
+        if (jt[GS_HAS]) {
+            D.jk = 2; D.j_n = jt[GS_N]; D.j_ptr = (long long)(F.jarena + jt[GS_OFF]); D.j_reflen = jt[GS_TLEN]; D.j_readlen = G.s_qlen;
+            if (D.j_n > 0) { D.j_first = F.jarena[jt[GS_OFF]]; D.j_last = F.jarena[jt[GS_OFF] + D.j_n - 1]; }
+        }
+    }
+}
+
+HP_NOINL void phase_fillrepair(const PhaseArgs &a, int round, int u, int wave_slot, HP_L int32_t *lds, ReadCtx &r)
+{
+    UnitRec &U = a.units[(size_t)round * a.unit_cap + u];
+    const int rd = U.read, line = U.line;
+    RdMeta &M = a.meta[rd];
+    if (*(volatile int32_t *)&M.status & ST_DEAD) return;
+    if (!lj_params_ok(&a.P) || a.job_cap <= 64) return;
+    read_bind(r, a.P, a.ref, a.in, rd, a.slab + (size_t)wave_slot * a.slab_fill, a.slab_fill, lds, a.prof, 0);
+    pers_bind(r, a, rd);
+    Ctx &cx = r.cx;
+#ifdef HP_PROF
+    cx.prof_rp = a.prof ? a.prof + ((size_t)a.n_reads + 1 + rd) * 64 : nullptr;
+#endif
+    const lamsa_hp_para *P = cx.P;
+    FLines F;
+    F.n = M.fl_n[round]; F.nfrag = M.fl_nfrag[round];
+    flines_bind(F, a.fl_base + M.fl_off[round], F.n, M.fl_tot[round]);
+    F.jarena = a.job_base;
+    const int f0 = F.frag_off[line], nfr = F.frag_off[line + 1] - f0;
+    if (nfr < 2) return;
+    const int strand = r.h_strand[F.fr_seed[F.fr_seed_off[f0]]];
+    cig_t *cbuf = (cig_t *)arena_alloc(cx, sizeof(cig_t) * HP_RP_CIG * 64);
+    uint8_t *zbuf = (uint8_t *)arena_alloc(cx, (size_t)HP_RP_QCAP * HP_RP_TCAP * 64 + 64);
+    int32_t *cand = (int32_t *)arena_alloc(cx, sizeof(int32_t) * RP_CAND_WORDS * (2 * (size_t)nfr + 2));
+    if (!cbuf || !zbuf || !cand) return;
+    r.flip = strand != 1;
+    HP_G int32_t *g_cand = (HP_G int32_t *)cand;
+    int n_cand = 0;
+    for (int t0 = 0; t0 < nfr; t0 += 64) {
+        wv::Lane<int> hasA, hasB, first, CA[RP_CAND_WORDS], CB[RP_CAND_WORDS];
+        WAVE_FOR(l) {
+            const int t = t0 + l;
+            hasA[l] = 0; hasB[l] = 0; first[l] = 0;
+#pragma unroll
+            for (int k = 0; k < RP_CAND_WORDS; ++k) { CA[k][l] = 0; CB[k][l] = 0; }
+            RpCand A, B;
+            if (t < nfr) {
+                RpStep D, N;
+                const int f = strand == 1 ? f0 + nfr - 1 - t : f0 + t;
+                rp_step(r, F, a.fl_base, strand, f, t < nfr - 1, D);
+                if (D.single && t < nfr - 1 && D.jk != 3) {
+                    rp_seed_piece(r, F, a.fl_base, strand, strand == 1 ? f - 1 : f + 1, false, N);
+                    const bool junc = D.jk != 0 && D.j_n > 0;
+                    if (N.single && N.s_n > 0 && (junc || D.s_n > 0) && rp_junction_test(junc ? D.j_last : D.s_last, N.s_first)) {
+                        if ((junc ? D.j_n : D.s_n) < 2) first[l] += 1;
+                        else {
+                            hasA[l] = 1;
+                            A.c1 = junc ? D.j_ptr : D.s_ptr; A.n1 = junc ? D.j_n : D.s_n; A.c2 = N.s_ptr; A.n2 = N.s_n; A.first2 = N.s_first;
+                            A.readend0 = D.rend + (junc ? D.j_readlen : 0); A.refend0 = D.fend + (junc ? D.j_reflen : 0); A.chr = N.s_chr; A.slot = N.s_slot + GS_OFF;
+#pragma unroll
+                            for (int k = 0; k < RP_CAND_WORDS; ++k) CA[k][l] = rp_cand_word(A, k);
+                        }
+                    }
+                }
+                if (D.single && D.s_n > 0 && (D.jk == 1 || D.jk == 2) && D.j_n > 0 && rp_junction_test(D.s_last, D.j_first)) {
+                    if (D.s_n < 2) first[l] += 1;
+                    else {
+                        hasB[l] = 1;
+                        B.c1 = D.s_ptr; B.n1 = D.s_n; B.c2 = D.jk == 2 ? D.j_ptr : 0; B.n2 = D.j_n; B.first2 = D.j_first;
+                        B.readend0 = D.rend; B.refend0 = D.fend; B.chr = D.j_chr; B.slot = D.s_slot + GS_N;
+#pragma unroll
+                        for (int k = 0; k < RP_CAND_WORDS; ++k) CB[k][l] = rp_cand_word(B, k);
+                    }
+                }
+            }
+        }
+        if (wv::ballot(first)) HP_RP_COUNT(cx, 105, wv::reduce_sum(first));
+        const unsigned long long ma = wv::ballot(hasA), mb = wv::ballot(hasB);
+        if (!(ma | mb)) continue;
+        const int na = __builtin_popcountll(ma);
+        WAVE_FOR(l) {
+            HP_G int32_t *wa = g_cand + RP_CAND_WORDS * (size_t)(n_cand + __builtin_popcountll(ma & ((1ull << l) - 1)));
+            HP_G int32_t *wb = g_cand + RP_CAND_WORDS * (size_t)(n_cand + na + __builtin_popcountll(mb & ((1ull << l) - 1)));
+#pragma unroll
+            for (int k = 0; k < RP_CAND_WORDS; ++k) { if (hasA[l]) wa[k] = CA[k][l]; if (hasB[l]) wb[k] = CB[k][l]; }
+        }
+        n_cand += na + __builtin_popcountll(mb);
+    }
+    wv::sync();
+    const HP_G uint8_t *read = (const HP_G uint8_t *)(a.in.read_seq + a.in.read_off[rd]);
+    for (int c0 = 0; c0 < n_cand; c0 += 64) {
+        wv::Lane<int> nw, slot, whyl;
+        WAVE_FOR(l) {
+            nw[l] = 0; slot[l] = 0; whyl[l] = 0;
+            if (c0 + l < n_cand) {
+                RpCand C; RpOut o; LCig bd;
+                o.len2 = o.len1 = o.band = o.rounds = o.need = 0;
+                rp_cand_load(g_cand + RP_CAND_WORDS * (size_t)(c0 + l), C);
+                cig_t *w = cbuf + (size_t)l * HP_RP_CIG;
+                bd.c = w + RP_HDR; bd.n = 0;
+                LaneJob J;
+                J.pac = (const HP_G uint8_t *)a.ref.pac; J.z = (HP_G uint8_t *)zbuf; J.zl = l; J.zs = HP_RP_QCAP; J.cells = 0;
+                J.row = lds + l; J.qrow = (HP_L uint8_t *)(lds + (HP_RP_QCAP + 2) * 64) + l; J.rev = 0;
+                const int why = rp_lane_job(P, a.ref, read, r.L, strand == 1, C, J, bd, o);
+                if (why == 0) {
+                    nw[l] = RP_HDR + bd.n; slot[l] = C.slot;
+                    w[RP_TAIL] = o.tail; w[RP_READEND] = C.readend0; w[RP_REFEND_LO] = (int32_t)(C.refend0 & 0xffffffffll); w[RP_REFEND_HI] = (int32_t)(C.refend0 >> 32);
+                    w[RP_NEED] = o.need; w[RP_POP] = o.pop; w[RP_E1] = o.e1; w[RP_CI] = o.ci; w[RP_E2] = o.e2; w[RP_BDN] = bd.n; w[RP_TB] = o.tb; w[RP_CELLS] = (int)J.cells;
+                } else whyl[l] = why;
+                HP_RPLOG(why, o.len2, o.len1, o.band, o.rounds, o.need, C.n1);
+            }
+        }
+        for (int k = 105; k <= 109; ++k) { wv::Lane<int> is; WAVE_FOR(l) { is[l] = whyl[l] == k; } const unsigned long long m = wv::ballot(is); if (m) HP_RP_COUNT(cx, k, __builtin_popcountll(m)); }
+        wv::Lane<int> pre = nw;
+        wv::scan_add_excl(pre);
+        const int total = wv::reduce_sum(nw);
+        if (total == 0) continue;
+        unsigned long long base = 0;
+        if (wv::leader()) base = atomicAdd(&a.ctl->job_cursor, (unsigned long long)total);
+        base = (unsigned long long)wv::uni64((long long)base);
+        if ((int64_t)(base + (unsigned long long)total) + 64 > a.job_cap) { HP_RP_COUNT(cx, 110, __builtin_popcountll(wv::ballot(nw))); break; }
+        WAVE_FOR(l) {
+            if (nw[l] > 0) {
+                HP_G int32_t *w = (HP_G int32_t *)(a.job_base + base + pre[l]);
+                const cig_t *src = cbuf + (size_t)l * HP_RP_CIG;
+                for (int k = 0; k < nw[l]; ++k) w[k] = src[k];
+                ((HP_G int32_t *)a.fl_base)[slot[l]] = (int32_t)(base + pre[l]) + 1;
+            }
+        }
+        HP_RP_COUNT(cx, 104, __builtin_popcountll(wv::ballot(nw)));
+        wv::sync();
+    }
+    r.flip = false;
+}
+
+HP_FN void phase_fillrepair(const PhaseArgs &a, int round, int u, int wave_slot, HP_L int32_t *lds)
+{
+    PH_FRAME_CTX(r);
+    phase_fillrepair(a, round, u, wave_slot, lds, r);
+}
+
+}
```

New measurement: 4.384 (median of 6 runs). +1.6%, better.
